# eridgd/WCT-TF

Measured on AMD Instinct MI355X. Metric: stylized frames/sec @512x512, 5-level relu5->1 pipeline, alpha=0.8, higher is better.
Workload: dtype f16

## Files before the change

wct_tf_amd/csrc/api.h:

```cpp
#pragma once
#include "common.h"
#include "../../include/wct_hip.h"

#include <stdio.h>
#include <string.h>
#include <stdlib.h>
#include <memory>
#include <vector>
#include <cmath>
#include <algorithm>

struct DevBuf {
  void* p = nullptr;
  size_t cap = 0;
  DevBuf() = default;
  DevBuf(const DevBuf&) = delete;
  DevBuf& operator=(const DevBuf&) = delete;
  ~DevBuf() { if (p) hipFree(p); }
};

struct ConvLayer {
  half_t* w = nullptr;
  float* b = nullptr;
  half_t* ww = nullptr;
  int cin = 0, cout = 0;
};

struct PlanStep { char kind; int cin, cout, relu; };

struct Decoder {
  bool loaded = false;
  std::vector<PlanStep> plan;
  std::vector<ConvLayer> convs;
  half_t* last_w = nullptr;
  float* last_b = nullptr;
  std::vector<float*> w32, b32, mw, vw, mb, vb, gw, gb;
  std::vector<int> cin, cout;
  float* grad_arena = nullptr;
  size_t grad_count = 0;
};

struct ProfRec { hipEvent_t a, b; int cls; double flops, bytes; };
constexpr int WCT_EIG_WORDS = 2 + 6 * 3;

constexpr int STYLE_CACHE_KEYS = 4;
struct StyleState {
  WctStyleKey key; int kind;
  float* buf;
  unsigned long long stamp;
};
struct StyleSource {
  float* img = nullptr;
  uint8_t* map = nullptr;
  StyleSource() = default;
  StyleSource(const StyleSource&) = delete;
  StyleSource& operator=(const StyleSource&) = delete;
  ~StyleSource() { if (img) hipFree(img); if (map) hipFree(map); }
};
struct wct_style {
  int Hs = 0, Ws = 0;
  unsigned level_set = 0;
  std::shared_ptr<StyleSource> src;
  int label = -1;
  int rows[6] = {0};
  std::vector<StyleState> cache[6];
  ~wct_style() {
    for (auto& lv : cache)
      for (auto& e : lv) if (e.buf) hipFree(e.buf);
  }
};

struct wct_warm {
  unsigned level_set = 0;
  float* basis[6] = {nullptr};
  bool valid[6] = {false};
  ~wct_warm() { for (float* b : basis) if (b) hipFree(b); }
};

struct wct_ctx {
  int device = 0;
  hipStream_t stream = nullptr;
  bool enc_loaded = false;
  half_t* first_w = nullptr;
  float* first_b = nullptr;
  ConvLayer enc[12];
  float* first_w32 = nullptr;
  float* enc_wt[12] = {nullptr};
  DevBuf train_ws;
  Decoder dec[6];
  DevBuf act[2], feat_c, feat_s[6], img_c, img_s, img_t[2], wct_out, wct_ws, stage[4];
  DevBuf usum_c, usum_s[6], umax;
  DevBuf mix_in, feat_mix[6];
  DevBuf mask_in;
  DevBuf region_ws;
  DevBuf tex_noise, tex[2];
  DevBuf band_f, band_g, band_img;
  DevBuf wrap_img, wrap_g, wrap_f;
  DevBuf resize_tab;
  std::vector<int> resize_host;
  ResizeGeom resize_geom = {};
  DevBuf guided_ab;
  int guided_radius = 8, guided_eps = 650;
  std::vector<wct_style*> styles;
  unsigned long long style_clock = 0;
  std::vector<wct_warm*> warms;
  std::vector<wct_warm*> warm_used;

  int* eig_fail = nullptr;
  int* eig_fail_dev = nullptr;
  float ss_alpha = 0.6f;
  int ss_patch = 3, ss_stride = 1;
  bool prof = false;
  bool no_wino = false;
  std::vector<ProfRec> recs;
  std::vector<std::pair<hipEvent_t, hipEvent_t>> free_events;
  double prof_ms[WCT_PROF_CLASSES] = {0};
  long long prof_n[WCT_PROF_CLASSES] = {0};
  double prof_flops[WCT_PROF_CLASSES] = {0};
  double prof_bytes[WCT_PROF_CLASSES] = {0};
};

inline constexpr int LEVEL_C[6] = {0, 64, 128, 256, 512, 512};
inline constexpr int ENC_CIN[12] = {64, 64, 128, 128, 256, 256, 256, 256, 512, 512, 512, 512};
inline constexpr int ENC_COUT[12] = {64, 128, 128, 256, 256, 256, 256, 512, 512, 512, 512, 512};
inline constexpr int ENC_TAP[12] = {0, 2, 0, 3, 0, 0, 0, 4, 0, 0, 0, 5};
inline constexpr int ENC_POOL_AFTER[12] = {1, 0, 1, 0, 0, 0, 1, 0, 0, 0, 1, 0};

#define TRY(expr) do { int _rc = (expr); if (_rc) return _rc; } while (0)

struct ProfScope {
  wct_ctx* c; ProfRec r; bool on;
  ProfScope(wct_ctx* ctx, int cls, double flops, double bytes) : c(ctx), on(ctx->prof) {
    if (!on) return;
    if (c->free_events.empty()) {
      hipEventCreate(&r.a); hipEventCreate(&r.b);
    } else {
      r.a = c->free_events.back().first; r.b = c->free_events.back().second;
      c->free_events.pop_back();
    }
    r.cls = cls; r.flops = flops; r.bytes = bytes;
    hipEventRecord(r.a, c->stream);
  }
  ~ProfScope() {
    if (!on) return;
    hipEventRecord(r.b, c->stream);
    c->recs.push_back(r);
  }
};

struct StageCost { double cov_flops, cov_bytes, apply_flops, apply_bytes, adain_bytes; };

int ensure(wct_ctx* c, DevBuf& b, size_t bytes);
int stage_in(wct_ctx* c, int slot, const void* host, size_t bytes, void** dev);
int fetch(wct_ctx* c, void* host, const void* dev, size_t bytes);
int eig_status(wct_ctx* c);
int eig_stale(wct_ctx* c);
void free_layer(ConvLayer& l);
void free_decoder(Decoder& d);

int upload(wct_ctx* c, const void* host, size_t bytes, void** dev);
int pack_conv(wct_ctx* c, const float* w_hwio, const float* b, int cin, int cout, ConvLayer* out);

static inline WctCall ctx_call(wct_ctx* c, int mode, int stages) {
  WctCall r = {};
  r.mode = mode; r.stages = stages; r.workspace = c->wct_ws.p; r.workspace_bytes = c->wct_ws.cap;
  r.eig_fail = c->eig_fail_dev; r.stream = c->stream;
  return r;
}
template <typename Launch>
static int run_stages(wct_ctx* c, size_t ws_bytes, unsigned flags, const StageCost& cost, Launch&& launch) {
  TRY(ensure(c, c->wct_ws, ws_bytes));
  if (flags & WCT_FLAG_ADAIN) {
    ProfScope ps(c, 7, 0, cost.adain_bytes);
    return launch(ctx_call(c, 0, 0));
  }
  const int mode = (flags & WCT_FLAG_MODE_NP) ? WCT_MODE_NP : WCT_MODE_TF;
  {
    ProfScope ps(c, 4, cost.cov_flops, cost.cov_bytes);
    TRY(launch(ctx_call(c, mode, WCT_STAGE_COV)));
  }
  {
    ProfScope ps(c, 5, 0, 0);
    TRY(launch(ctx_call(c, mode, WCT_STAGE_EIG)));
  }
  ProfScope ps(c, 6, cost.apply_flops, cost.apply_bytes);
  return launch(ctx_call(c, mode, WCT_STAGE_APPLY));
}
void level_dims(int H, int W, int level, int* h, int* w);
int check_min_size(const char* what, int H, int W, int level);
struct ChainLevel { int l, C, H, W, h, w; };
struct Chain { std::vector<ChainLevel> lv; int Ho, Wo; };
int chain_geometry(int Hc, int Wc, const int* levels, int n_levels, Chain* out);
int run_conv(wct_ctx* c, const ConvLayer& l, const half_t* x, half_t* y16, float* y32, int B, int H, int W, int upsample, int relu,
             int pool = 0, float* usum = nullptr, unsigned* umax = nullptr, bool tap_layer = false);
int run_encoder(wct_ctx* c, const float* img, int B, int H, int W, int clamp01, int deepest, float* const taps32[6],
                float* const* usum = nullptr, unsigned* const* umax = nullptr);
int run_decoder(wct_ctx* c, int level, const half_t* feat16, int B, int h, int w, float* img_out);
int run_transform(wct_ctx* c, const float* fc, int Nc, const float* fs, int Ns, int C, int P, float alpha, unsigned flags, float eps,
                  half_t* out16, float* out32, int* sweeps_dev, const WctFeatStats* st = nullptr,
                  const WctStyleRef* prep = nullptr ,
                  const WctWarmRef* warm = nullptr ,
                  const WctStrength* sm = nullptr );
int mix_weights(const float* weights, int K, float* lambda);
int run_transform_mix(wct_ctx* c, const float* fc, int Nc, const float* const* fs, const int* Ns, int K, const float* lambda, int C,
                      float alpha, unsigned flags, float eps, half_t* out16, float* out32, int* sweeps_dev,
                      const WctFeatStats* st = nullptr, const WctStyleRef* prep = nullptr );
int mask_check(const uint8_t* labels, size_t n, int K);
void mask_counts(const uint8_t* mask, int Hm, int Wm, int h, int w, int stride, int K, int* nk);
int run_transform_masked(wct_ctx* c, const float* fc, int Nc, const MaskGeom& g, const int* nk, const float* const* fs, const int* Ns,
                         int K, int C, float alpha, unsigned flags, float eps, half_t* out16, float* out32, int* sweeps_dev);

int band_rows_for(const Chain& chain, int* band_rows);
int band_rows_check(const Chain& chain, int band_rows);
int run_encoder_banded(wct_ctx* c, const float* img, int H, int W, int clamp01, int level, int band_rows, float* F);
int run_decoder_banded(wct_ctx* c, int level, const half_t* G, int h, int w, int band_rows, float* img_out);
int chunk_rule(int h, int w, int C, int stat_rows, int* rows, int* K);
int run_transform_chunked(wct_ctx* c, const float* fc, size_t Nc, int n_full, int K, const float* fs, int Ns, int C, float alpha,
                          unsigned flags, float eps, half_t* out16, float* out32, int* sweeps_dev, const WctStyleRef* prep = nullptr);

void wrap_halo(int level, int* enc, int* dec_before, int* dec_after);
int wrap_chain_check(int H, int W, const int* levels, int n_levels, Chain* chain);

int run_encoder_wrap(wct_ctx* c, const float* img, int B, int H, int W, int clamp01, int level, float* tap);
int run_decoder_wrap(wct_ctx* c, int level, const half_t* G, int B, int h, int w, float* img_out);
int wrap_encoder_buffers(wct_ctx* c, int B, int H, int W, int level);
int wrap_decoder_buffers(wct_ctx* c, int B, int h, int w, int level);

int run_guided_filter(wct_ctx* c, const uint8_t* stylized, const void* content, int content_f32, int B, int Ho, int Wo, int Hc, int Wc,
                      int radius, int eps_q, uint8_t* out);

int warm_live(const wct_ctx* c, const wct_warm* wm);
```

wct_tf_amd/csrc/api_drivers.hip:

```cpp
#include "api.h"

void level_dims(int H, int W, int level, int* h, int* w) {
  for (int l = 1; l < level; ++l) { H = (H + 1) / 2; W = (W + 1) / 2; }
  *h = H; *w = W;
}

int check_min_size(const char* what, int H, int W, int level) {
  int h, w;
  level_dims(H, W, level, &h, &w);
  if (h < 2 || w < 2) {
    wct_set_error("%s %dx%d is too small for relu%d_1: its %dx%d feature map cannot be reflect-padded (need >= %dx%d pixels)",
                  what, H, W, level, h, w, (1 << (level - 1)) + 1, (1 << (level - 1)) + 1);
    return WCT_ERR_ARG;
  }
  return WCT_OK;
}

int chain_geometry(int Hc, int Wc, const int* levels, int n_levels, Chain* out) {
  ARG_CHECK(levels && out && n_levels >= 1 && Hc >= 2 && Wc >= 2);
  out->lv.clear();
  int H = Hc, W = Wc;
  for (int i = 0; i < n_levels; ++i) {
    ARG_CHECK(levels[i] >= 1 && levels[i] <= 5);
    const int l = levels[i];
    TRY(check_min_size("content", H, W, l));
    int h, w;
    level_dims(H, W, l, &h, &w);
    out->lv.push_back(ChainLevel{l, LEVEL_C[l], H, W, h, w});
    H = h << (l - 1); W = w << (l - 1);
  }
  out->Ho = H; out->Wo = W;
  return WCT_OK;
}

int run_conv(wct_ctx* c, const ConvLayer& l, const half_t* x, half_t* y16, float* y32, int B, int H, int W, int upsample, int relu,
             int pool, float* usum, unsigned* umax, bool tap_layer) {
  ConvArgs a;
  a.x = x; a.w = l.w; a.bias = l.b; a.y16 = y16; a.y32 = y32; a.usum = usum; a.umax = umax;
  a.w_wino = c->no_wino || tap_layer ? nullptr : l.ww;
  a.B = B; a.H = H; a.W = W; a.Cin = l.cin; a.Cout = l.cout; a.upsample = upsample; a.relu = relu; a.pool = pool;
  const double px = (double)B * H * W;
  const double in_px = upsample ? px / 4 : px;
  const double out_px = pool ? (double)B * ((H + 1) / 2) * ((W + 1) / 2) : px;
  ProfScope ps(c, conv3x3_wino_takes(a) ? 9 : 0, 2.0 * px * 9 * l.cin * l.cout,
               in_px * l.cin * 2 + out_px * l.cout * ((y16 ? 2 : 0) + (y32 ? 4 : 0)) + 9.0 * l.cin * l.cout * 2);
  return launch_conv3x3(a, c->stream);
}

int run_encoder(wct_ctx* c, const float* img, int B, int H, int W, int clamp01, int deepest, float* const taps32[6],
                float* const* usum, unsigned* const* umax) {
  if (!c->enc_loaded) { wct_set_error("encoder weights not set (wct_set_encoder)"); return WCT_ERR_STATE; }
  ARG_CHECK(deepest >= 1 && deepest <= 5 && H >= 2 && W >= 2);
  const size_t act_bytes = (size_t)B * H * W * 64 * sizeof(half_t);
  TRY(ensure(c, c->act[0], act_bytes));
  TRY(ensure(c, c->act[1], act_bytes));
  half_t* cur = (half_t*)c->act[0].p;
  half_t* nxt = (half_t*)c->act[1].p;
  static const int fuse_conv1_env = getenv("WCT_FUSE_CONV1") ? atoi(getenv("WCT_FUSE_CONV1")) : 1;
  const bool fuse_conv1 = fuse_conv1_env && deepest > 1 && !taps32[1];
  if (!fuse_conv1) {
    ConvFirstArgs a;
    a.x = img; a.wfrag = c->first_w; a.bias = c->first_b;
    a.y16 = deepest > 1 ? cur : nullptr; a.y32 = taps32[1];
    a.B = B; a.H = H; a.W = W; a.clamp01 = clamp01;
    a.usum = usum && taps32[1] ? usum[1] : nullptr; a.umax = a.usum ? umax[1] : nullptr;
    const double px = (double)B * H * W;
    ProfScope ps(c, 1, 2.0 * px * 27 * 64, px * (12 + 64 * ((a.y16 ? 2 : 0) + (a.y32 ? 4 : 0))));
    TRY(launch_conv_first(a, c->stream));
  }
  if (deepest == 1) return WCT_OK;
  int h = H, w = W;
  for (int i = 0; i < 12; ++i) {
    const ConvLayer& l = c->enc[i];
    const int tap = ENC_TAP[i];
    const bool last = tap == deepest;
    const bool fuse = ENC_POOL_AFTER[i];
    float* const us = tap && taps32[tap] && usum ? usum[tap] : nullptr;
    if (i == 0 && fuse_conv1) {
      ConvArgs a;
      a.x = nullptr; a.w = l.w; a.bias = l.b; a.y16 = nxt; a.y32 = nullptr; a.usum = nullptr; a.umax = nullptr;
      a.B = B; a.H = h; a.W = w; a.Cin = 64; a.Cout = 64; a.upsample = 0; a.relu = 1; a.pool = fuse;
      a.img1 = img; a.w1frag = c->first_w; a.bias1 = c->first_b; a.clamp01 = clamp01;
      const double px = (double)B * h * w, out_px = fuse ? (double)B * ((h + 1) / 2) * ((w + 1) / 2) : px;
      ProfScope ps(c, 8, 2.0 * px * (27 * 64 + 9 * 64 * 64), px * 12 + out_px * 64 * 2 + 9.0 * 64 * 64 * 2);
      TRY(launch_conv3x3(a, c->stream));
    } else
    TRY(run_conv(c, l, cur, last ? nullptr : nxt, tap ? taps32[tap] : nullptr, B, h, w, 0, 1, fuse, us, us ? umax[tap] : nullptr, tap != 0));
    half_t* t = cur; cur = nxt; nxt = t;
    if (last) break;
    if (fuse) { h = (h + 1) / 2; w = (w + 1) / 2; }
  }
  return WCT_OK;
}

int run_decoder(wct_ctx* c, int level, const half_t* feat16, int B, int h, int w, float* img_out) {
  Decoder& d = c->dec[level];
  if (!d.loaded) { wct_set_error("decoder weights for relu%d_1 not set (wct_set_decoder)", level); return WCT_ERR_STATE; }
  const int scale = 1 << (level - 1);
  const size_t act_bytes = (size_t)B * h * scale * w * scale * 64 * sizeof(half_t);
  const size_t deep_bytes = (size_t)B * h * w * LEVEL_C[level] * sizeof(half_t) * 4;
  TRY(ensure(c, c->act[0], act_bytes > deep_bytes ? act_bytes : deep_bytes));
  TRY(ensure(c, c->act[1], act_bytes > deep_bytes ? act_bytes : deep_bytes));
  const half_t* cur = feat16;
  half_t* bufs[2] = {(half_t*)c->act[0].p, (half_t*)c->act[1].p};
  int which = 0, ci = 0, up = 0;
  const size_t nsteps = d.plan.size();
  for (size_t si = 0; si < nsteps; ++si) {
    const PlanStep& s = d.plan[si];
    if (s.kind == 'U') { up = 1; h *= 2; w *= 2; continue; }
    if (s.cout == 3) {
      ARG_CHECK(up == 0);
      ConvLastArgs a;
      a.x = cur; a.wfrag = d.last_w; a.bias = d.last_b; a.y = img_out; a.B = B; a.H = h; a.W = w;
      const double px = (double)B * h * w;
      ProfScope ps(c, 2, 2.0 * px * 576 * 3, px * (128 + 12));
      TRY(launch_conv_last(a, c->stream));
    } else {
      half_t* out = bufs[which];
      TRY(run_conv(c, d.convs[ci++], cur, out, nullptr, B, h, w, up, 1));
      cur = out; which ^= 1; up = 0;
    }
  }
  return WCT_OK;
}

int run_transform(wct_ctx* c, const float* fc, int Nc, const float* fs, int Ns, int C, int P, float alpha, unsigned flags, float eps,
                  half_t* out16, float* out32, int* sweeps_dev, const WctFeatStats* st, const WctStyleRef* prep, const WctWarmRef* warm,
                  const WctStrength* sm) {
  const WctSkip skip = (flags & WCT_FLAG_STYLE_SHARED) ? WCT_SKIP_SHARED_STYLE : WCT_SKIP_NONE;
  const StageCost cost = {(double)P * 2.0 * C * C * ((double)Nc + Ns), (double)P * 2.0 * ((double)Nc + Ns) * C * 4,
                          (double)P * (2.0 * C * C * Nc + 6.0 * C * C * C),
                          (double)P * Nc * C * (4 + (out16 ? 2 : 0) + (out32 ? 4 : 0) + (sm ? 4 : 0)) + (sm ? (double)P * Nc : 0.0),
                          (double)P * (2.0 * Nc + 2.0 * Ns) * C * 4 + (double)P * Nc * C * 6 + (sm ? (double)P * Nc : 0.0)};
  return run_stages(c, wct_workspace_bytes(C, Nc, Ns, P), flags, cost, [&](WctCall r) {
    r.alpha = alpha; r.eps = r.stages ? eps : 1e-5f; r.out16 = out16; r.out32 = out32; r.sweeps_dev = sweeps_dev;
    if (!r.stages) return launch_adain(fc, Nc, fs, Ns, C, P, skip, r, st, prep, sm);
    return launch_wct(fc, Nc, fs, Ns, C, P, skip, r, st, prep, warm, sm);
  });
}

int mix_weights(const float* weights, int K, float* lambda) {
  if (K < 1 || K > WCT_MIX_MAX) { wct_set_error("style mix: K = %d styles, must be 1 .. %d", K, (int)WCT_MIX_MAX); return WCT_ERR_ARG; }
  if (!weights) { wct_set_error("style mix: no weights"); return WCT_ERR_ARG; }
  double sum = 0.0;
  for (int k = 0; k < K; ++k) {
    if (!(weights[k] >= 0.f) || !std::isfinite(weights[k])) {
      wct_set_error("style mix: weight %d is %g; weights must be finite and >= 0", k, (double)weights[k]);
      return WCT_ERR_ARG;
    }
    sum += weights[k];
  }
  if (!(sum > 0.0) || !std::isfinite(sum)) { wct_set_error("style mix: the weights sum to %g, must be > 0", sum); return WCT_ERR_ARG; }
  for (int k = 0; k < K; ++k) lambda[k] = (float)(weights[k] / sum);
  return WCT_OK;
}

int run_transform_mix(wct_ctx* c, const float* fc, int Nc, const float* const* fs, const int* Ns, int K, const float* lambda, int C,
                      float alpha, unsigned flags, float eps, half_t* out16, float* out32, int* sweeps_dev, const WctFeatStats* st,
                      const WctStyleRef* prep) {
  double ns = 0;
  for (int k = 0; k < K; ++k) ns += Ns[k];
  const StageCost cost = {2.0 * C * C * (Nc + ns), 2.0 * (Nc + ns) * C * 4, 2.0 * C * C * Nc + 6.0 * C * C * C * (K + 1) + 2.0 * C * C * K,
                          (double)Nc * C * (4 + (out16 ? 2 : 0) + (out32 ? 4 : 0)), (2.0 * Nc + 2.0 * ns) * C * 4 + (double)Nc * C * 6};
  return run_stages(c, wct_mix_workspace_bytes(C, Nc, Ns, K, lambda), flags, cost, [&](WctCall r) {
    r.alpha = alpha; r.eps = r.stages ? eps : 1e-5f; r.out16 = out16; r.out32 = out32; r.sweeps_dev = sweeps_dev;
    if (!r.stages) return launch_adain_mix(fc, Nc, fs, Ns, K, lambda, C, r, st, prep);
    return launch_wct_mix(fc, Nc, fs, Ns, K, lambda, C, r, st, prep);
  });
}

int mask_check(const uint8_t* labels, size_t n, int K) {
  if (K < 1 || K > WCT_MIX_MAX) { wct_set_error("mask: K = %d styles, must be 1 .. %d", K, (int)WCT_MIX_MAX); return WCT_ERR_ARG; }
  uint8_t top = 0;
  for (size_t i = 0; i < n; ++i) top = labels[i] > top ? labels[i] : top;
  if (top >= K) { wct_set_error("mask: label %d with K = %d styles (labels must be 0 .. K - 1)", (int)top, K); return WCT_ERR_ARG; }
  return WCT_OK;
}

void mask_counts(const uint8_t* mask, int Hm, int Wm, int h, int w, int stride, int K, int* nk) {
  for (int k = 0; k < K; ++k) nk[k] = 0;
  for (int i = 0; i < h; ++i) {
    const uint8_t* row = mask + (size_t)std::min(i * stride, Hm - 1) * Wm;
    for (int j = 0; j < w; ++j) ++nk[row[std::min(j * stride, Wm - 1)]];
  }
}

int run_transform_masked(wct_ctx* c, const float* fc, int Nc, const MaskGeom& g, const int* nk, const float* const* fs, const int* Ns,
                         int K, int C, float alpha, unsigned flags, float eps, half_t* out16, float* out32, int* sweeps_dev) {
  double ns = 0;
  int P = 0;
  for (int k = 0; k < K; ++k) { ns += nk[k] >= 2 ? Ns[k] : 0; P += nk[k] >= 2; }
  const StageCost cost = {2.0 * C * C * (Nc + ns), (4.0 * Nc + 2.0 * (Nc + ns)) * C * 4, 2.0 * C * C * Nc + 6.0 * C * C * C * P,
                          (double)Nc * C * (4 + (out16 ? 2 : 0) + (out32 ? 4 : 0)), (4.0 * Nc + 2.0 * ns) * C * 4 + (double)Nc * C * 6};
  return run_stages(c, wct_masked_workspace_bytes(C, Nc, nk, Ns, K), flags, cost, [&](WctCall r) {
    r.alpha = alpha; r.eps = r.stages ? eps : 1e-5f; r.out16 = out16; r.out32 = out32; r.sweeps_dev = sweeps_dev;
    if (!r.stages) return launch_adain_masked(fc, Nc, g, nk, fs, Ns, K, C, r);
    return launch_wct_masked(fc, Nc, g, nk, fs, Ns, K, C, r);
  });
}
```

wct_tf_amd/csrc/api_stylize.hip:

```cpp
#include "api.h"

extern "C" int wct_output_size(int Hc, int Wc, const int* levels, int n_levels, int* Ho, int* Wo) {
  ARG_CHECK(Ho && Wo);
  Chain chain;
  TRY(chain_geometry(Hc, Wc, levels, n_levels, &chain));
  *Ho = chain.Ho; *Wo = chain.Wo;
  return WCT_OK;
}

static int check_levels(const wct_ctx* c, const int* levels, int n_levels, const wct_style* const* handles = nullptr, int K = 0) {
  for (int i = 0; i < n_levels; ++i) {
    ARG_CHECK(levels[i] >= 1 && levels[i] <= 5);
    for (int k = 0; k < K; ++k)
      if (!(handles[k]->level_set & (1u << levels[i]))) {
        wct_set_error("prepared style %d was not prepared for relu%d_1", k, levels[i]);
        return WCT_ERR_ARG;
      }
    if (!c->dec[levels[i]].loaded) { wct_set_error("decoder weights for relu%d_1 not set", levels[i]); return WCT_ERR_STATE; }
  }
  return WCT_OK;
}

static int stylize_checks(wct_ctx* c, int Hc, int Wc, const uint8_t* const* styles, const int* Hs, const int* Ws, int K,
                          const int* levels, int n_levels, int* deepest, Chain* chain) {
  TRY(check_levels(c, levels, n_levels));
  TRY(chain_geometry(Hc, Wc, levels, n_levels, chain));
  *deepest = *std::max_element(levels, levels + n_levels);
  for (int k = 0; k < K; ++k) { ARG_CHECK(styles[k]); TRY(check_min_size("style", Hs[k], Ws[k], *deepest)); }
  return WCT_OK;
}

static size_t sample_bytes(unsigned flags) { return (flags & WCT_FLAG_IMAGES_F32) ? sizeof(float) : 1; }

static int images_f32(wct_ctx* c, unsigned flags, const void* content, size_t nc, const void* style, size_t ns, const float** img_c,
                      const float** img_s) {
  *img_c = (const float*)content; *img_s = (const float*)style;
  if (flags & WCT_FLAG_IMAGES_F32) return WCT_OK;
  TRY(ensure(c, c->img_c, nc * 4));
  TRY(ensure(c, c->img_s, ns * 4));
  ProfScope ps(c, 7, 0, (double)(nc + ns) * 5);
  TRY(launch_u8_to_f32((const uint8_t*)content, (float*)c->img_c.p, nc, c->stream));
  TRY(launch_u8_to_f32((const uint8_t*)style, (float*)c->img_s.p, ns, c->stream));
  *img_c = (const float*)c->img_c.p; *img_s = (const float*)c->img_s.p;
  return WCT_OK;
}

constexpr size_t UROW = 32 * UMAX_SLOTS;
static bool fuse_stats() {
  static const int on = getenv("WCT_FUSE_STATS") ? atoi(getenv("WCT_FUSE_STATS")) : 1;
  return on != 0;
}

template <typename StyleAt, typename Transform>
static int stylize_levels(wct_ctx* c, const float* img_c, const void* content_raw, int B, const Chain& chain, unsigned flags,
                          size_t umax_clear, int clear_from, StyleAt&& style_at, Transform&& transform, uint8_t* out) {
  unsigned* const umax_c = (unsigned*)c->umax.p;
  const float* cur = img_c;
  for (int i = 0; i < (int)chain.lv.size(); ++i) {
    const ChainLevel& g = chain.lv[i];
    const int l = g.l, C = g.C, h = g.h, w = g.w;
    TRY(ensure(c, c->feat_c, (size_t)B * h * w * C * 4));
    float* ctaps[6] = {};
    ctaps[l] = (float*)c->feat_c.p;
    float* us_c[6] = {};
    unsigned* um_c[6] = {};
    if (fuse_stats() && w % 16 == 0) {
      TRY(ensure(c, c->usum_c, (size_t)B * h * (w / 16) * C * 4));
      us_c[l] = (float*)c->usum_c.p; um_c[l] = umax_c;
      if (i >= clear_from) HIP_TRY(hipMemsetAsync(umax_c, 0, umax_clear, c->stream));
    }
    WctFeatStats st = {};
    st.u[0] = us_c[l]; st.umax[0] = um_c[l];
    TRY(run_encoder(c, cur, B, g.H, g.W, i > 0, l, ctaps, us_c, um_c));
    TRY(ensure(c, c->wct_out, (size_t)B * h * w * C * 2));
    if (l == 5 && (flags & WCT_FLAG_SWAP5)) {
      int hs, ws;
      style_at(l, 0, &hs, &ws);
      ARG_CHECK(h >= c->ss_patch && w >= c->ss_patch && hs >= c->ss_patch && ws >= c->ss_patch);
      TRY(ensure(c, c->wct_ws, style_swap_workspace_bytes(C, h, w, hs, ws, c->ss_patch, c->ss_stride)));
      ProfScope ps(c, 7, 0, 0);
      for (int b = 0; b < B; ++b)
        TRY(launch_style_swap((float*)c->feat_c.p + (size_t)b * h * w * C, h, w, style_at(l, b, &hs, &ws), hs, ws, C, c->ss_alpha,
                              c->ss_patch, c->ss_stride, -1.f, (half_t*)c->wct_out.p + (size_t)b * h * w * C, nullptr,
                              c->wct_ws.p, c->wct_ws.cap, c->stream, c->eig_fail_dev));
    } else
      TRY(transform(i, g, st));
    DevBuf& dst = c->img_t[i & 1];
    TRY(ensure(c, dst, (size_t)B * (h << (l - 1)) * (w << (l - 1)) * 3 * 4));
    TRY(run_decoder(c, l, (half_t*)c->wct_out.p, B, h, w, (float*)dst.p));
    cur = (float*)dst.p;
  }
  const int H = chain.Ho, W = chain.Wo, Hc = chain.lv[0].H, Wc = chain.lv[0].W;
  const int f32 = (flags & WCT_FLAG_IMAGES_F32) ? 1 : 0;
  if (flags & WCT_FLAG_GUIDED) {
    {
      ProfScope ps(c, 7, 0, (double)B * H * W * 3 * 5);
      TRY(launch_f32_to_u8(cur, out, (size_t)B * H * W * 3, c->stream));
    }
    TRY(run_guided_filter(c, out, content_raw, f32, B, H, W, Hc, Wc, c->guided_radius, c->guided_eps, out));
    if (!(flags & WCT_FLAG_CONTENT_COLORS)) return WCT_OK;
    ProfScope ps(c, 7, 0, (double)B * H * W * 3 * 2 + (double)B * Hc * Wc * 3 * (f32 ? 4 : 1));
    return launch_content_colors_u8_any(out, content_raw, f32, B, H, W, Hc, Wc, out, c->stream);
  }
  if (flags & WCT_FLAG_CONTENT_COLORS) {
    ProfScope ps(c, 7, 0, (double)B * H * W * 3 * 5 + (double)B * Hc * Wc * 3 * (f32 ? 4 : 1));
    return launch_content_colors_f32(cur, content_raw, f32, B, H, W, Hc, Wc, out, c->stream);
  }
  ProfScope ps(c, 7, 0, (double)B * H * W * 3 * 5);
  return launch_f32_to_u8(cur, out, (size_t)B * H * W * 3, c->stream);
}

template <typename Enqueue>
static int host_frame(wct_ctx* c, const uint8_t* content, int Hc, int Wc, const int* levels, int n_levels, unsigned flags,
                      uint8_t* out, Enqueue&& enqueue) {
  HIP_TRY(hipSetDevice(c->device));
  TRY(eig_stale(c));
  int Ho, Wo;
  TRY(wct_output_size(Hc, Wc, levels, n_levels, &Ho, &Wo));
  void* dc;
  TRY(stage_in(c, 0, content, (size_t)Hc * Wc * 3 * sample_bytes(flags), &dc));
  TRY(ensure(c, c->stage[2], (size_t)Ho * Wo * 3));
  TRY(enqueue(dc, (uint8_t*)c->stage[2].p));
  TRY(fetch(c, out, c->stage[2].p, (size_t)Ho * Wo * 3));
  return eig_status(c);
}

extern "C" int wct_stylize_batch_dev(wct_ctx* c, const uint8_t* content, int Hc, int Wc, const uint8_t* style,
                                     int Hs, int Ws, int B, const int* levels, int n_levels, float alpha,
                                     unsigned flags, uint8_t* out) {
  ARG_CHECK(c && content && style && out && levels && n_levels >= 1 && n_levels <= 16 && B >= 1 && B <= 32);
  HIP_TRY(hipSetDevice(c->device));
  int deepest;
  Chain chain;
  TRY(stylize_checks(c, Hc, Wc, &style, &Hs, &Ws, 1, levels, n_levels, &deepest, &chain));

  const int shared = (flags & WCT_FLAG_STYLE_SHARED) ? 1 : 0;
  const int Bs = shared ? 1 : B;
  const float *img_c, *img_s;
  TRY(images_f32(c, flags, content, (size_t)B * Hc * Wc * 3, style, (size_t)Bs * Hs * Ws * 3, &img_c, &img_s));
  const bool want_stats = fuse_stats();
  TRY(ensure(c, c->umax, 7 * UROW * sizeof(unsigned)));
  unsigned* const umax_c = (unsigned*)c->umax.p;
  if (want_stats) HIP_TRY(hipMemsetAsync(c->umax.p, 0, 7 * UROW * sizeof(unsigned), c->stream));
  float* taps[6] = {};
  float* us_s[6] = {};
  unsigned* um_s[6] = {};
  for (int i = 0; i < n_levels; ++i) {
    const int l = levels[i];
    int h, w;
    level_dims(Hs, Ws, l, &h, &w);
    TRY(ensure(c, c->feat_s[l], (size_t)Bs * h * w * LEVEL_C[l] * 4));
    taps[l] = (float*)c->feat_s[l].p;
    if (want_stats && w % 16 == 0) {
      TRY(ensure(c, c->usum_s[l], (size_t)Bs * h * (w / 16) * LEVEL_C[l] * 4));
      us_s[l] = (float*)c->usum_s[l].p; um_s[l] = umax_c + UROW * l;
    }
  }
  TRY(run_encoder(c, img_s, Bs, Hs, Ws, 0, deepest, taps, us_s, um_s));

  auto style_at = [&](int l, int b, int* hs, int* ws) {
    level_dims(Hs, Ws, l, hs, ws);
    return (const float*)c->feat_s[l].p + (size_t)(shared ? 0 : b) * *hs * *ws * LEVEL_C[l];
  };
  return stylize_levels(c, img_c, content, B, chain, flags, UROW * sizeof(unsigned), 1, style_at,
                        [&](int, const ChainLevel& g, WctFeatStats st) {
                          int hs, ws;
                          const float* fs = style_at(g.l, 0, &hs, &ws);
                          st.u[1] = us_s[g.l]; st.umax[1] = um_s[g.l];
                          return run_transform(c, (float*)c->feat_c.p, g.h * g.w, fs, hs * ws, g.C, B, alpha, flags, -1.f,
                                               (half_t*)c->wct_out.p, nullptr, nullptr, &st);
                        }, out);
}

extern "C" int wct_stylize(wct_ctx* c, const uint8_t* content, int Hc, int Wc, const uint8_t* style, int Hs, int Ws,
                           const int* levels, int n_levels, float alpha, unsigned flags, uint8_t* out) {
  ARG_CHECK(c && content && style && out);
  return host_frame(c, content, Hc, Wc, levels, n_levels, flags, out, [&](void* dc, uint8_t* frame) {
    void* ds;
    TRY(stage_in(c, 1, style, (size_t)Hs * Ws * 3 * sample_bytes(flags), &ds));
    return wct_stylize_batch_dev(c, (uint8_t*)dc, Hc, Wc, (uint8_t*)ds, Hs, Ws, 1, levels, n_levels, alpha, flags, frame);
  });
}

template <typename LevelTransform>
static int stylize_multi(wct_ctx* c, const uint8_t* content, int Hc, int Wc, const uint8_t* const* styles, const int* Hs,
                         const int* Ws, int K, const int* levels, int n_levels, unsigned flags, uint8_t* out,
                         LevelTransform&& level_transform) {
  HIP_TRY(hipSetDevice(c->device));
  int deepest;
  Chain chain;
  TRY(stylize_checks(c, Hc, Wc, styles, Hs, Ws, K, levels, n_levels, &deepest, &chain));
  TRY(eig_stale(c));
  const size_t px = sample_bytes(flags);
  size_t ns_tot = 0, soff[WCT_MIX_MAX];
  for (int k = 0; k < K; ++k) { soff[k] = ns_tot; ns_tot += (size_t)Hs[k] * Ws[k] * 3; }
  const size_t nc = (size_t)Hc * Wc * 3;
  void* dc;
  TRY(stage_in(c, 0, content, nc * px, &dc));
  TRY(ensure(c, c->mix_in, ns_tot * px));
  for (int k = 0; k < K; ++k)
    HIP_TRY(hipMemcpyAsync((char*)c->mix_in.p + soff[k] * px, styles[k], (size_t)Hs[k] * Ws[k] * 3 * px, hipMemcpyHostToDevice, c->stream));
  const float *img_c, *img_s;
  TRY(images_f32(c, flags, dc, nc, c->mix_in.p, ns_tot, &img_c, &img_s));

  size_t foff[6][WCT_MIX_MAX];
  for (int i = 0; i < n_levels; ++i) {
    const int l = levels[i];
    size_t tot = 0;
    for (int k = 0; k < K; ++k) {
      int h, w;
      level_dims(Hs[k], Ws[k], l, &h, &w);
      foff[l][k] = tot;
      tot += (size_t)h * w * LEVEL_C[l];
    }
    TRY(ensure(c, c->feat_mix[l], tot * 4));
  }
  for (int k = 0; k < K; ++k) {
    float* taps[6] = {};
    for (int i = 0; i < n_levels; ++i) taps[levels[i]] = (float*)c->feat_mix[levels[i]].p + foff[levels[i]][k];
    TRY(run_encoder(c, img_s + soff[k], 1, Hs[k], Ws[k], 0, deepest, taps));
  }

  TRY(ensure(c, c->umax, 32 * UMAX_SLOTS * sizeof(unsigned)));
  const size_t frame_bytes = (size_t)chain.Ho * chain.Wo * 3;
  TRY(ensure(c, c->stage[2], frame_bytes));
  auto style_at = [&](int l, int k, int* hs, int* ws) {
    level_dims(Hs[k], Ws[k], l, hs, ws);
    return (const float*)c->feat_mix[l].p + foff[l][k];
  };
  TRY(stylize_levels(c, img_c, dc, 1, chain, flags, UMAX_SLOTS * sizeof(unsigned), 0, style_at,
                     [&](int, const ChainLevel& g, const WctFeatStats& st) {
                       const float* fs[WCT_MIX_MAX];
                       int Ns[WCT_MIX_MAX];
                       for (int k = 0; k < K; ++k) {
                         int hs, ws;
                         fs[k] = style_at(g.l, k, &hs, &ws);
                         Ns[k] = hs * ws;
                       }
                       return level_transform(g, fs, Ns, &st);
                     }, (uint8_t*)c->stage[2].p));
  TRY(fetch(c, out, c->stage[2].p, frame_bytes));
  return eig_status(c);
}

extern "C" int wct_stylize_mix(wct_ctx* c, const uint8_t* content, int Hc, int Wc, const uint8_t* const* styles, const int* Hs,
                               const int* Ws, int K, const float* weights, const int* levels, int n_levels, float alpha,
                               unsigned flags, uint8_t* out) {
  ARG_CHECK(c && content && styles && Hs && Ws && out && levels && n_levels >= 1 && n_levels <= 16);
  float lambda[WCT_MIX_MAX];
  TRY(mix_weights(weights, K, lambda));
  if ((flags & WCT_FLAG_SWAP5) && K > 1) {
    wct_set_error("style mix: WCT_FLAG_SWAP5 needs K = 1 (style-swap is not linear in the style; got K = %d)", K);
    return WCT_ERR_ARG;
  }
  if (flags & WCT_FLAG_STYLE_SHARED) { wct_set_error("style mix: WCT_FLAG_STYLE_SHARED is for wct_stylize_batch_dev"); return WCT_ERR_ARG; }
  return stylize_multi(c, content, Hc, Wc, styles, Hs, Ws, K, levels, n_levels, flags, out,
                       [&](const ChainLevel& g, const float* const* fs, const int* Ns, const WctFeatStats* st) {
                         return run_transform_mix(c, (float*)c->feat_c.p, g.h * g.w, fs, Ns, K, lambda, g.C, alpha, flags, -1.f,
                                                  (half_t*)c->wct_out.p, nullptr, nullptr, st);
                       });
}

extern "C" int wct_stylize_masked(wct_ctx* c, const uint8_t* content, int Hc, int Wc, const uint8_t* mask, const uint8_t* const* styles,
                                  const int* Hs, const int* Ws, int K, const int* levels, int n_levels, float alpha, unsigned flags,
                                  uint8_t* out) {
  ARG_CHECK(c && content && mask && styles && Hs && Ws && out && levels && n_levels >= 1 && n_levels <= 16 && Hc >= 2 && Wc >= 2);
  TRY(mask_check(mask, (size_t)Hc * Wc, K));
  if ((flags & WCT_FLAG_SWAP5) && K > 1) {
    wct_set_error("mask: WCT_FLAG_SWAP5 needs K = 1 (style-swap is not a per-region affine map; got K = %d)", K);
    return WCT_ERR_ARG;
  }
  if (flags & WCT_FLAG_STYLE_SHARED) { wct_set_error("mask: WCT_FLAG_STYLE_SHARED is for wct_stylize_batch_dev"); return WCT_ERR_ARG; }
  for (int i = 0; i < n_levels; ++i) ARG_CHECK(levels[i] >= 1 && levels[i] <= 5);
  HIP_TRY(hipSetDevice(c->device));
  TRY(ensure(c, c->mask_in, (size_t)Hc * Wc));
  HIP_TRY(hipMemcpyAsync(c->mask_in.p, mask, (size_t)Hc * Wc, hipMemcpyHostToDevice, c->stream));
  return stylize_multi(c, content, Hc, Wc, styles, Hs, Ws, K, levels, n_levels, flags, out,
                       [&](const ChainLevel& g, const float* const* fs, const int* Ns, const WctFeatStats*) {
                         int nk[WCT_MIX_MAX];
                         mask_counts(mask, Hc, Wc, g.h, g.w, 1 << (g.l - 1), K, nk);
                         const MaskGeom mg = {(const uint8_t*)c->mask_in.p, Hc, Wc, g.w, 1 << (g.l - 1)};
                         return run_transform_masked(c, (float*)c->feat_c.p, g.h * g.w, mg, nk, fs, Ns, K, g.C, alpha, flags, -1.f,
                                                     (half_t*)c->wct_out.p, nullptr, nullptr);
                       });
}

int warm_live(const wct_ctx* c, const wct_warm* wm) {
  if (wm && std::find(c->warms.begin(), c->warms.end(), wm) != c->warms.end()) return WCT_OK;
  wct_set_error("warm state %p is not a live state of this context (freed, or created by another context)", (const void*)wm);
  return WCT_ERR_STATE;
}

extern "C" int wct_warm_create(wct_ctx* c, const int* levels, int n_levels, wct_warm** out) {
  ARG_CHECK(c && levels && out && n_levels >= 1 && n_levels <= 16);
  *out = nullptr;
  for (int i = 0; i < n_levels; ++i) ARG_CHECK(levels[i] >= 1 && levels[i] <= 5);
  HIP_TRY(hipSetDevice(c->device));
  std::unique_ptr<wct_warm> wm(new wct_warm());
  for (int i = 0; i < n_levels; ++i) {
    const int l = levels[i];
    if (wm->basis[l]) continue;
    wm->level_set |= 1u << l;
    if (hipMalloc((void**)&wm->basis[l], (size_t)LEVEL_C[l] * LEVEL_C[l] * sizeof(float)) != hipSuccess) {
      wct_set_error("hipMalloc failed (warm state, relu%d_1)", l);
      return WCT_ERR_NOMEM;
    }
  }
  c->warms.push_back(wm.get());
  *out = wm.release();
  return WCT_OK;
}

extern "C" void wct_warm_free(wct_ctx* c, wct_warm* wm) {
  if (!c || !wm) return;
  auto it = std::find(c->warms.begin(), c->warms.end(), wm);
  if (it == c->warms.end()) return;
  hipSetDevice(c->device);
  hipStreamSynchronize(c->stream);
  c->warms.erase(it);
  c->warm_used.erase(std::remove(c->warm_used.begin(), c->warm_used.end(), wm), c->warm_used.end());
  delete wm;
}

extern "C" int wct_warm_reset(wct_ctx* c, wct_warm* wm) {
  ARG_CHECK(c != nullptr);
  TRY(warm_live(c, wm));
  for (bool& v : wm->valid) v = false;
  return WCT_OK;
}

extern "C" int wct_warm_basis(wct_ctx* c, const wct_warm* wm, int level, int* valid, float* V_host) {
  ARG_CHECK(c && valid);
  TRY(warm_live(c, wm));
  if (level < 1 || level > 5 || !(wm->level_set & (1u << level))) {
    wct_set_error("warm state: relu%d_1 is not in the state's level set", level);
    return WCT_ERR_ARG;
  }
  HIP_TRY(hipSetDevice(c->device));
  HIP_TRY(hipStreamSynchronize(c->stream));
  *valid = wm->valid[level] ? 1 : 0;
  if (V_host && wm->valid[level]) TRY(fetch(c, V_host, wm->basis[level], (size_t)LEVEL_C[level] * LEVEL_C[level] * sizeof(float)));
  return WCT_OK;
}

static int style_live(const wct_ctx* c, const wct_style* st) {
  if (st && std::find(c->styles.begin(), c->styles.end(), st) != c->styles.end()) return WCT_OK;
  wct_set_error("prepared style %p is not a live handle of this context (freed, or prepared by another context)", (const void*)st);
  return WCT_ERR_STATE;
}

static bool same_key(const WctStyleKey& a, const WctStyleKey& b) { return a.nslab == b.nslab && a.nsplit == b.nsplit && a.ksplit == b.ksplit; }

static StyleState* state_find(wct_style* st, int level, const WctStyleKey& key, int kind) {
  for (auto& e : st->cache[level])
    if (e.kind == kind && same_key(e.key, key)) return &e;
  return nullptr;
}

struct StyleNeed { int level; WctStyleKey key; };

static int style_rows(const wct_style* st, int level) { return st->rows[level]; }

static int region_count(const uint8_t* map, int Hm, int Wm, int h, int w, int stride, int label) {
  int n = 0;
  for (int i = 0; i < h; ++i) {
    const uint8_t* row = map + (size_t)std::min(i * stride, Hm - 1) * Wm;
    for (int j = 0; j < w; ++j) n += row[std::min(j * stride, Wm - 1)] == label;
  }
  return n;
}

static int style_fill(wct_ctx* c, wct_style* const* group, int G, int kind, const std::vector<StyleNeed>* needs) {
  bool any = false;
  for (int g = 0; g < G; ++g) any = any || !needs[g].empty();
  if (!any) return WCT_OK;
  HIP_TRY(hipStreamSynchronize(c->stream));
  const wct_style* st0 = group[0];
  const bool region = st0->label >= 0;
  int deepest = 0, labels = 0;
  size_t row_floats = 0;
  float* taps[6] = {};
  for (int g = 0; g < G; ++g)
    for (const StyleNeed& n : needs[g]) {
      int h, w;
      level_dims(st0->Hs, st0->Ws, n.level, &h, &w);
      TRY(ensure(c, c->feat_s[n.level], (size_t)h * w * LEVEL_C[n.level] * 4));
      taps[n.level] = (float*)c->feat_s[n.level].p;
      deepest = std::max(deepest, n.level);
      labels = std::max(labels, group[g]->label + 1);
      row_floats = std::max(row_floats, (size_t)style_rows(group[g], n.level) * LEVEL_C[n.level]);
    }
  int *perm[6] = {}, *seg_off[6] = {};
  void* compact_ws = nullptr;
  float* rows = nullptr;
  if (region) {
    size_t off = 0, poff[6] = {}, soff[6] = {}, cbytes = 0;
    auto take = [&](size_t bytes) { const size_t at = off; off += (bytes + 255) & ~(size_t)255; return at; };
    for (int l = 1; l <= 5; ++l) {
      if (!taps[l]) continue;
      int h, w;
      level_dims(st0->Hs, st0->Ws, l, &h, &w);
      poff[l] = take((size_t)h * w * sizeof(int));
      soff[l] = take((WCT_MIX_MAX + 1) * sizeof(int));
      cbytes = std::max(cbytes, mask_compact_workspace_bytes(h * w));
    }
    const size_t coff = take(cbytes), roff = take(row_floats * sizeof(float));
    TRY(ensure(c, c->region_ws, off));
    char* base = (char*)c->region_ws.p;
    for (int l = 1; l <= 5; ++l)
      if (taps[l]) { perm[l] = (int*)(base + poff[l]); seg_off[l] = (int*)(base + soff[l]); }
    compact_ws = base + coff;
    rows = (float*)(base + roff);
  }
  TRY(run_encoder(c, st0->src->img, 1, st0->Hs, st0->Ws, 0, deepest, taps));
  if (region)
    for (int l = 1; l <= 5; ++l) {
      if (!taps[l]) continue;
      int h, w;
      level_dims(st0->Hs, st0->Ws, l, &h, &w);
      ProfScope ps(c, 7, 0, (double)h * w * 2);
      TRY(launch_mask_compact(MaskGeom{st0->src->map, st0->Hs, st0->Ws, w, 1 << (l - 1)}, h * w, labels, perm[l], seg_off[l], compact_ws,
                              c->stream));
    }
  std::vector<float*> fresh;
  int rc = WCT_OK;
  for (int g = 0; g < G && !rc; ++g) {
    wct_style* st = group[g];
    int gathered = 0;
    for (const StyleNeed& n : needs[g]) {
      const int C = LEVEL_C[n.level], Ns = style_rows(st, n.level);
      auto& lv = st->cache[n.level];
      float* buf = nullptr;
      if ((int)lv.size() >= STYLE_CACHE_KEYS) {
        int old = -1;
        for (int i = 0; i < (int)lv.size(); ++i)
          if (lv[i].stamp != c->style_clock && (old < 0 || lv[i].stamp < lv[old].stamp)) old = i;
        if (old >= 0) { buf = lv[old].buf; lv.erase(lv.begin() + old); }
      }
      if (!buf && hipMalloc((void**)&buf, wct_style_state_floats(C) * sizeof(float)) != hipSuccess) {
        wct_set_error("hipMalloc failed (prepared style state, relu%d_1)", n.level);
        rc = WCT_ERR_NOMEM;
        break;
      }
      lv.push_back(StyleState{n.key, kind, buf, c->style_clock});
      fresh.push_back(buf);
      if (hipMemsetAsync(buf, 0, wct_style_state_floats(C) * sizeof(float), c->stream) != hipSuccess) { wct_set_error("hipMemsetAsync failed"); rc = WCT_ERR_HIP; break; }
      const float* feat = taps[n.level];
      if (region) {
        if (gathered != n.level) {
          ProfScope ps(c, 7, 0, (double)Ns * C * 8);
          if ((rc = launch_mask_gather_segment(taps[n.level], perm[n.level], seg_off[n.level], st->label, Ns, C, rows, c->stream))) break;
          gathered = n.level;
        }
        feat = rows;
      }
      if ((rc = ensure(c, c->wct_ws, wct_style_workspace_bytes(C, Ns, n.key)))) break;
      ProfScope ps(c, kind == 2 ? 7 : 5, 0, 0);
      WctCall r = ctx_call(c, kind == 1 ? WCT_MODE_NP : WCT_MODE_TF, WCT_STAGE_ALL);
      r.eps = -1.f;
      if ((rc = launch_style_state(feat, Ns, C, n.key, kind == 2, r, buf))) break;
    }
  }
  if (!rc && hipStreamSynchronize(c->stream) != hipSuccess) { wct_set_error("hipStreamSynchronize failed (prepared style)"); rc = WCT_ERR_HIP; }
  if (!rc) rc = eig_status(c);
  if (rc) {
    hipStreamSynchronize(c->stream);
    for (int g = 0; g < G; ++g)
      for (auto& lv : group[g]->cache)
        for (size_t i = lv.size(); i-- > 0;)
          if (std::find(fresh.begin(), fresh.end(), lv[i].buf) != fresh.end()) { hipFree(lv[i].buf); lv.erase(lv.begin() + i); }
  }
  return rc;
}

// ... 709 lines not shown
```

wct_tf_amd/csrc/common.h:

```cpp
#pragma once
#include <hip/hip_runtime.h>
#include <stdint.h>
#include <stddef.h>
#include "skip_rule.h"

typedef _Float16 half_t;
typedef _Float16 half8 __attribute__((ext_vector_type(8)));
typedef _Float16 half4 __attribute__((ext_vector_type(4)));
typedef float f32x16 __attribute__((ext_vector_type(16)));
typedef float f32x4 __attribute__((ext_vector_type(4)));

#define WCT_OK 0
#define WCT_ERR_HIP -1
#define WCT_ERR_ARG -2
#define WCT_ERR_STATE -3
#define WCT_ERR_NOMEM -4
#define WCT_ERR_NOCONV -5

void wct_set_error(const char* fmt, ...);

#define HIP_TRY(expr)                                                          \
  do {                                                                         \
    hipError_t _e = (expr);                                                    \
    if (_e != hipSuccess) {                                                    \
      wct_set_error("%s failed: %s (%s:%d)", #expr, hipGetErrorString(_e),     \
                    __FILE__, __LINE__);                                       \
      return WCT_ERR_HIP;                                                      \
    }                                                                          \
  } while (0)

#define ARG_CHECK(cond)                                                        \
  do {                                                                         \
    if (!(cond)) {                                                             \
      wct_set_error("invalid argument: %s (%s:%d)", #cond, __FILE__, __LINE__);\
      return WCT_ERR_ARG;                                                      \
    }                                                                          \
  } while (0)

static inline int cdiv(int a, int b) { return (a + b - 1) / b; }

constexpr size_t WCT_LAUNCH_BYTES = (size_t)1 << 31;
static inline bool launch_map_fits(size_t elems, size_t bytes) { return elems * bytes < WCT_LAUNCH_BYTES; }


struct ConvArgs {
  const half_t* x;
  const half_t* w;
  const float* bias;
  half_t* y16;
  float* y32;
  int B, H, W;
  int Cin, Cout;
  int upsample;
  int relu;
  int pool;
  float* usum;
  unsigned* umax;
  const float* img1 = nullptr;
  const half_t* w1frag = nullptr;
  const float* bias1 = nullptr;
  int clamp01 = 0;
  const half_t* w_wino = nullptr;
};
constexpr int UMAX_SLOTS = 64;
__device__ __forceinline__ void umax_merge(unsigned* umax_img, int slot, float vmax, int lane) {
#pragma unroll
  for (int o = 32; o > 0; o >>= 1) vmax = fmaxf(vmax, __shfl_xor(vmax, o, 64));
  if (lane == 0) {
    unsigned* w = umax_img + (slot & (UMAX_SLOTS - 1));
    const unsigned bits = __builtin_bit_cast(unsigned, vmax);
    if (bits > __atomic_load_n(w, __ATOMIC_RELAXED)) atomicMax(w, bits);
  }
}
int launch_conv3x3(const ConvArgs& a, hipStream_t s);
bool conv3x3_wino_takes(const ConvArgs& a);
int launch_conv3x3_wino(const ConvArgs& a, hipStream_t s);

struct ConvFirstArgs {
  const float* x;
  const half_t* wfrag;
  const float* bias;
  half_t* y16;
  float* y32;
  int B, H, W;
  int clamp01;
  float* usum;
  unsigned* umax;
};

__device__ __forceinline__ void unit_row_sum4(f32x4& t) {
  float a = t[0], b = t[1], c = t[2], d = t[3];
#define WCT_DPP_STEP(ctrl)                                                             \
  "v_add_f32_dpp %0, %0, %0 " ctrl " row_mask:0xf bank_mask:0xf bound_ctrl:1\n"       \
  "v_add_f32_dpp %1, %1, %1 " ctrl " row_mask:0xf bank_mask:0xf bound_ctrl:1\n"       \
  "v_add_f32_dpp %2, %2, %2 " ctrl " row_mask:0xf bank_mask:0xf bound_ctrl:1\n"       \
  "v_add_f32_dpp %3, %3, %3 " ctrl " row_mask:0xf bank_mask:0xf bound_ctrl:1\n"
  asm volatile("s_nop 1\n"
               WCT_DPP_STEP("quad_perm:[1,0,3,2]")
               WCT_DPP_STEP("quad_perm:[2,3,0,1]")
               WCT_DPP_STEP("row_half_mirror")
               WCT_DPP_STEP("row_mirror")
               : "+v"(a), "+v"(b), "+v"(c), "+v"(d));
#undef WCT_DPP_STEP
  t[0] = a; t[1] = b; t[2] = c; t[3] = d;
}
int launch_conv_first(const ConvFirstArgs& a, hipStream_t s);

struct ConvLastArgs {
  const half_t* x;
  const half_t* wfrag;
  const float* bias;
  float* y;
  int B, H, W;
};
int launch_conv_last(const ConvLastArgs& a, hipStream_t s);

int launch_maxpool2x2(const half_t* x, half_t* y, int B, int H, int W, int C, hipStream_t s);
int launch_u8_to_f32(const uint8_t* x, float* y, size_t n, hipStream_t s);
int launch_f32_to_u8(const float* x, uint8_t* y, size_t n, hipStream_t s);
int launch_f32_to_f16(const float* x, half_t* y, size_t n, hipStream_t s);
int launch_f16_to_f32(const half_t* x, float* y, size_t n, hipStream_t s);

struct GemmArgs {
  const float* A; int lda; int a_kmajor;
  const float* B; int ldb; int b_kmajor;
  const float* a_sub_m;
  const float* b_sub_n;
  const float* a_sub_k;
  const float* a_scale_k;
  int M, N, K;
  int ksplit;
  float* out32; half_t* out16; int ldo;
  size_t out_split_stride;
  const float* bias_n;
  int nsplit;
  size_t sA, sB, s_sub_m, s_sub_n, s_sub_k, s_scale_k, s_out, s_bias;
  const float* A_odd;
  size_t sA_odd;
  WctSkip skip;
  int blend; float alpha; unsigned* mabs;
  const float* mask_diag; size_t s_mask; int* mask_out; const int* mask_in;
};

int launch_gemm(GemmArgs g, int nsplit, int nbatch, hipStream_t s);

enum { WCT_MODE_NP = 0, WCT_MODE_TF = 1 };

struct WctFeatStats { const float* u[2]; const unsigned* umax[2]; };

struct WctStyleKey { int nslab, nsplit, ksplit; };
WctStyleKey wct_style_key(int C, int Nc, int Ns);
size_t wct_style_state_floats(int C);
size_t wct_style_workspace_bytes(int C, int Ns, const WctStyleKey& key);
struct WctStyleRef { const float* state[8]; };
struct WctStyleSlots { const float* state[32]; };

struct WctWarmRef { float* basis; int valid; };

struct WctStrength { const uint8_t* smap; int Hm, Wm, w, stride; };

struct WctCall {
  float alpha; int mode;
  float eps;
  half_t* out16; float* out32;
  void* workspace; size_t workspace_bytes;
  int* sweeps_dev;
  int stages;
  int* eig_fail;
  hipStream_t stream;
};
enum { WCT_STAGE_COV = 1, WCT_STAGE_EIG = 2, WCT_STAGE_APPLY = 4, WCT_STAGE_ALL = 7, WCT_STAGE_EIG_FP32UPDATE = 8 };

int launch_style_state(const float* style, int Ns, int C, const WctStyleKey& key, int adain, const WctCall& r, float* state);

size_t wct_workspace_bytes(int C, int Nc, int Ns, int P);
int launch_wct(const float* content, int Nc, const float* style, int Ns, int C, int P, WctSkip skip, const WctCall& r,
               const WctFeatStats* stats, const WctStyleRef* prep, const WctWarmRef* warm, const WctStrength* sm = nullptr);
int launch_adain(const float* content, int Nc, const float* style, int Ns, int C, int P, WctSkip skip, const WctCall& r,
                 const WctFeatStats* stats, const WctStyleRef* prep, const WctStrength* sm = nullptr);
enum { WCT_MIX_MAX = 8 };
size_t wct_mix_workspace_bytes(int C, int Nc, const int* Ns, int K, const float* lambda);
int launch_wct_mix(const float* content, int Nc, const float* const* styles, const int* Ns, int K, const float* lambda, int C,
                   const WctCall& r, const WctFeatStats* stats, const WctStyleRef* prep);
int launch_adain_mix(const float* content, int Nc, const float* const* styles, const int* Ns, int K, const float* lambda, int C,
                     const WctCall& r, const WctFeatStats* stats, const WctStyleRef* prep);
struct MaskGeom { const uint8_t* mask; int Hm, Wm, w, stride; };
size_t mask_compact_workspace_bytes(int N, int G = 1);
int launch_mask_compact(const MaskGeom& g, int N, int K, int* perm, int* seg_off, void* workspace, hipStream_t s);
int launch_mask_gather_segment(const float* x, const int* perm, const int* seg_off, int k, int nk, int C, float* xg, hipStream_t s);
size_t wct_masked_workspace_bytes(int C, int Nc, const int* nk, const int* Ns, int K);
int launch_wct_masked(const float* content, int Nc, const MaskGeom& g, const int* nk, const float* const* styles, const int* Ns, int K,
                      int C, const WctCall& r);
int launch_adain_masked(const float* content, int Nc, const MaskGeom& g, const int* nk, const float* const* styles, const int* Ns, int K,
                        int C, const WctCall& r);
size_t wct_masked_batch_workspace_bytes(int C, int Nc, int G, const int* nk, const int* Ns, int K);
int wct_masked_batch_pairs(int G, const int* nk, int K);
int launch_mask_compact_batch(const MaskGeom& g, int N, int K, int G, int* perm, int* seg_off, void* workspace, hipStream_t s);
int launch_wct_masked_batch(const float* content, int Nc, int G, const MaskGeom& g, const int* nk, const int* Ns, int K, int C,
                            const WctCall& r, const WctStyleSlots& states);
int launch_adain_masked_batch(const float* content, int Nc, int G, const MaskGeom& g, const int* nk, const int* Ns, int K, int C,
                              const WctCall& r, const WctStyleSlots& states);
int launch_jacobi_eigh(float* A, float* V, int C, int nmat, void* workspace,
                       size_t workspace_bytes, int* sweeps_done_dev, int* eig_fail, hipStream_t s);
size_t jacobi_workspace_bytes(int C, int nmat);

size_t style_swap_workspace_bytes(int C, int hc, int wc, int hs, int ws, int patch, int stride);
int launch_style_swap(const float* content, int hc, int wc, const float* style, int hs, int ws, int C,
                      float alpha, int patch, int stride, float eps, half_t* out16, float* out32,
                      void* workspace, size_t workspace_bytes, hipStream_t s, int* eig_fail);

int launch_im2col_act(const half_t* x, float* col, int B, int H, int W, int C, int upsample, hipStream_t s);
int launch_im2col_grad(const float* g, float* col, int B, int H, int W, int C, hipStream_t s);
int launch_reflect_fold(const float* gp, float* g, int B, int H, int W, int C, hipStream_t s);
int launch_relu_mask16(float* g, const half_t* act, size_t n, hipStream_t s);
int launch_relu_mask32(float* g, const float* act, size_t n, hipStream_t s);
int launch_upsample_adjoint(const float* gb, float* gs, int B, int h, int w, int C, hipStream_t s);
int launch_maxpool_adjoint(const half_t* pre, const float* gpool, float* gpre, int B, int H, int W, int C, hipStream_t s);
int launch_mse(const float* a, const float* b, size_t n, float weight, float* grad, int accumulate, double* partial,
               float* loss_out, hipStream_t s);
int launch_tv(const float* x, int B, int H, int W, int C, float weight, float* grad, double* partial, float* loss_out, hipStream_t s);
int launch_bias_grad(const float* g, size_t rows, int C, float* partial, float* out, hipStream_t s);
int launch_reduce_slabs(const float* partial, size_t n, int nslab, float* out, hipStream_t s);
int launch_adam(float* w, float* m, float* v, const float* g, size_t n, float lr_t, float b1, float b2, float eps, hipStream_t s);
int launch_pack_conv_frag(const float* w, half_t* frag, int cin, int cout, hipStream_t s);
int launch_pack_conv_wino_frag(const float* w, half_t* frag, int cin, int cout, hipStream_t s);
int launch_pack_last_frag(const float* w, half_t* frag, hipStream_t s);
int launch_transpose_w(const float* w, float* wt, int cin, int cout, int cout_pad, hipStream_t s);
int launch_pad3to4(const float* x, float* y, size_t n, hipStream_t s);
int launch_conv_dgrad(const float* g, const float* wt, int B, int H, int W, int cin, int cout,
                      float* col, float* gp, float* gin, void* scratch, hipStream_t s);
int launch_conv_wgrad(const half_t* x16, int upsample, const float* g, int ldg, int B, int H, int W, int cin, int cout,
                      float* col, float* partial, int nsplit, float* dw, void* scratch, hipStream_t s);
int conv_wgrad_splits(int B, int H, int W);
int launch_pow2_scale(const float* x, size_t n, void* scratch, hipStream_t s);
int launch_conv_first_dgrad(const float* g, const float* wf, float* gp, int B, int H, int W, hipStream_t s);

struct CoralApplyArgs {
  double M[9], src_mean[3], src_std[3], tgt_mean[3], tgt_std[3];
};
int launch_coral_stats(const uint8_t* img, size_t npix, unsigned long long* partial, int nblocks,
                       unsigned long long* out9, hipStream_t s);
int launch_coral_apply(const uint8_t* src, size_t npix, const CoralApplyArgs& a, uint8_t* out_u8,
                       double* out_f64, hipStream_t s);

int launch_content_colors_f32(const float* frame, const void* content, int content_f32, int B, int Ho, int Wo, int Hc, int Wc,
                              uint8_t* out, hipStream_t s);
int launch_content_colors_u8(const uint8_t* stylized, const uint8_t* content, int B, int Ho, int Wo, int Hc, int Wc, uint8_t* out,
                             hipStream_t s);
int launch_content_colors_u8_any(const uint8_t* stylized, const void* content, int content_f32, int B, int Ho, int Wo, int Hc, int Wc,
                                 uint8_t* out, hipStream_t s);

int guided_check(int B, int Ho, int Wo, int Hc, int Wc, int radius, int eps_q);
size_t guided_workspace_bytes(int B, int Ho, int Wo);
int launch_guided_filter(const uint8_t* stylized, const void* content, int content_f32, int B, int Ho, int Wo, int Hc, int Wc, int radius,
                         int eps_q, void* workspace, uint8_t* out, hipStream_t s);

int launch_texture_noise(uint8_t* out, int B, int H, int W, unsigned seed, unsigned first_sample, int smooth, hipStream_t s);

int launch_wrap_pad(const void* in, void* out, int B, int H, int W, int E, int elem_bytes, int t, int b, int l, int r, hipStream_t s);
int launch_wrap_crop(const void* in, void* out, int B, int Hp, int Wp, int E, int elem_bytes, int t, int l, int h, int w, hipStream_t s);

struct ResizeGeom { int H, W, h, w, ksx, ksy, th; };
int resize_check_bytes(int B, int H, int W, int h, int w);
size_t resize_table_ints(int H, int W, int h, int w);
int resize_plan(int H, int W, int h, int w, ResizeGeom* g, int* tabs);
int launch_resize(const uint8_t* in, uint8_t* out, int B, const ResizeGeom& g, const int* tabs_dev, hipStream_t s);
```

wct_tf_amd/csrc/conv.hip:

```cpp
#include "common.h"
#include "conv_tile.h"


template <int MT, int NT, bool POOL, bool OUT32>
__device__ __forceinline__ void conv_epilogue_t(const ConvArgs& p, f32x16 (&acc)[NT][MT], int b, int y0, int x0, int n0,
                                                int wm, int wn, int lane, const unsigned char* bias_lds) {
  constexpr int OOB = (int)0x80000000u;
  const int frag_px = lane & 15;
  const int frag_py = (lane & 31) >> 4;
  const int kgrp = lane >> 5;
  const int Ho = POOL ? (p.H + 1) / 2 : p.H, Wo = POOL ? (p.W + 1) / 2 : p.W;
  const unsigned img_elems = (unsigned)Ho * Wo * p.Cout;
  const __amdgpu_buffer_rsrc_t r16 = __builtin_amdgcn_make_buffer_rsrc(
      (void*)(p.y16 ? p.y16 + (size_t)b * img_elems : nullptr), 0, p.y16 ? img_elems * 2 : 0, 0x00020000);
  const __amdgpu_buffer_rsrc_t r32 = __builtin_amdgcn_make_buffer_rsrc(
      (void*)(OUT32 && p.y32 ? p.y32 + (size_t)b * img_elems : nullptr), 0, OUT32 && p.y32 ? img_elems * 4 : 0, 0x00020000);
  f32x4 bvs[NT][4];
#pragma unroll
  for (int nt = 0; nt < NT; ++nt)
#pragma unroll
    for (int rq = 0; rq < 4; ++rq)
      bvs[nt][rq] = *reinterpret_cast<const f32x4*>(bias_lds + ((wn * NT + nt) * 32 + 8 * rq + 4 * kgrp) * 4);
  const float lo1 = p.relu ? 0.f : -__builtin_inff();
  const h2 lo2 = {(half_t)lo1, (half_t)lo1};
  const int ox = x0 + frag_px;
  const int chan = n0 + wn * NT * 32;
  const bool stats = OUT32 && p.usum != nullptr;
  float* const us = stats ? p.usum + (size_t)b * (p.H * (p.W >> 4)) * p.Cout + chan + 4 * kgrp : nullptr;
  float vmax = 0.f;
#pragma unroll
  for (int mt = 0; mt < MT; ++mt) {
    const int oy = y0 + (wm * MT + mt) * 2 + frag_py;
    const bool in_img = (oy < p.H) & (ox < p.W);
    const bool inside = POOL ? (in_img & (frag_py == 0) & ((frag_px & 1) == 0)) : in_img;
    const int pix = POOL ? (oy >> 1) * Wo + (ox >> 1) : oy * p.W + ox;
    const int off16 = inside ? (pix * p.Cout + chan + 8 * kgrp) * 2 : OOB;
    const int off32 = inside ? (pix * p.Cout + chan + 4 * kgrp) * 4 : OOB;
#pragma unroll
    for (int nt = 0; nt < NT; ++nt) {
      unsigned pk[4][2];
#pragma unroll
      for (int rq = 0; rq < 4; ++rq) {
        f32x4 v;
#pragma unroll
        for (int j = 0; j < 4; ++j) v[j] = acc[nt][mt][rq * 4 + j] + bvs[nt][rq][j];
        if (OUT32) {
#pragma unroll
          for (int j = 0; j < 4; ++j) v[j] = fmaxf(v[j], lo1);
          __builtin_amdgcn_raw_buffer_store_b128(__builtin_bit_cast(u32x4, v), r32, off32 + (nt * 32 + 8 * rq) * 4, 0, 0);
          if (stats) {
            f32x4 t = v;
            unit_row_sum4(t);
            if (in_img) {
              vmax = fmaxf(fmaxf(vmax, fmaxf(v[0], v[1])), fmaxf(v[2], v[3]));
              if (frag_px == 0)
                *reinterpret_cast<f32x4*>(us + (size_t)(oy * (p.W >> 4) + (x0 >> 4)) * p.Cout + nt * 32 + 8 * rq) = t;
            }
          }
        }
        h2 lo = {(half_t)v[0], (half_t)v[1]}, hi = {(half_t)v[2], (half_t)v[3]};
        if (!OUT32) {
          lo = __builtin_elementwise_max(lo, lo2);
          hi = __builtin_elementwise_max(hi, lo2);
        }
        if (POOL) {
          const h2 zero = {(half_t)0.f, (half_t)0.f};
          h2 q[2] = {in_img ? lo : zero, in_img ? hi : zero};
#pragma unroll
          for (int d = 0; d < 2; ++d) {
            unsigned t = __builtin_bit_cast(unsigned, q[d]);
            const h2 o = __builtin_bit_cast(h2, __builtin_amdgcn_update_dpp(0, (int)t, 0xB1, 0xF, 0xF, true));
            q[d] = __builtin_elementwise_max(q[d], o);
            t = __builtin_bit_cast(unsigned, q[d]);
            const auto rows = __builtin_amdgcn_permlane16_swap(t, t, false, false);
            q[d] = __builtin_elementwise_max(__builtin_bit_cast(h2, (unsigned)rows[0]), __builtin_bit_cast(h2, (unsigned)rows[1]));
          }
          lo = q[0]; hi = q[1];
        }
        pk[rq][0] = __builtin_bit_cast(unsigned, lo);
        pk[rq][1] = __builtin_bit_cast(unsigned, hi);
      }
#pragma unroll
      for (int m = 0; m < 2; ++m) {
        auto sx = __builtin_amdgcn_permlane32_swap(pk[2 * m][0], pk[2 * m + 1][0], false, false);
        auto sy = __builtin_amdgcn_permlane32_swap(pk[2 * m][1], pk[2 * m + 1][1], false, false);
        u32x4 o = {sx[0], sy[0], sx[1], sy[1]};
        __builtin_amdgcn_raw_buffer_store_b128(o, r16, off16 + (nt * 32 + 16 * m) * 2, 0, 0);
      }
    }
  }
  if (stats) umax_merge(p.umax + b * UMAX_SLOTS, (int)blockIdx.x * 4 + (int)(threadIdx.x >> 6), vmax, lane);
}

template <int MT, int NT>
__device__ __forceinline__ void conv_epilogue(const ConvArgs& p, f32x16 (&acc)[NT][MT], int b, int y0, int x0, int n0,
                                              int wm, int wn, int lane, const unsigned char* bias_lds) {
  if (p.pool) conv_epilogue_t<MT, NT, true, false>(p, acc, b, y0, x0, n0, wm, wn, lane, bias_lds);
  else if (p.y32) conv_epilogue_t<MT, NT, false, true>(p, acc, b, y0, x0, n0, wm, wn, lane, bias_lds);
  else conv_epilogue_t<MT, NT, false, false>(p, acc, b, y0, x0, n0, wm, wn, lane, bias_lds);
}

template <int TH, int BN, int WM, int WN, bool FUSE1 = false>
__global__ __launch_bounds__(256, ((TH / 2) / WM) * ((BN / 32) / WN) > 8 ? 1 : 2) void conv3x3_mfma_kernel(ConvArgs p, int tiles_x, int tiles_y, int n_tiles, int strip) {
  constexpr int PH = TH + 2;
  constexpr int MT = (TH / 2) / WM;
  constexpr int NT = (BN / 32) / WN;
  constexpr int PATCH_ITEMS = PH * 18 * 4;
  constexpr int PATCH_PER_THREAD = (PATCH_ITEMS + 255) / 256;
  constexpr int PATCH_BYTES = PH * PITCH * 64;
  constexpr bool DB = MT * NT > 8;
  constexpr int NBUF = DB ? 2 : 1;
  constexpr int DUMP_OFF = PATCH_BYTES;
  constexpr int BUF_STRIDE = PATCH_BYTES + 4096;
  constexpr int BIAS_OFF = NBUF * BUF_STRIDE;
  constexpr int IMG_OFF = BIAS_OFF + BN * 4, IMG_H = TH + 4, IMG_W = 20, IMG_ROW = IMG_W * 3, IMG_ZERO = IMG_OFF + IMG_H * IMG_ROW * 4;
  constexpr int W1_OFF = IMG_ZERO + 64, B1_OFF = W1_OFF + 8192;
  constexpr int STG_OFF = B1_OFF + 256;
  static_assert(!FUSE1 || (BN == 64 && !(((TH / 2) / WM) * ((BN / 32) / WN) > 8)), "FUSE1: 64 output channels, single patch buffer");
  constexpr int PF_TAP = TH <= 16 ? 6 : 9;

  extern __shared__ __attribute__((aligned(16))) unsigned char smem[];
  unsigned char* const patch_lds = smem;

  int bid = blockIdx.x;
  const int ntile = bid % n_tiles;
  bid /= n_tiles;
  const int strips_x = FUSE1 ? (tiles_x + strip - 1) / strip : tiles_x;
  const int tx = FUSE1 ? (bid % strips_x) * strip : bid % strips_x;
  const int ty = bid / strips_x;
  const int b = blockIdx.y;
  int y0 = ty * TH;
  int x0 = tx * TW;
  int strip_i = 0;
  const int n0 = ntile * BN;
  int tid_ = threadIdx.x;

next_tile:
  if (FUSE1) asm volatile("" : "+v"(tid_), "+s"(y0));
  const int tid = tid_;
  const int lane = tid & 63;
  const int wave = tid >> 6;
  const int wm = wave / WN, wn = wave % WN;

  const int Hin = p.upsample ? p.H / 2 : p.H;
  const int Win = p.upsample ? p.W / 2 : p.W;
  const half_t* xb = p.x + (size_t)b * Hin * Win * p.Cin;

  unsigned patch_src[PATCH_PER_THREAD];
  unsigned patch_dst[PATCH_PER_THREAD];
#pragma unroll
  for (int i = 0; i < PATCH_PER_THREAD; ++i) {
    int item = tid + i * 256;
    int valid = item < PATCH_ITEMS;
    int pix = valid ? item >> 2 : 0;
    int chunk = item & 3;
    int py = pix / 18, px = pix - py * 18;
    int iy = reflect_idx(y0 - 1 + py, p.H);
    int ix = reflect_idx(x0 - 1 + px, p.W);
    if (p.upsample) { iy >>= 1; ix >>= 1; }
    patch_src[i] = valid ? ((iy * Win + ix) * p.Cin + chunk * 8) * 2 : 0;
    patch_dst[i] = valid ? ((py * PITCH + px) * 4 + (chunk ^ ((px >> 2) & 3))) * 16 : DUMP_OFF + tid * 16;
  }

  const int frag_px = lane & 15;
  const int frag_py = (lane & 31) >> 4;
  const int kgrp = lane >> 5;

  int rd_base[3][2];
#pragma unroll
  for (int kx = 0; kx < 3; ++kx)
#pragma unroll
    for (int ks = 0; ks < 2; ++ks) {
      const int px = frag_px + kx;
      rd_base[kx][ks] = ((wm * MT * 2 + frag_py) * PITCH + px) * 64 + (((ks * 2 + kgrp) ^ ((px >> 2) & 3)) * 16);
    }

  const int c16 = p.Cin >> 4;
  unsigned wfrag[NT];
#pragma unroll
  for (int nt = 0; nt < NT; ++nt)
    wfrag[nt] = (((n0 >> 5) + wn * NT + nt) * 9 * c16 * 512 + lane * 8) * 2;
  const __amdgpu_buffer_rsrc_t w_rsrc = __builtin_amdgcn_make_buffer_rsrc((void*)p.w, 0, 0x7FFFFFFF, 0x00020000);
  const __amdgpu_buffer_rsrc_t x_rsrc = __builtin_amdgcn_make_buffer_rsrc((void*)xb, 0, 0x7FFFFFFF, 0x00020000);

  f32x16 acc[NT][MT];
  if (tid < BN / 4 && strip_i == 0)
    *reinterpret_cast<f32x4*>(smem + BIAS_OFF + tid * 16) = *reinterpret_cast<const f32x4*>(p.bias + n0 + tid * 4);

  const int n_chunks = p.Cin / BK;
  u32x4 patch_regs[PATCH_PER_THREAD];
  half8 wf[2][NT][2];
  half8 bf[2][MT];

  auto read_group = [&](half8 (&dst)[MT], int ky, int kx, int ks, int buf) {
#pragma unroll
    for (int mt = 0; mt < MT; ++mt)
      dst[mt] = *reinterpret_cast<const half8*>(patch_lds + rd_base[kx][ks] + (mt * 2 + ky) * PITCH * 64 + buf * BUF_STRIDE);
  };
  auto mma_group = [&](half8 (&w)[NT][2], half8 (&bq)[MT], int ks) {
#pragma unroll
    for (int mt = 0; mt < MT; ++mt)
#pragma unroll
      for (int nt = 0; nt < NT; ++nt)
        acc[nt][mt] = __builtin_amdgcn_mfma_f32_32x32x16_f16(w[nt][ks], bq[mt], acc[nt][mt], 0, 0, 0);
  };
  auto load_patch = [&](int chunk) {
#pragma unroll
    for (int i = 0; i < PATCH_PER_THREAD; ++i)
      patch_regs[i] = __builtin_amdgcn_raw_buffer_load_b128(x_rsrc, patch_src[i], chunk * BK * 2, 0);
  };
  auto store_patch = [&](int buf) {
#pragma unroll
    for (int i = 0; i < PATCH_PER_THREAD; ++i)
      *reinterpret_cast<u32x4*>(smem + patch_dst[i] + buf * BUF_STRIDE) = patch_regs[i];
  };

  auto make_patch = [&](int chunk) {
    typedef _Float16 h2v __attribute__((ext_vector_type(2)));
    const unsigned char* w1 = smem + W1_OFF + chunk * 4096;
    half8 wh[2], wl[2];
#pragma unroll
    for (int ks = 0; ks < 2; ++ks) {
      wh[ks] = *reinterpret_cast<const half8*>(w1 + ((ks * 2 + 0) * 64 + lane) * 16);
      wl[ks] = *reinterpret_cast<const half8*>(w1 + ((ks * 2 + 1) * 64 + lane) * 16);
    }
    const int l = lane & 31, kg = lane >> 5;
    f32x4 b1[4];
#pragma unroll
    for (int rq = 0; rq < 4; ++rq) b1[rq] = *reinterpret_cast<const f32x4*>(smem + B1_OFF + (chunk * 32 + 8 * rq + 4 * kg) * 4);
    constexpr int NMAIN = PH / 2, NEDGE = (PH + 15) / 16, NT1 = (NMAIN + NEDGE + 3) / 4, R = IMG_ROW;
    const int pxm = l & 15, pxe = 16 + (l & 1);
    const int colm = IMG_OFF + (reflect_idx(x0 - 1 + pxm, p.W) - x0 + 1) * 12 - (y0 - 1) * R * 4;
    const int cole = IMG_OFF + (reflect_idx(x0 - 1 + pxe, p.W) - x0 + 1) * 12 - (y0 - 1) * R * 4;
    const int dstm = pxm * 64 + kg * 8, dste = pxe * 64 + kg * 8, swm = (pxm >> 2) & 3;
#pragma unroll 1
    for (int t = 0; t < NT1; ++t) {
      const int T = t * 4 + wave;
      const bool edge = T >= NMAIN;
      const int py = edge ? (T - NMAIN) * 16 + (l >> 1) : 2 * T + (l >> 4);
      const bool valid = py < PH && T < NMAIN + NEDGE;
      const int pyc = py < PH ? py : PH - 1;
      const int base = (edge ? cole : colm) + reflect_idx(y0 - 1 + pyc, p.H) * (R * 4);
      const unsigned char* b8 = smem + base + kg * 32;
      const unsigned char* bR = smem + base + kg * (R - 1) * 4;
      unsigned w[2][8];
      w[0][0] = *reinterpret_cast<const unsigned*>(b8);
#pragma unroll
      for (int j = 1; j < 8; ++j) w[0][j] = *reinterpret_cast<const unsigned*>(bR + j * 4);
      w[1][0] = *reinterpret_cast<const unsigned*>(bR + (R + 7) * 4);
      w[1][1] = *reinterpret_cast<const unsigned*>(bR + (R + 8) * 4);
#pragma unroll
      for (int j = 2; j < 8; ++j) w[1][j] = *reinterpret_cast<const unsigned*>(b8 + (2 * R + j - 2) * 4);
      f32x16 a1;
#pragma unroll
      for (int r = 0; r < 16; ++r) a1[r] = 0.f;
#pragma unroll
      for (int ks = 0; ks < 2; ++ks) {
        unsigned uh[4], ul[4];
#pragma unroll
        for (int i2 = 0; i2 < 4; ++i2) {
          uh[i2] = __builtin_amdgcn_perm(w[ks][2 * i2 + 1], w[ks][2 * i2], 0x05040100u);
          ul[i2] = __builtin_amdgcn_perm(w[ks][2 * i2 + 1], w[ks][2 * i2], 0x07060302u);
        }
        const half8 bh = __builtin_bit_cast(half8, u32x4{uh[0], uh[1], uh[2], uh[3]});
        const half8 bl = __builtin_bit_cast(half8, u32x4{ul[0], ul[1], ul[2], ul[3]});
        a1 = __builtin_amdgcn_mfma_f32_32x32x16_f16(wl[ks], bh, a1, 0, 0, 0);
        a1 = __builtin_amdgcn_mfma_f32_32x32x16_f16(wh[ks], bl, a1, 0, 0, 0);
        a1 = __builtin_amdgcn_mfma_f32_32x32x16_f16(wh[ks], bh, a1, 0, 0, 0);
      }
      const int dst = valid ? pyc * (PITCH * 64) + (edge ? dste : dstm) : DUMP_OFF + tid * 16;
      const int sw = valid && !edge ? swm : 0;
      const h2v zero2 = {(half_t)0.f, (half_t)0.f};
#pragma unroll
      for (int rq = 0; rq < 4; ++rq) {
        h2v h0 = {(half_t)(a1[rq * 4 + 0] + b1[rq][0]), (half_t)(a1[rq * 4 + 1] + b1[rq][1])};
        h2v h1 = {(half_t)(a1[rq * 4 + 2] + b1[rq][2]), (half_t)(a1[rq * 4 + 3] + b1[rq][3])};
        h0 = __builtin_elementwise_max(h0, zero2);
        h1 = __builtin_elementwise_max(h1, zero2);
        typedef unsigned u32x2 __attribute__((ext_vector_type(2)));
        *reinterpret_cast<u32x2*>(smem + dst + (valid ? (rq ^ sw) * 16 : 0)) = u32x2{__builtin_bit_cast(unsigned, h0), __builtin_bit_cast(unsigned, h1)};
      }
    }
  };

  constexpr int IMG_NP = IMG_H * IMG_W, IMG_PER = (IMG_NP + 255) / 256;
  auto fetch_img = [&](int xt) {
    const float* ib = p.img1 + (size_t)b * p.H * p.W * 3;
#pragma unroll
    for (int i = 0; i < IMG_PER; ++i) {
      const int e = tid + i * 256, ee = e < IMG_NP ? e : IMG_NP - 1;
      const int ry = ee / IMG_W, rx = ee - ry * IMG_W;
      const float* s = ib + ((size_t)reflect_idx(y0 - 2 + ry, p.H) * p.W + reflect_idx(xt - 2 + rx, p.W)) * 3;
#pragma unroll
      for (int c = 0; c < 3; ++c)
        __builtin_amdgcn_global_load_lds(s + c, reinterpret_cast<__attribute__((address_space(3))) void*>(
            (__attribute__((address_space(3))) unsigned char*)smem + STG_OFF + ((i * 3 + c) * 256 + wave * 64) * 4), 4, 0, 0);
    }
  };
  auto park_img = [&]() {
    asm volatile("s_waitcnt vmcnt(0)" ::: "memory");
#pragma unroll
    for (int i = 0; i < IMG_PER; ++i) {
      const int e = tid + i * 256;
      if (e < IMG_NP) {
#pragma unroll
        for (int c = 0; c < 3; ++c) {
          const float raw = *reinterpret_cast<const float*>(smem + STG_OFF + ((i * 3 + c) * 256 + tid) * 4);
          const float v = p.clamp01 ? fminf(fmaxf(raw, 0.f), 1.f) : raw;
          const half_t hi = (half_t)v, lo = (half_t)(v - (float)hi);
          *reinterpret_cast<unsigned*>(smem + IMG_OFF + (e * 3 + c) * 4) =
              (unsigned)__builtin_bit_cast(unsigned short, hi) | ((unsigned)__builtin_bit_cast(unsigned short, lo) << 16);
        }
      }
    }
  };
  if (FUSE1 && strip_i == 0) {
    fetch_img(x0);
    const u32x4 wa = *reinterpret_cast<const u32x4*>(reinterpret_cast<const unsigned char*>(p.w1frag) + tid * 32);
    const u32x4 wb = *reinterpret_cast<const u32x4*>(reinterpret_cast<const unsigned char*>(p.w1frag) + tid * 32 + 16);
    *reinterpret_cast<u32x4*>(smem + W1_OFF + tid * 32) = wa;
    *reinterpret_cast<u32x4*>(smem + W1_OFF + tid * 32 + 16) = wb;
    if (tid < 16) {
      *reinterpret_cast<f32x4*>(smem + B1_OFF + tid * 16) = *reinterpret_cast<const f32x4*>(p.bias1 + tid * 4);
      *reinterpret_cast<unsigned*>(smem + IMG_ZERO + tid * 4) = 0u;
    }
  }

#pragma unroll
  for (int nt = 0; nt < NT; ++nt)
#pragma unroll
    for (int mt = 0; mt < MT; ++mt)
#pragma unroll
      for (int r = 0; r < 16; ++r) acc[nt][mt][r] = 0.f;
  if (FUSE1) {
    park_img();
  } else {
    load_patch(0);
  }
#pragma unroll
  for (int nt = 0; nt < NT; ++nt)
#pragma unroll
    for (int ks = 0; ks < 2; ++ks)
      wf[0][nt][ks] = __builtin_bit_cast(half8, __builtin_amdgcn_raw_buffer_load_b128(w_rsrc, wfrag[nt] + ks * 1024, 0, 0));
  if (FUSE1) {
    __syncthreads();
    make_patch(0);
  } else {
    store_patch(0);
  }
  __syncthreads();
  read_group(bf[0], 0, 0, 0, 0);

#pragma unroll 1
  for (int pair = 0; pair < n_chunks; pair += 2) {
#pragma unroll
    for (int t = 0; t < 18; ++t) {
      const int tap = t % 9, chunk_i = pair + t / 9;
      const int ky = tap / 3, kx = tap % 3;
      const int ntap = (tap + 1) % 9, nky = ntap / 3, nkx = ntap % 3;
      const bool more = chunk_i + 1 < n_chunks;
      const int buf = DB ? t / 9 : 0;
      {
        const int nchunk = tap == 8 ? (more ? chunk_i + 1 : chunk_i) : chunk_i;
        const int wtap = (ntap * c16 + nchunk * 2) * 1024;
#pragma unroll
        for (int nt = 0; nt < NT; ++nt)
#pragma unroll
          for (int ks = 0; ks < 2; ++ks)
            wf[(t + 1) & 1][nt][ks] =
                __builtin_bit_cast(half8, __builtin_amdgcn_raw_buffer_load_b128(w_rsrc, wfrag[nt] + ks * 1024, wtap, 0));
      }
      if (!FUSE1 && tap == PF_TAP && more) load_patch(chunk_i + 1);
      read_group(bf[1], ky, kx, 1, buf);
      if (DB && tap == 8 && more) store_patch(buf ^ 1);
      __builtin_amdgcn_sched_barrier(0);
      mma_group(wf[t & 1], bf[0], 0);
      __builtin_amdgcn_sched_barrier(0);
      if (tap != 8) {
        read_group(bf[0], nky, nkx, 0, buf);
        __builtin_amdgcn_sched_barrier(0);
        mma_group(wf[t & 1], bf[1], 1);
      } else {
        mma_group(wf[t & 1], bf[1], 1);
        if (more) {
          __syncthreads();
          if (FUSE1) {
            make_patch(chunk_i + 1);
            __syncthreads();
          } else if (!DB) {
            if (PF_TAP > 8) load_patch(chunk_i + 1);
            store_patch(0);
            __syncthreads();
          }
        }
        read_group(bf[0], 0, 0, 0, DB ? buf ^ 1 : 0);
      }
      __builtin_amdgcn_sched_barrier(0);
    }
  }
  const bool more_tiles = FUSE1 && strip_i + 1 < strip && tx + strip_i + 1 < tiles_x;
  if (more_tiles) fetch_img(x0 + TW);
  conv_epilogue<MT, NT>(p, acc, b, y0, x0, n0, wm, wn, lane, smem + BIAS_OFF);
  if (more_tiles) {
    ++strip_i;
    x0 += TW;
    goto next_tile;
  }
}

template <int TH, int BN, int WM, int WN, bool FUSE1 = false>
static int launch_conv_cfg(const ConvArgs& a, hipStream_t s) {
  const int tiles_x = cdiv(a.W, TW), tiles_y = cdiv(a.H, TH);
  const int n_tiles = a.Cout / BN;
  constexpr int PH = TH + 2;
  constexpr int NBUF = ((TH / 2) / WM) * ((BN / 32) / WN) > 8 ? 2 : 1;
  const size_t lds = (size_t)NBUF * (PH * PITCH * 64 + 4096) + BN * sizeof(float)
                     + (FUSE1 ? (size_t)(TH + 4) * 20 * 3 * 4 + 64 + 8192 + 256 + 9 * 1024 : 0);
  const long tiles = (long)tiles_x * tiles_y * a.B;
  const int strip = !FUSE1 ? 1 : tiles >= 8192 ? 4 : tiles >= 4096 ? 2 : 1;
  dim3 grid((FUSE1 ? cdiv(tiles_x, strip) : tiles_x) * tiles_y * n_tiles, a.B);
  if (lds > 64 * 1024) {
    static bool raised[16] = {};
    int dev = 0;
    HIP_TRY(hipGetDevice(&dev));
    if (dev >= 0 && dev < 16 && !raised[dev]) {
      HIP_TRY(hipFuncSetAttribute(reinterpret_cast<const void*>(&conv3x3_mfma_kernel<TH, BN, WM, WN, FUSE1>),
                                  hipFuncAttributeMaxDynamicSharedMemorySize, (int)lds));
      raised[dev] = true;
    }
  }
  hipLaunchKernelGGL((conv3x3_mfma_kernel<TH, BN, WM, WN, FUSE1>), grid, dim3(256), lds, s, a, tiles_x, tiles_y, n_tiles, strip);
  HIP_TRY(hipGetLastError());
  return WCT_OK;
}

int launch_conv3x3(const ConvArgs& a, hipStream_t s) {
  ARG_CHECK(a.Cin % 64 == 0 && a.Cout % 64 == 0 && a.H > 1 && a.W > 1 && a.B > 0);
  ARG_CHECK(!a.upsample || (a.H % 2 == 0 && a.W % 2 == 0));
  ARG_CHECK(launch_map_fits((size_t)a.H * a.W * a.Cin, 2));
  ARG_CHECK(launch_map_fits((size_t)a.H * a.W * a.Cout, a.y32 ? 4 : 2));
  ARG_CHECK(!a.usum || (a.y32 && a.umax && a.relu && a.W % 16 == 0));
  ARG_CHECK(!a.pool || (a.relu && !a.y32));
  if (conv3x3_wino_takes(a)) return launch_conv3x3_wino(a, s);
  if (a.img1) {
    ARG_CHECK(a.Cin == 64 && a.Cout == 64 && !a.upsample && a.w1frag && a.bias1);
    return launch_conv_cfg<32, 64, 4, 1, true>(a, s);
  }
  const long px16 = (long)cdiv(a.W, TW) * cdiv(a.H, 16) * a.B;
  const long px32 = (long)cdiv(a.W, TW) * cdiv(a.H, 32) * a.B;
  if (a.Cout % 128 == 0 && px16 * (a.Cout / 128) >= 512) return launch_conv_cfg<16, 128, 2, 2>(a, s);
  if (px32 * (a.Cout / 64) >= 512) return launch_conv_cfg<32, 64, 4, 1>(a, s);
  if (a.Cout % 128 == 0 && px16 * (a.Cout / 128) >= 256) return launch_conv_cfg<16, 128, 2, 2>(a, s);
  if (px16 * (a.Cout / 64) >= 256) return launch_conv_cfg<16, 64, 4, 1>(a, s);
  return launch_conv_cfg<8, 64, 2, 2>(a, s);
}

__global__ __launch_bounds__(256) void conv_first_kernel(ConvFirstArgs p, int strips_x) {
  constexpr int CF_TILES = 4, PATCH_N = 18 * 18 * 3, PER = (PATCH_N + 255) / 256;
  __shared__ float patch[PATCH_N + 4];
  __shared__ __attribute__((aligned(16))) unsigned char tr[4][32 * 256];
  typedef unsigned int u32x4 __attribute__((ext_vector_type(4)));
  const int tid = threadIdx.x, lane = tid & 63, wave = tid >> 6;
  const int sx = blockIdx.x % strips_x, ty = blockIdx.x / strips_x;
  const int b = blockIdx.y;
  const int y0 = ty * 16;
  const float* xb = p.x + (size_t)b * p.H * p.W * 3;
  int e_row[PER], e_px[PER], e_c[PER];
#pragma unroll
  for (int i = 0; i < PER; ++i) {
    const int e = tid + i * 256;
    const int pix = e < PATCH_N ? e / 3 : 0;
    e_c[i] = e < PATCH_N ? e - pix * 3 : 0;
    const int py = pix / 18;
    e_px[i] = pix - py * 18;
    e_row[i] = reflect_idx(y0 - 1 + py, p.H) * p.W;
  }
  float pre[PER];
  auto fetch = [&](int x0) {
#pragma unroll
    for (int i = 0; i < PER; ++i) {
      float v = xb[((size_t)e_row[i] + reflect_idx(x0 - 1 + e_px[i], p.W)) * 3 + e_c[i]];
      pre[i] = p.clamp01 ? fminf(fmaxf(v, 0.f), 1.f) : v;
    }
  };
  auto park = [&]() {
#pragma unroll
    for (int i = 0; i < PER; ++i) if (tid + i * 256 < PATCH_N) patch[tid + i * 256] = pre[i];
  };
  if (tid < 4) patch[PATCH_N + tid] = 0.f;
  fetch(sx * CF_TILES * 16);
  half8 wh[2][2], wl[2][2];
#pragma unroll
  for (int t = 0; t < 2; ++t)
#pragma unroll
    for (int ks = 0; ks < 2; ++ks) {
      wh[t][ks] = *reinterpret_cast<const half8*>(p.wfrag + (((t * 2 + ks) * 2 + 0) * 64 + lane) * 8);
      wl[t][ks] = *reinterpret_cast<const half8*>(p.wfrag + (((t * 2 + ks) * 2 + 1) * 64 + lane) * 8);
    }
  const int frag_px = lane & 15, frag_py = (lane & 31) >> 4, kgrp = lane >> 5;
  int addr[2][8];
#pragma unroll
  for (int ks = 0; ks < 2; ++ks)
#pragma unroll
    for (int j = 0; j < 8; ++j) {
      const int k = ks * 16 + kgrp * 8 + j;
      const int ky = k / 9, kp = k - ky * 9;
      addr[ks][j] = k < 27 ? (((wave * 4 + frag_py + ky) * 18 + frag_px) * 3 + kp) * 4 : 972 * 4;
    }
  f32x4 bias[2][4];
#pragma unroll
  for (int nt = 0; nt < 2; ++nt)
#pragma unroll
    for (int rq = 0; rq < 4; ++rq) bias[nt][rq] = *reinterpret_cast<const f32x4*>(p.bias + nt * 32 + 8 * rq + 4 * kgrp);
  park();
  __syncthreads();
  const unsigned char* pb = reinterpret_cast<const unsigned char*>(patch);
  unsigned char* const wt = tr[wave];
  float vmax = 0.f;
  for (int tile = 0; tile < CF_TILES; ++tile) {
  const int x0 = (sx * CF_TILES + tile) * 16;
  if (x0 >= p.W) break;
  const bool next = tile + 1 < CF_TILES && x0 + 16 < p.W;
  if (next) fetch(x0 + 16);
#pragma unroll
  for (int mt = 0; mt < 2; ++mt) {
    f32x16 acc[2];
#pragma unroll
    for (int nt = 0; nt < 2; ++nt)
#pragma unroll
      for (int r = 0; r < 16; ++r) acc[nt][r] = 0.f;
#pragma unroll
    for (int ks = 0; ks < 2; ++ks) {
      half8 bh, bl;
#pragma unroll
      for (int j = 0; j < 8; ++j) {
        const int off = (ks * 16 + kgrp * 8 + j < 27) ? mt * 2 * 54 * 4 : 0;
        const float v = *reinterpret_cast<const float*>(pb + addr[ks][j] + off);
        bh[j] = (half_t)v;
        bl[j] = (half_t)(v - (float)bh[j]);
      }
#pragma unroll
      for (int nt = 0; nt < 2; ++nt) {
        acc[nt] = __builtin_amdgcn_mfma_f32_32x32x16_f16(wl[nt][ks], bh, acc[nt], 0, 0, 0);
        acc[nt] = __builtin_amdgcn_mfma_f32_32x32x16_f16(wh[nt][ks], bl, acc[nt], 0, 0, 0);
        acc[nt] = __builtin_amdgcn_mfma_f32_32x32x16_f16(wh[nt][ks], bh, acc[nt], 0, 0, 0);
      }
    }
    const int px = lane & 31;
#pragma unroll
    for (int nt = 0; nt < 2; ++nt)
#pragma unroll
      for (int rq = 0; rq < 4; ++rq) {
        f32x4 v;
#pragma unroll
        for (int j = 0; j < 4; ++j) v[j] = fmaxf(acc[nt][rq * 4 + j] + bias[nt][rq][j], 0.f);
        const int piece = nt * 8 + 2 * rq + kgrp;
        *reinterpret_cast<f32x4*>(wt + (px * 16 + (piece ^ (px & 15))) * 16) = v;
        if (p.usum) {
          f32x4 t = v;
          unit_row_sum4(t);
          const int sy = y0 + wave * 4 + mt * 2 + frag_py;
          if (sy < p.H) {
            vmax = fmaxf(fmaxf(vmax, fmaxf(v[0], v[1])), fmaxf(v[2], v[3]));
            if (frag_px == 0)
              *reinterpret_cast<f32x4*>(p.usum + ((size_t)b * (p.H * (p.W >> 4)) + sy * (p.W >> 4) + (x0 >> 4)) * 64 + piece * 4) = t;
          }
        }
      }
    __builtin_amdgcn_fence(__ATOMIC_RELEASE, "wavefront");
    __builtin_amdgcn_wave_barrier();
    const int oy0 = y0 + wave * 4 + mt * 2;
    if (p.y32) {
      const int piece = lane & 15;
#pragma unroll
      for (int it = 0; it < 8; ++it) {
        const int q = it * 4 + (lane >> 4);
        const int oy = oy0 + (q >> 4), ox = x0 + (q & 15);
        const f32x4 v = *reinterpret_cast<const f32x4*>(wt + (q * 16 + (piece ^ (q & 15))) * 16);
        if (oy < p.H && ox < p.W) *reinterpret_cast<f32x4*>(p.y32 + (((size_t)b * p.H + oy) * p.W + ox) * 64 + piece * 4) = v;
      }
    }
    if (p.y16) {
      const int c8 = lane & 7;
#pragma unroll
      for (int it = 0; it < 4; ++it) {
        const int q = it * 8 + (lane >> 3);
        const int oy = oy0 + (q >> 4), ox = x0 + (q & 15);
        const f32x4 v0 = *reinterpret_cast<const f32x4*>(wt + (q * 16 + ((2 * c8) ^ (q & 15))) * 16);
        const f32x4 v1 = *reinterpret_cast<const f32x4*>(wt + (q * 16 + ((2 * c8 + 1) ^ (q & 15))) * 16);
        half8 h;
#pragma unroll
        for (int j = 0; j < 4; ++j) { h[j] = (half_t)v0[j]; h[4 + j] = (half_t)v1[j]; }
        if (oy < p.H && ox < p.W) *reinterpret_cast<half8*>(p.y16 + (((size_t)b * p.H + oy) * p.W + ox) * 64 + c8 * 8) = h;
      }
    }
    __builtin_amdgcn_fence(__ATOMIC_RELEASE, "wavefront");
    __builtin_amdgcn_wave_barrier();
  }
  if (next) {
    __syncthreads();
    park();
    __syncthreads();
  }
  }
  if (p.usum) umax_merge(p.umax + b * UMAX_SLOTS, (int)blockIdx.x * 4 + wave, vmax, lane);
}

int launch_conv_first(const ConvFirstArgs& a, hipStream_t s) {
  ARG_CHECK(a.H > 1 && a.W > 1 && a.B > 0);
  ARG_CHECK(!a.usum || (a.y32 && a.umax && a.W % 16 == 0));
  const int strips_x = cdiv(a.W, 64), tiles_y = cdiv(a.H, 16);
  hipLaunchKernelGGL(conv_first_kernel, dim3(strips_x * tiles_y, a.B), dim3(256), 0, s, a, strips_x);
  HIP_TRY(hipGetLastError());
  return WCT_OK;
}

__global__ __launch_bounds__(256) void conv_last_kernel(ConvLastArgs p, int tiles_x) {
  constexpr int PP = 33;
  __shared__ float part[18 * 18 * PP];
  const int tid = threadIdx.x, lane = tid & 63, wave = tid >> 6;
  const int tx = blockIdx.x % tiles_x, ty = blockIdx.x / tiles_x;
  const int b = blockIdx.y;
  const int y0 = ty * 16, x0 = tx * 16;
  const half_t* xb = p.x + (size_t)b * p.H * p.W * 64;
  half8 wf[4];
#pragma unroll
  for (int ks = 0; ks < 4; ++ks) wf[ks] = *reinterpret_cast<const half8*>(p.wfrag + (ks * 64 + lane) * 8);
  half8 bf[3][4];
  int qs[3];
#pragma unroll
  for (int i = 0; i < 3; ++i) {
    const int tile = wave + 4 * i;
    const int q = tile * 32 + (lane & 31);
    qs[i] = q;
    const int qq = q < 324 ? q : 323;
    const int py = qq / 18, px = qq - py * 18;
    const int iy = reflect_idx(y0 - 1 + py, p.H), ix = reflect_idx(x0 - 1 + px, p.W);
    const half_t* src = xb + ((size_t)iy * p.W + ix) * 64 + (lane >> 5) * 8;
    if (tile < 11) {
#pragma unroll
      for (int ks = 0; ks < 4; ++ks) bf[i][ks] = *reinterpret_cast<const half8*>(src + ks * 16);
    }
  }
#pragma unroll
  for (int i = 0; i < 3; ++i) {
    if (wave + 4 * i >= 11) break;
    f32x16 acc;
#pragma unroll
    for (int r = 0; r < 16; ++r) acc[r] = 0.f;
#pragma unroll
    for (int ks = 0; ks < 4; ++ks) acc = __builtin_amdgcn_mfma_f32_32x32x16_f16(wf[ks], bf[i][ks], acc, 0, 0, 0);
    if (qs[i] < 324) {
#pragma unroll
      for (int r = 0; r < 16; ++r)
        part[qs[i] * PP + (r & 3) + 8 * (r >> 2) + 4 * (lane >> 5)] = acc[r];
    }
  }
  __syncthreads();
  const int ly = tid >> 4, lx = tid & 15;
  const int oy = y0 + ly, ox = x0 + lx;
  float a0 = p.bias[0], a1 = p.bias[1], a2 = p.bias[2];
#pragma unroll
  for (int tap = 0; tap < 9; ++tap) {
    const int ky = tap / 3, kx = tap - ky * 3;
    const float* pq = part + ((ly + ky) * 18 + lx + kx) * PP + tap * 3;
    a0 += pq[0]; a1 += pq[1]; a2 += pq[2];
  }
  if (oy < p.H && ox < p.W) {
    float* o = p.y + (((size_t)b * p.H + oy) * p.W + ox) * 3;
    o[0] = a0; o[1] = a1; o[2] = a2;
  }
}

int launch_conv_last(const ConvLastArgs& a, hipStream_t s) {
  ARG_CHECK(a.H > 1 && a.W > 1 && a.B > 0);
  const int tiles_x = cdiv(a.W, 16), tiles_y = cdiv(a.H, 16);
  hipLaunchKernelGGL(conv_last_kernel, dim3(tiles_x * tiles_y, a.B), dim3(256), 0, s, a, tiles_x);
  HIP_TRY(hipGetLastError());
  return WCT_OK;
}

__global__ void maxpool_kernel(const half_t* x, half_t* y, int B, int H, int W, int C, int Ho, int Wo) {
  const int c8 = C / 8;
  size_t total = (size_t)B * Ho * Wo * c8;
  for (size_t i = blockIdx.x * (size_t)blockDim.x + threadIdx.x; i < total; i += (size_t)gridDim.x * blockDim.x) {
    int c = (int)(i % c8);
    size_t t = i / c8;
    int ox = (int)(t % Wo); t /= Wo;
    int oy = (int)(t % Ho);
    int b = (int)(t / Ho);
    const half_t* xb = x + (size_t)b * H * W * C;
    int iy = oy * 2, ix = ox * 2;
    half8 m = *reinterpret_cast<const half8*>(xb + ((size_t)iy * W + ix) * C + c * 8);
    if (ix + 1 < W) m = __builtin_elementwise_max(m, *reinterpret_cast<const half8*>(xb + ((size_t)iy * W + ix + 1) * C + c * 8));
    if (iy + 1 < H) {
      m = __builtin_elementwise_max(m, *reinterpret_cast<const half8*>(xb + ((size_t)(iy + 1) * W + ix) * C + c * 8));
      if (ix + 1 < W) m = __builtin_elementwise_max(m, *reinterpret_cast<const half8*>(xb + ((size_t)(iy + 1) * W + ix + 1) * C + c * 8));
    }
    *reinterpret_cast<half8*>(y + i * 8) = m;
  }
}

int launch_maxpool2x2(const half_t* x, half_t* y, int B, int H, int W, int C, hipStream_t s) {
  ARG_CHECK(C % 8 == 0);
  const int Ho = (H + 1) / 2, Wo = (W + 1) / 2;
  size_t total = (size_t)B * Ho * Wo * (C / 8);
  int blocks = (int)((total + 255) / 256);
  if (blocks > 4096) blocks = 4096;
  hipLaunchKernelGGL(maxpool_kernel, dim3(blocks), dim3(256), 0, s, x, y, B, H, W, C, Ho, Wo);
  HIP_TRY(hipGetLastError());
  return WCT_OK;
}

__global__ void u8_to_f32_kernel(const uint8_t* x, float* y, size_t n) {
  for (size_t i = blockIdx.x * (size_t)blockDim.x + threadIdx.x; i < n; i += (size_t)gridDim.x * blockDim.x)
    y[i] = (float)((double)x[i] / 255.0);
}
__global__ void f32_to_u8_kernel(const float* x, uint8_t* y, size_t n) {
  for (size_t i = blockIdx.x * (size_t)blockDim.x + threadIdx.x; i < n; i += (size_t)gridDim.x * blockDim.x) {
    float v = fminf(fmaxf(x[i], 0.f), 1.f) * 255.f;
    y[i] = (uint8_t)v;
  }
}
__global__ void f32_to_f16_kernel(const float* x, half_t* y, size_t n) {
  for (size_t i = blockIdx.x * (size_t)blockDim.x + threadIdx.x; i < n; i += (size_t)gridDim.x * blockDim.x) y[i] = (half_t)x[i];
}
__global__ void f16_to_f32_kernel(const half_t* x, float* y, size_t n) {
  for (size_t i = blockIdx.x * (size_t)blockDim.x + threadIdx.x; i < n; i += (size_t)gridDim.x * blockDim.x) y[i] = (float)x[i];
}

static inline int ew_blocks(size_t n) {
  size_t b = (n + 255) / 256;
  return (int)(b > 4096 ? 4096 : (b ? b : 1));
}
int launch_u8_to_f32(const uint8_t* x, float* y, size_t n, hipStream_t s) {
  hipLaunchKernelGGL(u8_to_f32_kernel, dim3(ew_blocks(n)), dim3(256), 0, s, x, y, n);
  HIP_TRY(hipGetLastError());
  return WCT_OK;
}
int launch_f32_to_u8(const float* x, uint8_t* y, size_t n, hipStream_t s) {
  hipLaunchKernelGGL(f32_to_u8_kernel, dim3(ew_blocks(n)), dim3(256), 0, s, x, y, n);
  HIP_TRY(hipGetLastError());
  return WCT_OK;
}
int launch_f32_to_f16(const float* x, half_t* y, size_t n, hipStream_t s) {
  hipLaunchKernelGGL(f32_to_f16_kernel, dim3(ew_blocks(n)), dim3(256), 0, s, x, y, n);
  HIP_TRY(hipGetLastError());
  return WCT_OK;
}
int launch_f16_to_f32(const half_t* x, float* y, size_t n, hipStream_t s) {
  hipLaunchKernelGGL(f16_to_f32_kernel, dim3(ew_blocks(n)), dim3(256), 0, s, x, y, n);
  HIP_TRY(hipGetLastError());
  return WCT_OK;
}
```

wct_tf_amd/csrc/stats_gemm.hip:

```cpp
#include "wct_stages.h"


struct StatArgs {
  const float* x[2];
  int n[2];
  const float* u[2];
  const unsigned* umax[2];
  const float* mean;
  float* partial;
  float* absmax;
  int C, nslab;
  WctSkip skip;
};

__global__ __launch_bounds__(256) void colsum_kernel(StatArgs p) {
  __shared__ f32x4 red[256];
  const int mat = blockIdx.y, slab = blockIdx.x;
  if (skip_style_mat(mat, p.skip)) return;
  const int b = mat & 1, pair = mat >> 1;
  const int C = p.C, cq = C / 4;
  const int nrp = 256 / cq;
  const int tid = threadIdx.x;
  const int rp = tid / cq, c4 = tid % cq;
  const int N = p.n[b];
  const float* x = p.x[b] + (size_t)pair * N * C;
  f32x4 acc = {0.f, 0.f, 0.f, 0.f};
  float amax = 0.f;
  if (p.mean) {
    const int rows_per_slab = (N + p.nslab - 1) / p.nslab;
    const int r0 = slab * rows_per_slab;
    const int r1 = min(N, r0 + rows_per_slab);
    const f32x4 m = *reinterpret_cast<const f32x4*>(p.mean + mat * C + c4 * 4);
    if (rp < nrp)
      for (int r = r0 + rp; r < r1; r += nrp) {
        f32x4 v = *reinterpret_cast<const f32x4*>(x + (size_t)r * C + c4 * 4);
        v -= m; acc += v * v;
      }
  } else {
    const int units = (N + 15) >> 4;
    const int ups = (units + p.nslab - 1) / p.nslab;
    const int u0 = slab * ups, u1 = min(units, u0 + ups);
    const float* U = p.u[b] ? p.u[b] + (size_t)pair * units * C : nullptr;
    if (rp < nrp)
      for (int u = u0 + rp; u < u1; u += nrp) {
        if (U) {
          acc += *reinterpret_cast<const f32x4*>(U + (size_t)u * C + c4 * 4);
        } else {
          f32x4 t[16];
#pragma unroll
          for (int i = 0; i < 16; ++i) {
            const int r = u * 16 + i;
            t[i] = *reinterpret_cast<const f32x4*>(x + (size_t)min(r, N - 1) * C + c4 * 4);
            if (r >= N) t[i] = f32x4{0.f, 0.f, 0.f, 0.f};
            amax = fmaxf(fmaxf(amax, fmaxf(fabsf(t[i][0]), fabsf(t[i][1]))), fmaxf(fabsf(t[i][2]), fabsf(t[i][3])));
          }
#pragma unroll
          for (int w = 1; w < 16; w <<= 1)
#pragma unroll
            for (int i = 0; i < 16; i += 2 * w) t[i] += t[i + w];
          acc += t[0];
        }
      }
    if (U) amax = __builtin_bit_cast(float, p.umax[b][pair * UMAX_SLOTS + (tid & (UMAX_SLOTS - 1))]);
  }
  red[tid] = acc;
  __syncthreads();
  if (rp == 0) {
    for (int j = 1; j < nrp; ++j) acc += red[j * cq + c4];
    *reinterpret_cast<f32x4*>(p.partial + ((size_t)mat * p.nslab + slab) * C + c4 * 4) = acc;
  }
  if (p.absmax) {
    __syncthreads();
    float* redf = reinterpret_cast<float*>(red);
    redf[tid] = amax;
    __syncthreads();
    for (int st = 128; st > 0; st >>= 1) {
      if (tid < st) redf[tid] = fmaxf(redf[tid], redf[tid + st]);
      __syncthreads();
    }
    if (tid == 0) p.absmax[(size_t)mat * p.nslab + slab] = redf[0];
  }
}

__global__ void colsum_finish_kernel(const float* partial, float* out, int C, int nslab, float d0, float d1, int skip,
                                     const float* absmax = nullptr, float* scale = nullptr) {
  const int mat = blockIdx.y;
  if (skip_style_mat(mat, skip)) return;
  if (scale && blockIdx.x == 0 && threadIdx.x < 64) {
    float m = 0.f;
    for (int i = threadIdx.x; i < nslab; i += 64) m = fmaxf(m, absmax[(size_t)mat * nslab + i]);
    for (int o = 32; o > 0; o >>= 1) m = fmaxf(m, __shfl_xor(m, o, 64));
    if (threadIdx.x == 0) {
      float sc = 1.f;
      if (m > 0.f && m < 1e30f) {
        int e;
        frexpf(2.f * m, &e);
        sc = ldexpf(1.f, 14 - e);
      }
      scale[mat] = sc;
    }
  }
  const int c = blockIdx.x * blockDim.x + threadIdx.x;
  if (c >= C) return;
  float a[8] = {0.f, 0.f, 0.f, 0.f, 0.f, 0.f, 0.f, 0.f};
  const float* pp = partial + (size_t)mat * nslab * C + c;
  int i = 0;
  for (; i + 8 <= nslab; i += 8) {
#pragma unroll
    for (int j = 0; j < 8; ++j) a[j] += pp[(size_t)(i + j) * C];
  }
  for (; i < nslab; ++i) a[i & 7] += pp[(size_t)i * C];
  const float s = ((a[0] + a[1]) + (a[2] + a[3])) + ((a[4] + a[5]) + (a[6] + a[7]));
  out[mat * C + c] = s / ((mat & 1) == 0 ? d0 : d1);
}

constexpr int GK = 16;

template <int BX>
struct GemmStage {
  static constexpr int NV = GK * BX / 4 / 256;
  f32x4 v[NV];
  __device__ __forceinline__ void load(const float* src, int ld, bool kmajor, int k0, int kend, int x0, int X,
                                       const float* sub_x, const float* sub_k, const float* scale_k, int tid) {
#pragma unroll
    for (int i = 0; i < NV; ++i) {
      const int item = tid + i * 256;
      f32x4 t = {0.f, 0.f, 0.f, 0.f};
      if (kmajor) {
        const int k = item / (BX / 4), x4 = item % (BX / 4);
        const int gk = k0 + k, gx = x0 + x4 * 4;
        if (gk < kend && gx < X) {
          t = *reinterpret_cast<const f32x4*>(src + (size_t)gk * ld + gx);
          if (sub_x) t -= *reinterpret_cast<const f32x4*>(sub_x + gx);
        }
      } else {
        const int x = item / (GK / 4), k4 = item % (GK / 4);
        const int gx = x0 + x, gk = k0 + k4 * 4;
        if (gx < X && gk < kend) {
          t = *reinterpret_cast<const f32x4*>(src + (size_t)gx * ld + gk);
          if (sub_k) t -= *reinterpret_cast<const f32x4*>(sub_k + gk);
          if (scale_k) t *= *reinterpret_cast<const f32x4*>(scale_k + gk);
        }
      }
      v[i] = t;
    }
  }
  __device__ __forceinline__ void store(float* lds , bool kmajor, int tid) const {
    constexpr int P = BX + 4;
#pragma unroll
    for (int i = 0; i < NV; ++i) {
      const int item = tid + i * 256;
      if (kmajor) {
        const int k = item / (BX / 4), x4 = item % (BX / 4);
        *reinterpret_cast<f32x4*>(lds + k * P + x4 * 4) = v[i];
      } else {
        const int x = item / (GK / 4), k4 = item % (GK / 4);
#pragma unroll
        for (int j = 0; j < 4; ++j) lds[(k4 * 4 + j) * P + x] = v[i][j];
      }
    }
  }
};

constexpr float REFRESH_RATIO = 1e-4f;
__device__ __forceinline__ bool refresh_needed(const float* Am, int C, int tid) {
  float dmax = 0.f, dmin = 3.0e38f;
  for (int i = tid; i < C; i += 256) {
    const float d = Am[(size_t)i * C + i];
    dmax = fmaxf(dmax, fabsf(d));
    if (d > 3.3e-6f) dmin = fminf(dmin, d);
  }
  for (int o = 32; o > 0; o >>= 1) { dmax = fmaxf(dmax, __shfl_xor(dmax, o, 64)); dmin = fminf(dmin, __shfl_xor(dmin, o, 64)); }
  __shared__ float red[2][4];
  if ((tid & 63) == 0) { red[0][tid >> 6] = dmax; red[1][tid >> 6] = dmin; }
  __syncthreads();
  dmax = fmaxf(fmaxf(red[0][0], red[0][1]), fmaxf(red[0][2], red[0][3]));
  dmin = fminf(fminf(red[1][0], red[1][1]), fminf(red[1][2], red[1][3]));
  return dmin < 3.0e38f && dmin < REFRESH_RATIO * dmax;
}

template <int BM, int BN>
__global__ __launch_bounds__(256, 4) void gemm_f32_kernel(GemmArgs p) {
  constexpr int TM = BM / 64, TN = BN / 64;
  constexpr int PA = BM + 4, PB = BN + 4;
  __shared__ __attribute__((aligned(16))) float As[GK * PA];
  __shared__ __attribute__((aligned(16))) float Bs[GK * PB];
  const int tid = threadIdx.x, lane = tid & 63, wave = tid >> 6;
  const int wm = wave >> 1, wn = wave & 1;
  const int m0 = blockIdx.y * BM, n0 = blockIdx.x * BN;
  const int batch = blockIdx.z / p.nsplit, split = blockIdx.z % p.nsplit;
  if (p.skip != WCT_SKIP_NONE && skip_style_mat(batch, p.skip)) return;
  if (p.mask_in && !p.mask_in[batch]) return;
  if (p.mask_diag) {
    const bool need = refresh_needed(p.mask_diag + batch * p.s_mask, p.M, tid);
    if (p.mask_out && blockIdx.x == 0 && blockIdx.y == 0 && split == 0 && tid == 0) p.mask_out[batch] = need ? 1 : 0;
    if (!need) return;
  }
  const int kbeg = split * p.ksplit;
  const int kend = min(p.K, kbeg + p.ksplit);
  if (p.A_odd) p.A = (batch & 1) ? p.A_odd + (batch >> 1) * p.sA_odd : p.A + (batch >> 1) * p.sA;
  else p.A += batch * p.sA;
  p.B += batch * p.sB;
  if (p.a_sub_m) p.a_sub_m += batch * p.s_sub_m;
  if (p.b_sub_n) p.b_sub_n += batch * p.s_sub_n;
  if (p.a_sub_k) p.a_sub_k += batch * p.s_sub_k;
  if (p.a_scale_k) p.a_scale_k += batch * p.s_scale_k;
  if (p.bias_n) p.bias_n += batch * p.s_bias;

  f32x16 acc[TM][TN];
#pragma unroll
  for (int i = 0; i < TM; ++i)
#pragma unroll
    for (int j = 0; j < TN; ++j)
#pragma unroll
      for (int r = 0; r < 16; ++r) acc[i][j][r] = 0.f;

  GemmStage<BM> sa;
  GemmStage<BN> sb;
  if (kbeg < kend) {
    sa.load(p.A, p.lda, p.a_kmajor, kbeg, kend, m0, p.M, p.a_sub_m, p.a_sub_k, p.a_scale_k, tid);
    sb.load(p.B, p.ldb, p.b_kmajor, kbeg, kend, n0, p.N, p.b_sub_n, nullptr, nullptr, tid);
  }
  for (int k0 = kbeg; k0 < kend; k0 += GK) {
    sa.store(As, p.a_kmajor, tid);
    sb.store(Bs, p.b_kmajor, tid);
    __syncthreads();
    if (k0 + GK < kend) {
      sa.load(p.A, p.lda, p.a_kmajor, k0 + GK, kend, m0, p.M, p.a_sub_m, p.a_sub_k, p.a_scale_k, tid);
      sb.load(p.B, p.ldb, p.b_kmajor, k0 + GK, kend, n0, p.N, p.b_sub_n, nullptr, nullptr, tid);
    }
#pragma unroll
    for (int kk = 0; kk < GK; kk += 2) {
      float a[TM], b[TN];
      const int kr = kk + (lane >> 5);
#pragma unroll
      for (int i = 0; i < TM; ++i) a[i] = As[kr * PA + (wm * TM + i) * 32 + (lane & 31)];
#pragma unroll
      for (int j = 0; j < TN; ++j) b[j] = Bs[kr * PB + (wn * TN + j) * 32 + (lane & 31)];
#pragma unroll
      for (int i = 0; i < TM; ++i)
#pragma unroll
        for (int j = 0; j < TN; ++j)
          acc[i][j] = __builtin_amdgcn_mfma_f32_32x32x2f32(a[i], b[j], acc[i][j], 0, 0, 0);
    }
    __syncthreads();
  }

  float* o32 = p.out32 ? p.out32 + batch * p.s_out + (size_t)split * p.out_split_stride : nullptr;
  half_t* o16 = p.out16 ? p.out16 + batch * p.s_out : nullptr;
  float biasv[TN];
#pragma unroll
  for (int j = 0; j < TN; ++j) {
    const int gn = n0 + (wn * TN + j) * 32 + (lane & 31);
    biasv[j] = (p.bias_n && gn < p.N) ? p.bias_n[gn] : 0.f;
  }
#pragma unroll
  for (int j = 0; j < TN; ++j) asm volatile("" : "+v"(biasv[j]));
  float av = 0.f;
#pragma unroll
  for (int i = 0; i < TM; ++i)
#pragma unroll
    for (int j = 0; j < TN; ++j) {
      const int gn = n0 + (wn * TN + j) * 32 + (lane & 31);
      const float bias = biasv[j];
#pragma unroll
      for (int r = 0; r < 16; ++r) {
        const int gm = m0 + (wm * TM + i) * 32 + (r & 3) + 8 * (r >> 2) + 4 * (lane >> 5);
        if (gm < p.M && gn < p.N) {
          float v = acc[i][j][r] + bias;
          if (p.blend) {
            v = p.alpha * acc[i][j][r];
            if (gm == gn) v += 1.f - p.alpha;
            av = fmaxf(av, fabsf(v));
          }
          if (o32) o32[(size_t)gm * p.ldo + gn] = v;
          if (o16) o16[(size_t)gm * p.ldo + gn] = (half_t)v;
        }
      }
    }
  if (p.blend) {
    for (int o = 32; o > 0; o >>= 1) av = fmaxf(av, __shfl_xor(av, o, 64));
    if (lane == 0 && av < 1e30f) atomicMax(p.mabs + batch, __float_as_uint(av));
  }
}

int launch_gemm(GemmArgs g, int nsplit, int nbatch, hipStream_t s) {
  g.nsplit = nsplit;
  const int gz = nsplit * nbatch;
  const bool small_grid = (long)cdiv(g.M, 128) * cdiv(g.N, 128) * gz < 256;
  if (g.M >= 128 && g.N >= 128 && !small_grid) {
    dim3 grid(cdiv(g.N, 128), cdiv(g.M, 128), gz);
    hipLaunchKernelGGL((gemm_f32_kernel<128, 128>), grid, dim3(256), 0, s, g);
  } else if (g.M >= 128 && !small_grid) {
    dim3 grid(cdiv(g.N, 64), cdiv(g.M, 128), gz);
    hipLaunchKernelGGL((gemm_f32_kernel<128, 64>), grid, dim3(256), 0, s, g);
  } else {
    dim3 grid(cdiv(g.N, 64), cdiv(g.M, 64), gz);
    hipLaunchKernelGGL((gemm_f32_kernel<64, 64>), grid, dim3(256), 0, s, g);
  }
  HIP_TRY(hipGetLastError());
  return WCT_OK;
}

struct CovArgs {
  const float* x[2];
  int n[2];
  const float* mean;
  const float* scale;
  float* partial;
  int C, ksplit, nsplit, ntile;
  WctSkip skip;
};

template <int BT>
__global__ __launch_bounds__(256, 2) void cov_f16x2_kernel(CovArgs p) {
  constexpr int TM = BT / 64;
  constexpr int KPT = BT * 32 / 256;
  constexpr int NPC = KPT / 8;
  __shared__ __attribute__((aligned(16))) unsigned char lds[4][BT * 64];
  const int tid = threadIdx.x, lane = tid & 63, wave = tid >> 6;
  const int wm = wave >> 1, wn = wave & 1;
  int ti = 0, rem = blockIdx.x;
  while (rem >= p.ntile - ti) { rem -= p.ntile - ti; ++ti; }
  const int tj = ti + rem;
  const bool diag = ti == tj;
  const int m0 = ti * BT, n0 = tj * BT;
  const int mat = blockIdx.z, split = blockIdx.y;
  if (skip_style_mat(mat, p.skip)) return;
  const int side = mat & 1, pair = mat >> 1;
  const int N = p.n[side], C = p.C;
  const float* x = p.x[side] + (size_t)pair * N * C;
  const int kbeg = split * p.ksplit;
  const int kend = min(N, kbeg + p.ksplit);
  const float sc = p.scale[mat];

  const int c = tid % BT;
  const int kg = __builtin_amdgcn_readfirstlane(tid / BT);
  const float mean_a = p.mean[mat * C + min(m0 + c, C - 1)];
  const float mean_b = p.mean[mat * C + min(n0 + c, C - 1)];
  const __amdgpu_buffer_rsrc_t rsrc = __builtin_amdgcn_make_buffer_rsrc((void*)x, 0, (int)((size_t)N * C * 4), 0x00020000);
  const int voff_a = min(m0 + c, C - 1) * 4, voff_b = min(n0 + c, C - 1) * 4;

  f32x16 acc[TM][TM];
#pragma unroll
  for (int i = 0; i < TM; ++i)
#pragma unroll
    for (int j = 0; j < TM; ++j)
#pragma unroll
      for (int r = 0; r < 16; ++r) acc[i][j][r] = 0.f;

  auto load = [&](float (&r)[KPT], int voff, int k0) {
#pragma unroll
    for (int j = 0; j < KPT; ++j)
      r[j] = __builtin_bit_cast(float, __builtin_amdgcn_raw_buffer_load_b32(rsrc, voff, (k0 + kg * KPT + j) * C * 4, 0));
  };
  auto split_store = [&](const float (&r)[KPT], float mean, int k0, bool tail, unsigned char* hi, unsigned char* lo) {
#pragma unroll
    for (int q = 0; q < NPC; ++q) {
      half8 h, l;
#pragma unroll
      for (int j = 0; j < 8; ++j) {
        const float s_in = (!tail || k0 + kg * KPT + q * 8 + j < kend) ? sc : 0.f;
        const float v = (r[q * 8 + j] - mean) * s_in;
        h[j] = (half_t)v;
        l[j] = (half_t)(v - (float)h[j]);
      }
      const int chunk = kg * NPC + q;
      const int off = (c * 4 + (chunk ^ ((c >> 2) & 3))) * 16;
      *reinterpret_cast<half8*>(hi + off) = h;
      *reinterpret_cast<half8*>(lo + off) = l;
    }
  };
  auto mma_stage = [&](const unsigned char* bh, const unsigned char* bl) {
#pragma unroll
    for (int ks = 0; ks < 2; ++ks) {
      const int chunk = ks * 2 + (lane >> 5);
      half8 ah[TM], al[TM], bhf[TM], blf[TM];
#pragma unroll
      for (int i = 0; i < TM; ++i) {
        const int r = (wm * TM + i) * 32 + (lane & 31);
        const int off = (r * 4 + (chunk ^ ((r >> 2) & 3))) * 16;
        ah[i] = *reinterpret_cast<const half8*>(lds[0] + off);
        al[i] = *reinterpret_cast<const half8*>(lds[1] + off);
      }
#pragma unroll
      for (int j = 0; j < TM; ++j) {
        const int r = (wn * TM + j) * 32 + (lane & 31);
        const int off = (r * 4 + (chunk ^ ((r >> 2) & 3))) * 16;
        bhf[j] = *reinterpret_cast<const half8*>(bh + off);
        blf[j] = *reinterpret_cast<const half8*>(bl + off);
      }
#pragma unroll
      for (int i = 0; i < TM; ++i)
#pragma unroll
        for (int j = 0; j < TM; ++j) {
          acc[i][j] = __builtin_amdgcn_mfma_f32_32x32x16_f16(al[i], bhf[j], acc[i][j], 0, 0, 0);
          acc[i][j] = __builtin_amdgcn_mfma_f32_32x32x16_f16(ah[i], blf[j], acc[i][j], 0, 0, 0);
          acc[i][j] = __builtin_amdgcn_mfma_f32_32x32x16_f16(ah[i], bhf[j], acc[i][j], 0, 0, 0);
        }
    }
  };

  float ra[KPT], rb[KPT];
  if (diag) {
    if (kbeg < kend) load(ra, voff_a, kbeg);
    for (int k0 = kbeg; k0 < kend; k0 += 32) {
      if (k0 + 32 <= kend) split_store(ra, mean_a, k0, false, lds[0], lds[1]);
      else split_store(ra, mean_a, k0, true, lds[0], lds[1]);
      __syncthreads();
      if (k0 + 32 < kend) load(ra, voff_a, k0 + 32);
      mma_stage(lds[0], lds[1]);
      __syncthreads();
    }
  } else {
    if (kbeg < kend) { load(ra, voff_a, kbeg); load(rb, voff_b, kbeg); }
    for (int k0 = kbeg; k0 < kend; k0 += 32) {
      if (k0 + 32 <= kend) {
        split_store(ra, mean_a, k0, false, lds[0], lds[1]);
        split_store(rb, mean_b, k0, false, lds[2], lds[3]);
      } else {
        split_store(ra, mean_a, k0, true, lds[0], lds[1]);
        split_store(rb, mean_b, k0, true, lds[2], lds[3]);
      }
      __syncthreads();
      if (k0 + 32 < kend) { load(ra, voff_a, k0 + 32); load(rb, voff_b, k0 + 32); }
      mma_stage(lds[2], lds[3]);
      __syncthreads();
    }
  }

  float* out = p.partial + ((size_t)mat * p.nsplit + split) * C * C;
#pragma unroll
  for (int i = 0; i < TM; ++i)
#pragma unroll
    for (int j = 0; j < TM; ++j) {
      const int gn = n0 + (wn * TM + j) * 32 + (lane & 31);
#pragma unroll
      for (int r = 0; r < 16; ++r) {
        const int gm = m0 + (wm * TM + i) * 32 + (r & 3) + 8 * (r >> 2) + 4 * (lane >> 5);
        if (gm < C && gn < C) out[(size_t)gm * C + gn] = acc[i][j][r];
      }
    }
}

__global__ __launch_bounds__(256) void cov_finish_kernel(const float* partial, const float* scale, float* cov, int C, int nsplit, int BT,
                                                         float inv0, float inv1, float eps, int skip, float* cov0 = nullptr) {
  __shared__ float tt[64][65];
  const int mat = blockIdx.z;
  if (skip_style_mat(mat, skip)) return;
  const size_t cc = (size_t)C * C;
  const int r0 = blockIdx.y * 64, c0 = blockIdx.x * 64, tid = threadIdx.x, ty = tid >> 4, tx = tid & 15;
  const bool mirror = r0 / BT > c0 / BT;
  const float* pb = partial + (size_t)mat * nsplit * cc;
  const float sc = scale[mat];
  const float f = ((mat & 1) == 0 ? inv0 : inv1) / (sc * sc);
  f32x4 acc[4];
#pragma unroll
  for (int i = 0; i < 4; ++i) {
    const int r = (mirror ? c0 : r0) + ty * 4 + i, c = (mirror ? r0 : c0) + tx * 4;
    f32x4 sum = {0.f, 0.f, 0.f, 0.f};
    if (r < C && c < C)
      for (int k = 0; k < nsplit; ++k) sum += *reinterpret_cast<const f32x4*>(pb + (size_t)k * cc + (size_t)r * C + c);
    acc[i] = sum;
  }
  if (mirror) {
#pragma unroll
    for (int i = 0; i < 4; ++i)
#pragma unroll
      for (int j = 0; j < 4; ++j) tt[ty * 4 + i][tx * 4 + j] = acc[i][j];
    __syncthreads();
#pragma unroll
    for (int i = 0; i < 4; ++i)
#pragma unroll
      for (int j = 0; j < 4; ++j) acc[i][j] = tt[tx * 4 + j][ty * 4 + i];
  }
#pragma unroll
  for (int i = 0; i < 4; ++i) {
    const int r = r0 + ty * 4 + i, c = c0 + tx * 4;
    if (r >= C || c >= C) continue;
    f32x4 v = acc[i] * f;
#pragma unroll
    for (int j = 0; j < 4; ++j) if (r == c + j) v[j] += eps;
    *reinterpret_cast<f32x4*>(cov + (size_t)mat * cc + (size_t)r * C + c) = v;
    if (cov0) *reinterpret_cast<f32x4*>(cov0 + (size_t)mat * cc + (size_t)r * C + c) = v;
  }
}

static int stat_passes(StatArgs sa, int nmat, float* mean, float* var, float* scale, float d0, float d1, hipStream_t s) {
  const int C = sa.C;
  sa.mean = nullptr;
  hipLaunchKernelGGL(colsum_kernel, dim3(sa.nslab, nmat), dim3(256), 0, s, sa);
  hipLaunchKernelGGL(colsum_finish_kernel, dim3(cdiv(C, 256), nmat), dim3(256), 0, s, sa.partial, mean, C, sa.nslab, d0, d1, (int)sa.skip,
                     (const float*)sa.absmax, scale);
  if (var) {
    sa.mean = mean; sa.absmax = nullptr;
    hipLaunchKernelGGL(colsum_kernel, dim3(sa.nslab, nmat), dim3(256), 0, s, sa);
    hipLaunchKernelGGL(colsum_finish_kernel, dim3(cdiv(C, 256), nmat), dim3(256), 0, s, sa.partial, var, C, sa.nslab, d0, d1, (int)sa.skip,
                       (const float*)nullptr, (float*)nullptr);
  }
  HIP_TRY(hipGetLastError());
  return WCT_OK;
}

int launch_means(const float* content, int Nc, const float* style, int Ns, int C, int P, const WctCarve& w, bool with_var, WctSkip skip,
                 hipStream_t s, const WctFeatStats* fs) {
  StatArgs sa;
  sa.x[0] = content; sa.x[1] = style; sa.n[0] = Nc; sa.n[1] = Ns;
  for (int b = 0; b < 2; ++b) {
    sa.u[b] = fs && fs->umax[b] ? fs->u[b] : nullptr;
    sa.umax[b] = sa.u[b] ? fs->umax[b] : nullptr;
  }
  sa.partial = w.stat_partial; sa.absmax = w.absmax; sa.C = C; sa.nslab = w.nslab; sa.skip = skip;
  return stat_passes(sa, 2 * P, w.mean, with_var ? w.var : nullptr, w.scale, (float)Nc, (float)Ns, s);
}

static int cov_passes(CovArgs ca, int nmat, float* A, float* A0, float inv0, float inv1, float eps, hipStream_t s) {
  const int C = ca.C, BT = C >= 128 ? 128 : 64;
  ca.ntile = cdiv(C, BT);
  dim3 grid(ca.ntile * (ca.ntile + 1) / 2, ca.nsplit, nmat);
  if (BT == 128) hipLaunchKernelGGL((cov_f16x2_kernel<128>), grid, dim3(256), 0, s, ca);
  else hipLaunchKernelGGL((cov_f16x2_kernel<64>), grid, dim3(256), 0, s, ca);
  hipLaunchKernelGGL(cov_finish_kernel, dim3(cdiv(C, 64), cdiv(C, 64), nmat), dim3(256), 0, s, ca.partial, ca.scale, A, C, ca.nsplit, BT,
                     inv0, inv1, eps, (int)ca.skip, A0);
  HIP_TRY(hipGetLastError());
  return WCT_OK;
}

int launch_cov(const float* content, int Nc, const float* style, int Ns, int C, int P, const WctCarve& w, float eps, WctSkip skip,
               hipStream_t s) {
  CovArgs ca;
  ca.x[0] = content; ca.x[1] = style; ca.n[0] = Nc; ca.n[1] = Ns;
  ca.mean = w.mean; ca.scale = w.scale; ca.partial = w.cov_partial;
  ca.C = C; ca.ksplit = w.ksplit; ca.nsplit = w.nsplit; ca.skip = skip;
  return cov_passes(ca, 2 * P, w.A, w.A0, 1.f / (float)(Nc - 1), 1.f / (float)(Ns - 1), eps, s);
}

static int launch_slot_means(const float* x, int N, int C, int m, int nslab, const WctCarve& w, bool with_var, hipStream_t s,
                             const float* u, const unsigned* umax) {
  StatArgs sa = {};
  sa.x[0] = sa.x[1] = x; sa.n[0] = sa.n[1] = N;
  sa.u[0] = umax ? u : nullptr; sa.umax[0] = sa.u[0] ? umax : nullptr;
  sa.partial = w.stat_partial + (size_t)m * w.nslab * C; sa.absmax = w.absmax + (size_t)m * w.nslab;
  sa.C = C; sa.nslab = nslab; sa.skip = WCT_SKIP_NONE;
  return stat_passes(sa, 1, w.mean + (size_t)m * C, with_var ? w.var + (size_t)m * C : nullptr, w.scale + m, (float)N, (float)N, s);
}

static int launch_slot_cov(const float* x, int N, int C, int m, int nsplit, int ksplit, float eps, const WctCarve& w, hipStream_t s) {
  const size_t cc = (size_t)C * C;
  CovArgs ca;
  ca.x[0] = ca.x[1] = x; ca.n[0] = ca.n[1] = N;
  ca.mean = w.mean + (size_t)m * C; ca.scale = w.scale + m; ca.partial = w.cov_partial + (size_t)m * w.nsplit * cc;
  ca.C = C; ca.ksplit = ksplit; ca.nsplit = nsplit; ca.skip = WCT_SKIP_NONE;
  return cov_passes(ca, 1, w.A + m * cc, w.A0 + m * cc, 1.f / (float)(N - 1), 1.f / (float)(N - 1), eps, s);
}

int launch_plan_stats(const SlotPlan& sp, int C, bool with_var, bool with_cov, float eps, hipStream_t s) {
  int rc;
  for (int m = 0; m < 2 * sp.P; ++m) {
    const SlotPlan::Slot& t = sp.slot[m];
    if (!t.n) continue;
    if ((rc = launch_slot_means(t.x, t.n, C, m, t.lay.nslab, sp.w, with_var, s, m ? nullptr : sp.u0, m ? nullptr : sp.umax0))) return rc;
    if (with_cov && (rc = launch_slot_cov(t.x, t.n, C, m, t.lay.nsplit, t.lay.ksplit, eps, sp.w, s))) return rc;
  }
  return WCT_OK;
}
```

wct_tf_amd/csrc/wct.hip:

```cpp
#include "wct_stages.h"
#include "jacobi_dev.h"
#include "strength_rule.h"
#include <algorithm>
#include <type_traits>



template <int BC, int BP, typename Args = ApplyArgs>
__global__ __launch_bounds__(256, 2) void apply_f16x2_kernel(Args p) {
  constexpr bool SEGB = std::is_same<Args, ApplySegBatchArgs>::value;
  constexpr bool SEG = std::is_same<Args, ApplySegArgs>::value || SEGB;
  constexpr bool MAP = std::is_same<Args, ApplyMapArgs>::value;
  constexpr int TM = BC / 64, TN = BP / 64;
  constexpr int MI = BC * 4 / 256, XI = BP * 4 / 256;
  __shared__ __attribute__((aligned(16))) unsigned char lm[2][BC * 64];
  __shared__ __attribute__((aligned(16))) unsigned char lx[2][BP * 64];
  typedef unsigned int u32x4 __attribute__((ext_vector_type(4)));
  const int tid = threadIdx.x, lane = tid & 63, wave = tid >> 6;
  const int wm = wave >> 1, wn = wave & 1;
  const int pair = blockIdx.z;
  const int n0 = blockIdx.x * BP, c0 = blockIdx.y * BC;
  int seg0 = 0, N = p.N;
  [[maybe_unused]] int row0 = 0;
  if constexpr (SEGB) {
    const int f = seg_frame(p.fl[pair]), lab = seg_label(p.fl[pair]);
    const int first = p.seg_off[f * (WCT_MIX_MAX + 1) + lab];
    N = p.seg_off[f * (WCT_MIX_MAX + 1) + lab + 1] - first;
    if (n0 >= N) return;
    row0 = f * p.N;
    seg0 = row0 + first;
  } else if constexpr (SEG) {
    seg0 = p.seg_off[p.lab[pair]];
    N = p.seg_off[p.lab[pair] + 1] - seg0;
    if (n0 >= N) return;
  }
  const int C = p.C;
  const float* x = p.x + (SEG ? (size_t)seg0 * C : (size_t)pair * N * C);
  const float* M = p.M + (size_t)pair * C * C;
  const float* mean = p.mean + (size_t)pair * 2 * C;
  const float sx = p.xscale[2 * pair];
  float sM = 1.f;
  {
    const float m = __uint_as_float(p.mabs[pair]);
    if (m > 0.f) { int e; frexpf(m, &e); sM = ldexpf(1.f, 14 - e); }
  }

  const float* mp[MI]; const float* xp[XI];
  int moff[MI], xoff[XI], xk[XI];
#pragma unroll
  for (int i = 0; i < MI; ++i) {
    const int item = tid + i * 256, row = item >> 2, kq = item & 3;
    mp[i] = M + (size_t)min(c0 + row, C - 1) * C + kq * 8;
    moff[i] = (row * 4 + (kq ^ ((row >> 2) & 3))) * 16;
  }
#pragma unroll
  for (int i = 0; i < XI; ++i) {
    const int item = tid + i * 256, row = item >> 2, kq = item & 3;
    xp[i] = x + (size_t)min(n0 + row, N - 1) * C + kq * 8;
    xoff[i] = (row * 4 + (kq ^ ((row >> 2) & 3))) * 16;
    xk[i] = kq * 8;
  }

  f32x16 acc[TM][TN];
#pragma unroll
  for (int i = 0; i < TM; ++i)
#pragma unroll
    for (int j = 0; j < TN; ++j)
#pragma unroll
      for (int r = 0; r < 16; ++r) acc[i][j][r] = 0.f;

  f32x4 rm[MI][2], rx[XI][2];
  auto load = [&](int k0) {
#pragma unroll
    for (int i = 0; i < MI; ++i) {
      rm[i][0] = *reinterpret_cast<const f32x4*>(mp[i] + k0);
      rm[i][1] = *reinterpret_cast<const f32x4*>(mp[i] + k0 + 4);
    }
#pragma unroll
    for (int i = 0; i < XI; ++i) {
      rx[i][0] = *reinterpret_cast<const f32x4*>(xp[i] + k0) - *reinterpret_cast<const f32x4*>(mean + k0 + xk[i]);
      rx[i][1] = *reinterpret_cast<const f32x4*>(xp[i] + k0 + 4) - *reinterpret_cast<const f32x4*>(mean + k0 + xk[i] + 4);
    }
  };
  auto split_store = [&](const f32x4 (&r)[2], float sc, unsigned char* hi, unsigned char* lo, int off) {
    half8 h, l;
#pragma unroll
    for (int j = 0; j < 8; ++j) {
      const float v = r[j >> 2][j & 3] * sc;
      h[j] = (half_t)v;
      l[j] = (half_t)(v - (float)h[j]);
    }
    *reinterpret_cast<half8*>(hi + off) = h;
    *reinterpret_cast<half8*>(lo + off) = l;
  };

  load(0);
  for (int k0 = 0; k0 < C; k0 += 32) {
#pragma unroll
    for (int i = 0; i < MI; ++i) split_store(rm[i], sM, lm[0], lm[1], moff[i]);
#pragma unroll
    for (int i = 0; i < XI; ++i) split_store(rx[i], sx, lx[0], lx[1], xoff[i]);
    __syncthreads();
    if (k0 + 32 < C) load(k0 + 32);
#pragma unroll
    for (int ks = 0; ks < 2; ++ks) {
      const int chunk = ks * 2 + (lane >> 5);
      half8 ah[TM], al[TM], bh[TN], bl[TN];
#pragma unroll
      for (int i = 0; i < TM; ++i) {
        const int r = (wm * TM + i) * 32 + (lane & 31);
        const int off = (r * 4 + (chunk ^ ((r >> 2) & 3))) * 16;
        ah[i] = *reinterpret_cast<const half8*>(lm[0] + off);
        al[i] = *reinterpret_cast<const half8*>(lm[1] + off);
      }
#pragma unroll
      for (int j = 0; j < TN; ++j) {
        const int r = (wn * TN + j) * 32 + (lane & 31);
        const int off = (r * 4 + (chunk ^ ((r >> 2) & 3))) * 16;
        bh[j] = *reinterpret_cast<const half8*>(lx[0] + off);
        bl[j] = *reinterpret_cast<const half8*>(lx[1] + off);
      }
#pragma unroll
      for (int i = 0; i < TM; ++i)
#pragma unroll
        for (int j = 0; j < TN; ++j) {
          acc[i][j] = __builtin_amdgcn_mfma_f32_32x32x16_f16(al[i], bh[j], acc[i][j], 0, 0, 0);
          acc[i][j] = __builtin_amdgcn_mfma_f32_32x32x16_f16(ah[i], bl[j], acc[i][j], 0, 0, 0);
          acc[i][j] = __builtin_amdgcn_mfma_f32_32x32x16_f16(ah[i], bh[j], acc[i][j], 0, 0, 0);
        }
    }
    __syncthreads();
  }

  const float inv = 1.f / (sx * sM);
  const float* bias = p.bias + (size_t)pair * C;
  const int kgrp = lane >> 5;
  f32x4 bvs[TM][4];
#pragma unroll
  for (int i = 0; i < TM; ++i)
#pragma unroll
    for (int rq = 0; rq < 4; ++rq) {
      const int co = c0 + (wm * TM + i) * 32 + 8 * rq + 4 * kgrp;
      const f32x4 z = {0.f, 0.f, 0.f, 0.f};
      bvs[i][rq] = co < C ? *reinterpret_cast<const f32x4*>(bias + co) : z;
    }
  int dst[TN];
  if constexpr (SEG)
#pragma unroll
    for (int j = 0; j < TN; ++j) {
      const int n = n0 + (wn * TN + j) * 32 + (lane & 31);
      dst[j] = p.perm[seg0 + (n < N ? n : 0)];
      if constexpr (SEGB) dst[j] += row0;
    }
  [[maybe_unused]] float amap[TN];
  [[maybe_unused]] f32x4 xv[TN][TM][4];
  if constexpr (MAP)
#pragma unroll
    for (int j = 0; j < TN; ++j) {
      const int n = n0 + (wn * TN + j) * 32 + (lane & 31), nc = n < N ? n : 0;
      const uint8_t* sm = p.smap + (size_t)pair * p.Hm * p.Wm;
      amap[j] = wct_strength_a(p.alpha, sm[wct_strength_index(nc / p.w, nc % p.w, p.stride, p.Hm, p.Wm)]);
#pragma unroll
      for (int i = 0; i < TM; ++i)
#pragma unroll
        for (int rq = 0; rq < 4; ++rq) {
          const int co = c0 + (wm * TM + i) * 32 + 8 * rq + 4 * kgrp;
          const f32x4 z = {0.f, 0.f, 0.f, 0.f};
          xv[j][i][rq] = co < C ? *reinterpret_cast<const f32x4*>(x + (size_t)nc * C + co) : z;
        }
    }
#pragma unroll
  for (int j = 0; j < TN; ++j) {
    const int n = n0 + (wn * TN + j) * 32 + (lane & 31);
    const bool n_ok = n < N;
    const size_t row = SEG ? (size_t)dst[j] * C : ((size_t)pair * N + (n_ok ? n : 0)) * C;
#pragma unroll
    for (int i = 0; i < TM; ++i) {
      const int cb = c0 + (wm * TM + i) * 32;
      unsigned pk[4][2];
#pragma unroll
      for (int rq = 0; rq < 4; ++rq) {
        const int co = cb + 8 * rq + 4 * kgrp;
        const f32x4 bv = bvs[i][rq];
        f32x4 v;
#pragma unroll
        for (int q = 0; q < 4; ++q) v[q] = acc[i][j][rq * 4 + q] * inv + bv[q];
        if constexpr (MAP)
#pragma unroll
          for (int q = 0; q < 4; ++q) v[q] = wct_strength_blend(amap[j], v[q], xv[j][i][rq][q]);
        if (p.out32 && n_ok && co < C) *reinterpret_cast<f32x4*>(p.out32 + row + co) = v;
        typedef _Float16 h2 __attribute__((ext_vector_type(2)));
        h2 lo = {(half_t)v[0], (half_t)v[1]}, hi = {(half_t)v[2], (half_t)v[3]};
        pk[rq][0] = __builtin_bit_cast(unsigned, lo);
        pk[rq][1] = __builtin_bit_cast(unsigned, hi);
      }
      if (p.out16) {
#pragma unroll
        for (int m = 0; m < 2; ++m) {
          auto sxw = __builtin_amdgcn_permlane32_swap(pk[2 * m][0], pk[2 * m + 1][0], false, false);
          auto syw = __builtin_amdgcn_permlane32_swap(pk[2 * m][1], pk[2 * m + 1][1], false, false);
          u32x4 o = {sxw[0], syw[0], sxw[1], syw[1]};
          const int co = cb + 16 * m + 8 * kgrp;
          if (n_ok && co < C) *reinterpret_cast<u32x4*>(p.out16 + row + co) = o;
        }
      }
    }
  }
}

template <typename Args>
int launch_apply_args(const Args& a, int nmax, int P, hipStream_t s) {
  const int C = a.C;
  if (C >= 128) hipLaunchKernelGGL((apply_f16x2_kernel<128, 128, Args>), dim3(cdiv(nmax, 128), cdiv(C, 128), P), dim3(256), 0, s, a);
  else hipLaunchKernelGGL((apply_f16x2_kernel<64, 128, Args>), dim3(cdiv(nmax, 128), cdiv(C, 64), P), dim3(256), 0, s, a);
  HIP_TRY(hipGetLastError());
  return WCT_OK;
}
template int launch_apply_args<ApplySegArgs>(const ApplySegArgs&, int, int, hipStream_t);
template int launch_apply_args<ApplySegBatchArgs>(const ApplySegBatchArgs&, int, int, hipStream_t);
template int launch_apply_args<ApplyMapArgs>(const ApplyMapArgs&, int, int, hipStream_t);

static int wct_nslab(int N) { int s = cdiv(N, 64); return s < 1 ? 1 : (s > 256 ? 256 : s); }

static void cov_split(int C, int Nmax, int P, int* nsplit, int* ksplit) {
  const int nt = C >= 128 ? cdiv(C, 128) : 1;
  const int tiles = nt * (nt + 1) / 2 * P;
  int want = 32 / tiles;
  if (want < 1) want = 1;
  int ks = cdiv(cdiv(Nmax, want), 32) * 32;
  if (ks < 256) ks = 256;
  *ksplit = ks;
  *nsplit = cdiv(Nmax, ks);
}

PairLayout pair_layout(int C, int Nc, int Ns) {
  PairLayout L;
  const int Nmax = Nc > Ns ? Nc : Ns;
  L.nslab = wct_nslab(Nmax);
  cov_split(C, Nmax, 1, &L.nsplit, &L.ksplit);
  return L;
}

WctCarve carve(void* base, int C, int P, const PairLayout& lay) {
  WctCarve w;
  w.nslab = lay.nslab; w.nsplit = lay.nsplit; w.ksplit = lay.ksplit;
  size_t off = 0;
  char* b = reinterpret_cast<char*>(base);
  auto take = [&](size_t bytes) { void* p = b ? b + off : nullptr; off += align_up(bytes); return p; };
  const size_t cc = (size_t)C * C * sizeof(float);
  w.mean = (float*)take((size_t)2 * P * C * sizeof(float));
  w.var = (float*)take((size_t)2 * P * C * sizeof(float));
  w.stat_partial = (float*)take((size_t)2 * P * w.nslab * C * sizeof(float));
  w.absmax = (float*)take((size_t)2 * P * w.nslab * sizeof(float));
  w.scale = (float*)take((size_t)2 * P * sizeof(float));
  w.cov_partial = (float*)take((size_t)2 * P * w.nsplit * cc);
  w.A = (float*)take(2 * P * cc);
  w.A0 = (float*)take(2 * P * cc);
  w.refresh = (int*)take((size_t)2 * P * sizeof(int));
  w.V = (float*)take(2 * P * cc);
  w.d = (float*)take((size_t)2 * P * C * sizeof(float));
  w.G = (float*)take(2 * P * cc);
  w.X = (float*)take(2 * P * cc);
  w.S2 = (float*)take(7 * P * cc);
  w.Tw = (float*)take(2 * P * cc);
  w.Tcs = w.Tw + (size_t)C * C;
  w.T = (float*)take(P * cc);
  w.M = (float*)take(P * cc);
  w.bias = (float*)take((size_t)P * C * sizeof(float));
  w.mabs = (unsigned*)take((size_t)P * sizeof(unsigned));
  w.jacobi_bytes = jacobi_workspace_bytes(C, 2 * P) + 4 * (1024 + 64 * sizeof(JacobiState));
  w.jacobi_ws = take(w.jacobi_bytes);
  w.mix = (float*)take((size_t)2 * C * sizeof(float));
  w.total = off;
  return w;
}

size_t wct_workspace_bytes(int C, int Nc, int Ns, int P) {
  const int Cw = C < 32 ? 32 : C;
  return carve(nullptr, Cw, P, pair_layout(Cw, Nc, Ns)).total;
}

int launch_blend(const WctCarve& w, int C, int P, float alpha, WctSkip skip, hipStream_t s) {
  const size_t cc = (size_t)C * C;
  GemmArgs g = {};
  g.A = w.Tcs; g.lda = C; g.a_kmajor = 0; g.B = w.Tw; g.ldb = C; g.b_kmajor = 1; g.sA = one_style(skip) ? 0 : 2 * cc; g.sB = 2 * cc;
  g.M = C; g.N = C; g.K = C; g.ksplit = C; g.out32 = w.M; g.ldo = C; g.s_out = cc;
  g.blend = 1; g.alpha = alpha; g.mabs = w.mabs;
  return launch_gemm(g, 1, P, s);
}

int launch_apply(const WctCarve& w, const float* content, int Nc, int C, int P, half_t* out16, float* out32, hipStream_t s) {
  return launch_apply_args(apply_args<ApplyArgs>(w, content, Nc, C, out16, out32), Nc, P, s);
}

static bool strength_ok(const WctStrength& sm, int Nc) {
  return sm.smap && sm.Hm >= 1 && sm.Wm >= 1 && sm.w >= 1 && sm.stride >= 1 && Nc % sm.w == 0;
}

static int launch_blend_apply_map(const WctCarve& w, const float* content, int Nc, int C, int P, WctSkip skip, const WctCall& r,
                                  const WctStrength& sm) {
  int rc;
  if ((rc = launch_blend(w, C, P, 1.f, skip, r.stream))) return rc;
  ApplyMapArgs a = apply_args<ApplyMapArgs>(w, content, Nc, C, r.out16, r.out32);
  a.smap = sm.smap; a.Hm = sm.Hm; a.Wm = sm.Wm; a.w = sm.w; a.stride = sm.stride; a.alpha = r.alpha;
  return launch_apply_args(a, Nc, P, r.stream);
}

static int launch_blend_apply(const WctCarve& w, const float* content, int Nc, int C, int P, WctSkip skip, const WctCall& r) {
  int rc;
  if ((rc = launch_blend(w, C, P, r.alpha, skip, r.stream))) return rc;
  return launch_apply(w, content, Nc, C, P, r.out16, r.out32, r.stream);
}

WctStyleKey wct_style_key(int C, int Nc, int Ns) {
  const PairLayout L = pair_layout(std::max(C, 32), Nc, Ns);
  return WctStyleKey{L.nslab, L.nsplit, L.ksplit};
}
size_t wct_style_state_floats(int C) { return (size_t)2 * C + (size_t)C * C; }

template <typename Ref>
__global__ __launch_bounds__(256) void style_load_kernel(Ref r, float* mean, float* var, float* Tw, int C, int with_T) {
  const int k = blockIdx.y;
  const float* src = r.state[k];
  const size_t cc = (size_t)C * C, n = (size_t)2 * C + (with_T ? cc : 0), slot = (size_t)(2 * k + 1);
  for (size_t i = (blockIdx.x * (size_t)blockDim.x + threadIdx.x) * 4; i < n; i += (size_t)gridDim.x * blockDim.x * 4) {
    const f32x4 v = *reinterpret_cast<const f32x4*>(src + i);
    float* dst = i < (size_t)C ? mean + slot * C + i : (i < (size_t)2 * C ? var + slot * C + (i - C) : Tw + slot * cc + (i - 2 * C));
    *reinterpret_cast<f32x4*>(dst) = v;
  }
}

template <typename Ref>
static int launch_style_load(const Ref& r, int K, const WctCarve& w, int C, bool with_T, hipStream_t s) {
  for (int k = 0; k < K; ++k) ARG_CHECK(r.state[k] != nullptr);
  const size_t n4 = ((size_t)2 * C + (with_T ? (size_t)C * C : 0)) / 4;
  hipLaunchKernelGGL(style_load_kernel<Ref>, dim3((unsigned)std::min<size_t>((n4 + 255) / 256, 256), K), dim3(256), 0, s, r, w.mean, w.var,
                     w.Tw, C, with_T ? 1 : 0);
  HIP_TRY(hipGetLastError());
  return WCT_OK;
}

int launch_style_load_slots(const WctStyleSlots& r, int P, const WctCarve& w, int C, bool with_T, hipStream_t s) {
  ARG_CHECK(P >= 1 && P <= WCT_PLAN_PAIRS);
  return launch_style_load(r, P, w, C, with_T, s);
}

static void style_plan(SlotPlan* sp, void* base, int C, const float* style, int Ns, const WctStyleKey& key) {
  *sp = SlotPlan{};
  sp->P = 1; sp->skip = WCT_SKIP_CONTENT; sp->nwhite = 0;
  sp->slot[1] = {style, Ns, PairLayout{key.nslab, key.nsplit, key.ksplit}};
  plan_carve(sp, base, C);
}

size_t wct_style_workspace_bytes(int C, int Ns, const WctStyleKey& key) {
  SlotPlan sp;
  style_plan(&sp, nullptr, C, nullptr, Ns, key);
  return sp.total;
}

int launch_style_state(const float* style, int Ns, int C, const WctStyleKey& key, int adain, const WctCall& r, float* state) {
  const int mode = r.mode; hipStream_t s = r.stream;
  ARG_CHECK(style && state && C % 32 == 0 && C >= 32 && C <= 1024 && Ns >= (adain ? 1 : 2) && launch_map_fits((size_t)Ns * C, 4));
  ARG_CHECK(adain || mode == WCT_MODE_NP || mode == WCT_MODE_TF);
  ARG_CHECK(key.nslab >= 1 && key.nslab <= 256 && key.nsplit >= 1 && key.ksplit >= 256 && key.ksplit % 32 == 0 &&
            (long long)key.nsplit * key.ksplit >= Ns);
  SlotPlan sp;
  style_plan(&sp, r.workspace, C, style, Ns, key);
  ARG_CHECK(r.workspace_bytes >= sp.total);
  const WctCarve& w = sp.w;
  int rc;
  if (adain) {
    if ((rc = launch_plan_stats(sp, C, true, false, 0.f, s))) return rc;
    HIP_TRY(hipMemcpyAsync(state + C, w.var + C, (size_t)C * sizeof(float), hipMemcpyDeviceToDevice, s));
  } else {
    if ((rc = launch_plan_stats(sp, C, false, true, cov_eps(mode, r.eps), s))) return rc;
    if ((rc = launch_eig_stage(w, C, sp.P, sp.skip, 1, nullptr, r.eig_fail, s))) return rc;
    if ((rc = launch_spectral_tail(w, C, sp.P, 1.f, mode, r.eps, sp.skip, sp.nwhite, s))) return rc;
    HIP_TRY(hipMemcpyAsync(state + 2 * C, w.Tw + (size_t)C * C, (size_t)C * C * sizeof(float), hipMemcpyDeviceToDevice, s));
  }
  HIP_TRY(hipMemcpyAsync(state, w.mean + C, (size_t)C * sizeof(float), hipMemcpyDeviceToDevice, s));
  return WCT_OK;
}

int launch_wct(const float* content, int Nc, const float* style, int Ns, int C, int P, WctSkip skip, const WctCall& r,
               const WctFeatStats* stats, const WctStyleRef* prep, const WctWarmRef* warm, const WctStrength* sm) {
  const int mode = r.mode, stages = r.stages; hipStream_t s = r.stream;
  ARG_CHECK(C % 32 == 0 && C >= 32 && C <= 1024 && Nc >= 2 && Ns >= 2 && P >= 1 && P <= 32);
  ARG_CHECK(!sm || strength_ok(*sm, Nc));
  ARG_CHECK(skip == WCT_SKIP_NONE || skip == WCT_SKIP_SHARED_STYLE);
  ARG_CHECK(!warm || (warm->basis && (skip == WCT_SKIP_NONE || prep)));
  if (prep) skip = WCT_SKIP_STYLE;
  ARG_CHECK(mode == WCT_MODE_NP || mode == WCT_MODE_TF);
  ARG_CHECK(launch_map_fits((size_t)Nc * C, 4) && launch_map_fits((size_t)Ns * C, 4));
  WctCarve w = carve(r.workspace, C, P, pair_layout(C, Nc, Ns));
  ARG_CHECK(r.workspace_bytes >= w.total);
  int rc;
  if (stages & WCT_STAGE_COV) {
    if ((rc = launch_means(content, Nc, style, Ns, C, P, w, false, skip, s, stats))) return rc;
    if ((rc = launch_cov(content, Nc, style, Ns, C, P, w, cov_eps(mode, r.eps), skip, s))) return rc;
  }
  if (stages & WCT_STAGE_EIG) {
    const bool rotate = warm && warm->valid;
    if (rotate && (rc = launch_warm_rotate(w, C, P, warm->basis, s))) return rc;
    if ((rc = launch_eig_stage(w, C, P, skip, (stages & WCT_STAGE_EIG_FP32UPDATE) ? 0 : 1, r.sweeps_dev, r.eig_fail, s, rotate ? 0 : 2)))
      return rc;
    if (rotate && (rc = launch_warm_compose(w, C, P, warm->basis, s))) return rc;
    if (warm && (rc = launch_warm_store(w.V + (size_t)2 * (P - 1) * C * C, w.X, warm->basis, C, s))) return rc;
  }
  if (!(stages & WCT_STAGE_APPLY)) return WCT_OK;

  if (prep && (rc = launch_style_load(*prep, 1, w, C, true, s))) return rc;
  if ((rc = launch_spectral_tail(w, C, P, sm ? 1.f : r.alpha, mode, r.eps, skip, P, s))) return rc;
  if (sm) return launch_blend_apply_map(w, content, Nc, C, P, skip, r, *sm);
  return launch_blend_apply(w, content, Nc, C, P, skip, r);
}

void plan_carve(SlotPlan* sp, void* base, int C) {
  PairLayout mx = {1, 1, 0};
  for (int m = 0; m < 2 * sp->P; ++m)
    if (sp->slot[m].n) { mx.nslab = std::max(mx.nslab, sp->slot[m].lay.nslab); mx.nsplit = std::max(mx.nsplit, sp->slot[m].lay.nsplit); }
  sp->w = carve(base, C, std::max(sp->P, 1), mx);
  sp->total = sp->w.total;
}

bool plan_fits(const SlotPlan& sp, int C) {
  for (int m = 0; m < 2 * sp.P; ++m)
    if (!launch_map_fits((size_t)sp.slot[m].n * C, 4)) return false;
  return true;
}

static bool mix_plan(SlotPlan* sp, void* base, int C, const float* content, int Nc, const float* const* styles, const int* Ns,
                     int K, const float* lambda, int nmin, const WctFeatStats* stats, bool prepared = false) {
  if (!Ns || !lambda || K < 1 || K > WCT_MIX_MAX) return false;
  int ref = 0;
  for (int k = 0; k < K; ++k) {
    if ((styles && !styles[k]) || Ns[k] < nmin || !(lambda[k] >= 0.f && lambda[k] <= 1.f)) return false;
    if (lambda[k] > lambda[ref]) ref = k;
  }
  const int Cw = std::max(C, 32);
  *sp = SlotPlan{};
  sp->P = K; sp->skip = WCT_SKIP_MIX; sp->nwhite = 1;
  if (stats) { sp->u0 = stats->u[0]; sp->umax0 = stats->umax[0]; }
  sp->slot[0] = {content, Nc, pair_layout(Cw, Nc, Ns[ref])};
  for (int k = 0; k < K; ++k) sp->slot[2 * k + 1] = {styles ? styles[k] : nullptr, Ns[k], pair_layout(Cw, Nc, Ns[k])};
  if (prepared) {
    sp->skip = WCT_SKIP_MIX_STYLE;
    for (int k = 0; k < K; ++k) sp->slot[2 * k + 1].n = 0;
  }
  plan_carve(sp, base, Cw);
  return true;
}

size_t wct_mix_workspace_bytes(int C, int Nc, const int* Ns, int K, const float* lambda) {
  SlotPlan sp;
  return mix_plan(&sp, nullptr, C, nullptr, Nc, nullptr, Ns, K, lambda, 1, nullptr) ? sp.total : 0;
}

struct MixWeights { float lambda[WCT_MIX_MAX]; int K; };

__global__ __launch_bounds__(256) void wct_mix_kernel(float* Tw, float* bias, int C, MixWeights mw) {
  const size_t cc = (size_t)C * C, n4 = cc / 4;
  for (size_t i = blockIdx.x * (size_t)blockDim.x + threadIdx.x; i < n4; i += (size_t)gridDim.x * blockDim.x) {
    f32x4 acc = {0.f, 0.f, 0.f, 0.f};
    for (int k = 0; k < mw.K; ++k) {
      const f32x4 t = *reinterpret_cast<const f32x4*>(Tw + (2 * k + 1) * cc + i * 4);
#pragma unroll
      for (int j = 0; j < 4; ++j) acc[j] = fmaf(mw.lambda[k], t[j], acc[j]);
    }
    *reinterpret_cast<f32x4*>(Tw + cc + i * 4) = acc;
  }
  if (blockIdx.x == 0)
    for (int c = threadIdx.x; c < C; c += blockDim.x) {
      float acc = 0.f;
      for (int k = 0; k < mw.K; ++k) acc = fmaf(mw.lambda[k], bias[(size_t)k * C + c], acc);
      bias[c] = acc;
    }
}

int launch_wct_mix(const float* content, int Nc, const float* const* styles, const int* Ns, int K, const float* lambda, int C,
                   const WctCall& r, const WctFeatStats* stats, const WctStyleRef* prep) {
  const int mode = r.mode, stages = r.stages; hipStream_t s = r.stream;
  SlotPlan sp;
  ARG_CHECK(C % 32 == 0 && C >= 32 && C <= 1024 && Nc >= 2 && content && (styles || prep) &&
            mix_plan(&sp, r.workspace, C, content, Nc, prep ? nullptr : styles, Ns, K, lambda, 2, stats, prep != nullptr));
  ARG_CHECK(mode == WCT_MODE_NP || mode == WCT_MODE_TF);
  ARG_CHECK(plan_fits(sp, C));
  ARG_CHECK(r.workspace_bytes >= sp.total);
  const WctCarve& w = sp.w;
  int rc;
  if ((stages & WCT_STAGE_COV) && (rc = launch_plan_stats(sp, C, false, true, cov_eps(mode, r.eps), s))) return rc;
  if ((stages & WCT_STAGE_EIG) && (rc = launch_eig_stage(w, C, sp.P, sp.skip, 1, r.sweeps_dev, r.eig_fail, s))) return rc;
  if (!(stages & WCT_STAGE_APPLY)) return WCT_OK;
  if (prep && (rc = launch_style_load(*prep, K, w, C, true, s))) return rc;
  if ((rc = launch_spectral_tail(w, C, sp.P, r.alpha, mode, r.eps, sp.skip, sp.nwhite, s))) return rc;
  MixWeights mw = {};
  mw.K = K;
  for (int k = 0; k < K; ++k) mw.lambda[k] = lambda[k];
  const size_t n4 = (size_t)C * C / 4;
  hipLaunchKernelGGL(wct_mix_kernel, dim3((unsigned)std::min<size_t>((n4 + 255) / 256, 1024)), dim3(256), 0, s, w.Tw, w.bias, C, mw);
  HIP_TRY(hipGetLastError());
  return launch_blend_apply(w, content, Nc, C, 1, WCT_SKIP_NONE, r);
}

__global__ void adain_apply_kernel(const float* x, size_t n4_per_pair, int C, const float* mean, const float* var,
                                   float alpha, float eps, half_t* out16, float* out32, int style_of_pair0,
                                   const float* mix_mu = nullptr, const float* mix_sd = nullptr) {
  const int pair = blockIdx.y;
  const int cq = C / 4;
  const float* mp = mean + (size_t)pair * 2 * C;
  const float* vp = var + (size_t)pair * 2 * C;
  const float* ms = mix_mu ? mix_mu : mean + (size_t)(style_of_pair0 ? 0 : pair) * 2 * C + C;
  const float* vs = var + (size_t)(style_of_pair0 ? 0 : pair) * 2 * C + C;
  const size_t base = (size_t)pair * n4_per_pair;
  for (size_t i = blockIdx.x * (size_t)blockDim.x + threadIdx.x; i < n4_per_pair; i += (size_t)gridDim.x * blockDim.x) {
    const int c = (int)(i % cq) * 4;
    f32x4 v = *reinterpret_cast<const f32x4*>(x + (base + i) * 4);
    f32x4 o;
#pragma unroll
    for (int j = 0; j < 4; ++j) {
      const float inv = 1.f / sqrtf(vp[c + j] + eps);
      const float sd = mix_sd ? mix_sd[c + j] : sqrtf(vs[c + j]);
      const float y = (v[j] - mp[c + j]) * inv * sd + ms[c + j];
      o[j] = alpha * y + (1.f - alpha) * v[j];
    }
    if (out32) *reinterpret_cast<f32x4*>(out32 + (base + i) * 4) = o;
    if (out16) {
      half4 h;
#pragma unroll
      for (int j = 0; j < 4; ++j) h[j] = (half_t)o[j];
      *reinterpret_cast<half4*>(out16 + (base + i) * 4) = h;
    }
  }
}

__global__ void adain_apply_map_kernel(const float* x, size_t n4_per_pair, int C, const float* mean, const float* var, float eps,
                                       half_t* out16, float* out32, int style_of_pair0, WctStrength m, float alpha) {
  const int pair = blockIdx.y;
  const int cq = C / 4;
  const float* mp = mean + (size_t)pair * 2 * C;
  const float* vp = var + (size_t)pair * 2 * C;
  const float* ms = mean + (size_t)(style_of_pair0 ? 0 : pair) * 2 * C + C;
  const float* vs = var + (size_t)(style_of_pair0 ? 0 : pair) * 2 * C + C;
  const uint8_t* sm = m.smap + (size_t)pair * m.Hm * m.Wm;
  const size_t base = (size_t)pair * n4_per_pair;
  for (size_t i = blockIdx.x * (size_t)blockDim.x + threadIdx.x; i < n4_per_pair; i += (size_t)gridDim.x * blockDim.x) {
    const int c = (int)(i % cq) * 4, n = (int)(i / cq);
    const float a = wct_strength_a(alpha, sm[wct_strength_index(n / m.w, n % m.w, m.stride, m.Hm, m.Wm)]);
    f32x4 v = *reinterpret_cast<const f32x4*>(x + (base + i) * 4);
    f32x4 o;
#pragma unroll
    for (int j = 0; j < 4; ++j) {
      const float inv = 1.f / sqrtf(vp[c + j] + eps);
      const float sd = sqrtf(vs[c + j]);
      const float y = (v[j] - mp[c + j]) * inv * sd + ms[c + j];
      o[j] = wct_strength_blend(a, y, v[j]);
    }
    if (out32) *reinterpret_cast<f32x4*>(out32 + (base + i) * 4) = o;
    if (out16) {
      half4 h;
#pragma unroll
      for (int j = 0; j < 4; ++j) h[j] = (half_t)o[j];
      *reinterpret_cast<half4*>(out16 + (base + i) * 4) = h;
    }
  }
}

int launch_adain(const float* content, int Nc, const float* style, int Ns, int C, int P, WctSkip skip, const WctCall& r,
                 const WctFeatStats* stats, const WctStyleRef* prep, const WctStrength* sm) {
  hipStream_t s = r.stream;
  ARG_CHECK(C % 4 == 0 && C <= 1024 && Nc >= 1 && Ns >= 1 && P >= 1 && P <= 32);
  ARG_CHECK(!sm || strength_ok(*sm, Nc));
  ARG_CHECK(skip == WCT_SKIP_NONE || skip == WCT_SKIP_SHARED_STYLE);
  if (prep) skip = WCT_SKIP_STYLE;
  const int Cw = C < 32 ? 32 : C;
  WctCarve w = carve(r.workspace, Cw, P, pair_layout(Cw, Nc, Ns));
  ARG_CHECK(r.workspace_bytes >= w.total);
  int rc;
  if ((rc = launch_means(content, Nc, style, Ns, C, P, w, true, skip, s, stats))) return rc;
  if (prep && (rc = launch_style_load(*prep, 1, w, C, false, s))) return rc;
  const size_t n4 = (size_t)Nc * C / 4;
  if (sm)
    hipLaunchKernelGGL(adain_apply_map_kernel, dim3(rows_grid(Nc, C), P), dim3(256), 0, s, content, n4, C, w.mean, w.var, r.eps, r.out16,
                       r.out32, one_style(skip) ? 1 : 0, *sm, r.alpha);
  else
  hipLaunchKernelGGL(adain_apply_kernel, dim3(rows_grid(Nc, C), P), dim3(256), 0, s, content, n4, C, w.mean, w.var, r.alpha, r.eps, r.out16, r.out32,
                     one_style(skip) ? 1 : 0);
  HIP_TRY(hipGetLastError());
  return WCT_OK;
}

__global__ void adain_mix_moments_kernel(const float* mean, const float* var, float* mix, int C, MixWeights mw) {
  const int c = blockIdx.x * blockDim.x + threadIdx.x;
  if (c >= C) return;
  float mu = 0.f, sd = 0.f;
  for (int k = 0; k < mw.K; ++k) {
    mu = fmaf(mw.lambda[k], mean[(size_t)(2 * k + 1) * C + c], mu);
    sd = fmaf(mw.lambda[k], sqrtf(var[(size_t)(2 * k + 1) * C + c]), sd);
  }
  mix[c] = mu;
  mix[C + c] = sd;
}

int launch_adain_mix(const float* content, int Nc, const float* const* styles, const int* Ns, int K, const float* lambda, int C,
                     const WctCall& r, const WctFeatStats* stats, const WctStyleRef* prep) {
  hipStream_t s = r.stream;
  SlotPlan sp;
  ARG_CHECK(C % 4 == 0 && C <= 1024 && Nc >= 1 && content && (styles || prep) &&
            mix_plan(&sp, r.workspace, C, content, Nc, prep ? nullptr : styles, Ns, K, lambda, 1, stats, prep != nullptr));
  ARG_CHECK(!prep || C >= 32);
  ARG_CHECK(r.workspace_bytes >= sp.total);
  const WctCarve& w = sp.w;
  int rc;
  if ((rc = launch_plan_stats(sp, C, true, false, 0.f, s))) return rc;
  if (prep && (rc = launch_style_load(*prep, K, w, C, false, s))) return rc;
  MixWeights mw = {};
  mw.K = K;
  for (int k = 0; k < K; ++k) mw.lambda[k] = lambda[k];
  hipLaunchKernelGGL(adain_mix_moments_kernel, dim3(cdiv(C, 256)), dim3(256), 0, s, w.mean, w.var, w.mix, C, mw);
  const size_t n4 = (size_t)Nc * C / 4;
  hipLaunchKernelGGL(adain_apply_kernel, dim3(rows_grid(Nc, C), 1), dim3(256), 0, s, content, n4, C, w.mean, w.var, r.alpha, r.eps, r.out16,
                     r.out32, 0, (const float*)w.mix, (const float*)(w.mix + C));
  HIP_TRY(hipGetLastError());
  return WCT_OK;
}
```

wct_tf_amd/csrc/wct_stages.h:

```cpp
#pragma once
#include "common.h"


constexpr int EIG_CORRECT = 2;
constexpr float JACOBI_TOL_FN = 1.5e-2f;
constexpr float JACOBI_TOL_FN2 = 4e-2f;
constexpr float JACOBI_TOL_FN_WCT = EIG_CORRECT >= 2 ? JACOBI_TOL_FN2 : (EIG_CORRECT ? JACOBI_TOL_FN : 0.f);

static inline size_t align_up(size_t x) { return (x + 255) & ~(size_t)255; }

struct WctCarve {
  float *mean, *var, *stat_partial, *absmax, *scale, *cov_partial, *A, *A0, *V, *d, *G, *X, *S2, *Tw, *Tcs, *T, *M, *bias, *mix;
  unsigned* mabs; int* refresh;
  void* jacobi_ws; size_t jacobi_bytes;
  int nslab, nsplit, ksplit;
  size_t total;
};

struct PairLayout { int nslab, nsplit, ksplit; };
PairLayout pair_layout(int C, int Nc, int Ns);
WctCarve carve(void* base, int C, int P, const PairLayout& lay);

static inline float cov_eps(int mode, float eps_in) {
  return mode == WCT_MODE_TF ? (eps_in >= 0.f ? eps_in : 1e-8f) : 0.f;
}

static inline unsigned rows_grid(size_t N, int C) {
  const size_t blocks = (N * C / 4 + 255) / 256;
  return (unsigned)(blocks > 2048 ? 2048 : blocks);
}

constexpr int WCT_PLAN_PAIRS = 32;
struct SlotPlan {
  int P; WctSkip skip; int nwhite;
  struct Slot { const float* x; int n; PairLayout lay; } slot[2 * WCT_PLAN_PAIRS];
  const float* u0; const unsigned* umax0;
  WctCarve w;
  size_t total;
};
void plan_carve(SlotPlan* sp, void* base, int C);
bool plan_fits(const SlotPlan& sp, int C);

struct ApplyArgs {
  const float* x; int N; int C;
  const float* mean;
  const float* M; const float* bias;
  const float* xscale;
  const unsigned* mabs;
  half_t* out16; float* out32;
};
struct ApplySegArgs : ApplyArgs { const int* seg_off; const int* perm; int lab[WCT_MIX_MAX]; };
struct ApplySegBatchArgs : ApplyArgs { const int* seg_off; const int* perm; unsigned char fl[WCT_PLAN_PAIRS]; };
struct ApplyMapArgs : ApplyArgs { const uint8_t* smap; int Hm, Wm, w, stride; float alpha; };
template <typename Args>
static inline Args apply_args(const WctCarve& w, const float* x, int N, int C, half_t* out16, float* out32) {
  Args a;
  a.x = x; a.N = N; a.C = C; a.mean = w.mean; a.M = w.M; a.bias = w.bias;
  a.xscale = w.scale; a.mabs = w.mabs; a.out16 = out16; a.out32 = out32;
  return a;
}
__device__ __host__ __forceinline__ int seg_frame(unsigned char fl) { return fl >> 3; }
__device__ __host__ __forceinline__ int seg_label(unsigned char fl) { return fl & 7; }

int launch_means(const float* content, int Nc, const float* style, int Ns, int C, int P, const WctCarve& w, bool with_var,
                 WctSkip skip, hipStream_t s, const WctFeatStats* fs);
int launch_cov(const float* content, int Nc, const float* style, int Ns, int C, int P, const WctCarve& w, float eps, WctSkip skip,
               hipStream_t s);
int launch_plan_stats(const SlotPlan& sp, int C, bool with_var, bool with_cov, float eps, hipStream_t s);
int launch_eig_stage(const WctCarve& w, int C, int P, WctSkip skip, int u_f16, int* sweeps_dev, int* eig_fail, hipStream_t s,
                     int check_from = 2);
int launch_spectral_tail(const WctCarve& w, int C, int P, float alpha, int mode, float eps_in, WctSkip skip, int nwhite, hipStream_t s);
int launch_spectral_tail_refreshed(const WctCarve& w, int C, int P, float alpha, int mode, float eps_in, WctSkip skip, int nwhite,
                                   hipStream_t s);
int launch_blend(const WctCarve& w, int C, int P, float alpha, WctSkip skip, hipStream_t s);
int launch_apply(const WctCarve& w, const float* content, int Nc, int C, int P, half_t* out16, float* out32, hipStream_t s);
template <typename Args> int launch_apply_args(const Args& a, int nmax, int P, hipStream_t s);
int launch_warm_rotate(const WctCarve& w, int C, int P, const float* V0, hipStream_t s);
int launch_warm_compose(const WctCarve& w, int C, int P, const float* V0, hipStream_t s);
int launch_warm_store(const float* V, float* scratch, float* basis, int C, hipStream_t s);
int launch_style_load_slots(const WctStyleSlots& r, int P, const WctCarve& w, int C, bool with_T, hipStream_t s);
```

Before: 687.0.

## Recompute relu1_1 features from image inside covariance and apply kernels

Result: faster. 695.0, median of 6 (+1.2%).

```diff
diff --git a/wct_tf_amd/csrc/api.h b/wct_tf_amd/csrc/api.h
--- a/wct_tf_amd/csrc/api.h
+++ b/wct_tf_amd/csrc/api.h
@@ -200,7 +200,8 @@
                   half_t* out16, float* out32, int* sweeps_dev, const WctFeatStats* st = nullptr,
                   const WctStyleRef* prep = nullptr ,
                   const WctWarmRef* warm = nullptr ,
-                  const WctStrength* sm = nullptr );
+                  const WctStrength* sm = nullptr ,
+                  const WctImageSrc* src = nullptr );
 int mix_weights(const float* weights, int K, float* lambda);
 int run_transform_mix(wct_ctx* c, const float* fc, int Nc, const float* const* fs, const int* Ns, int K, const float* lambda, int C,
                       float alpha, unsigned flags, float eps, half_t* out16, float* out32, int* sweeps_dev,
diff --git a/wct_tf_amd/csrc/api_drivers.hip b/wct_tf_amd/csrc/api_drivers.hip
--- a/wct_tf_amd/csrc/api_drivers.hip
+++ b/wct_tf_amd/csrc/api_drivers.hip
@@ -57,15 +57,16 @@
   half_t* cur = (half_t*)c->act[0].p;
   half_t* nxt = (half_t*)c->act[1].p;
   static const int fuse_conv1_env = getenv("WCT_FUSE_CONV1") ? atoi(getenv("WCT_FUSE_CONV1")) : 1;
-  const bool fuse_conv1 = fuse_conv1_env && deepest > 1 && !taps32[1];
+  const bool stats1 = usum && usum[1] && !taps32[1];
+  const bool fuse_conv1 = fuse_conv1_env && deepest > 1 && !taps32[1] && !stats1;
   if (!fuse_conv1) {
     ConvFirstArgs a;
     a.x = img; a.wfrag = c->first_w; a.bias = c->first_b;
     a.y16 = deepest > 1 ? cur : nullptr; a.y32 = taps32[1];
     a.B = B; a.H = H; a.W = W; a.clamp01 = clamp01;
-    a.usum = usum && taps32[1] ? usum[1] : nullptr; a.umax = a.usum ? umax[1] : nullptr;
+    a.usum = usum && (taps32[1] || stats1) ? usum[1] : nullptr; a.umax = a.usum ? umax[1] : nullptr;
     const double px = (double)B * H * W;
-    ProfScope ps(c, 1, 2.0 * px * 27 * 64, px * (12 + 64 * ((a.y16 ? 2 : 0) + (a.y32 ? 4 : 0))));
+    ProfScope ps(c, 1, 2.0 * px * 27 * 64, px * (12 + 64 * ((a.y16 ? 2 : 0) + (a.y32 ? 4 : 0)) + (stats1 ? 64 * 4 / 16.0 : 0)));
     TRY(launch_conv_first(a, c->stream));
   }
   if (deepest == 1) return WCT_OK;
@@ -126,16 +127,19 @@
 
 int run_transform(wct_ctx* c, const float* fc, int Nc, const float* fs, int Ns, int C, int P, float alpha, unsigned flags, float eps,
                   half_t* out16, float* out32, int* sweeps_dev, const WctFeatStats* st, const WctStyleRef* prep, const WctWarmRef* warm,
-                  const WctStrength* sm) {
+                  const WctStrength* sm, const WctImageSrc* src) {
+  ARG_CHECK(!src || !(flags & WCT_FLAG_ADAIN));
   const WctSkip skip = (flags & WCT_FLAG_STYLE_SHARED) ? WCT_SKIP_SHARED_STYLE : WCT_SKIP_NONE;
-  const StageCost cost = {(double)P * 2.0 * C * C * ((double)Nc + Ns), (double)P * 2.0 * ((double)Nc + Ns) * C * 4,
-                          (double)P * (2.0 * C * C * Nc + 6.0 * C * C * C),
+  const StageCost cost = {(double)P * 2.0 * C * (C + (src ? 27 : 0)) * ((double)Nc + Ns),
+                          (double)P * ((double)Nc + Ns) * (src ? 12 + C * 4 / 16.0 : 2.0 * C * 4),
+                          (double)P * (2.0 * C * (C + (src ? 27 : 0)) * Nc + 6.0 * C * C * C),
+                          src ? (double)P * Nc * (12 + C * ((out16 ? 2 : 0) + (out32 ? 4 : 0))) :
                           (double)P * Nc * C * (4 + (out16 ? 2 : 0) + (out32 ? 4 : 0) + (sm ? 4 : 0)) + (sm ? (double)P * Nc : 0.0),
                           (double)P * (2.0 * Nc + 2.0 * Ns) * C * 4 + (double)P * Nc * C * 6 + (sm ? (double)P * Nc : 0.0)};
   return run_stages(c, wct_workspace_bytes(C, Nc, Ns, P), flags, cost, [&](WctCall r) {
     r.alpha = alpha; r.eps = r.stages ? eps : 1e-5f; r.out16 = out16; r.out32 = out32; r.sweeps_dev = sweeps_dev;
     if (!r.stages) return launch_adain(fc, Nc, fs, Ns, C, P, skip, r, st, prep, sm);
-    return launch_wct(fc, Nc, fs, Ns, C, P, skip, r, st, prep, warm, sm);
+    return launch_wct(fc, Nc, fs, Ns, C, P, skip, r, st, prep, warm, sm, src);
   });
 }
 
diff --git a/wct_tf_amd/csrc/api_stylize.hip b/wct_tf_amd/csrc/api_stylize.hip
--- a/wct_tf_amd/csrc/api_stylize.hip
+++ b/wct_tf_amd/csrc/api_stylize.hip
@@ -53,15 +53,19 @@
 
 template <typename StyleAt, typename Transform>
 static int stylize_levels(wct_ctx* c, const float* img_c, const void* content_raw, int B, const Chain& chain, unsigned flags,
-                          size_t umax_clear, int clear_from, StyleAt&& style_at, Transform&& transform, uint8_t* out) {
+                          size_t umax_clear, int clear_from, StyleAt&& style_at, Transform&& transform, uint8_t* out,
+                          bool l1_img = false) {
   unsigned* const umax_c = (unsigned*)c->umax.p;
   const float* cur = img_c;
   for (int i = 0; i < (int)chain.lv.size(); ++i) {
     const ChainLevel& g = chain.lv[i];
     const int l = g.l, C = g.C, h = g.h, w = g.w;
-    TRY(ensure(c, c->feat_c, (size_t)B * h * w * C * 4));
+    const bool from_image = l == 1 && l1_img;
     float* ctaps[6] = {};
-    ctaps[l] = (float*)c->feat_c.p;
+    if (!from_image) {
+      TRY(ensure(c, c->feat_c, (size_t)B * h * w * C * 4));
+      ctaps[l] = (float*)c->feat_c.p;
+    }
     float* us_c[6] = {};
     unsigned* um_c[6] = {};
     if (fuse_stats() && w % 16 == 0) {
@@ -142,6 +146,13 @@
   TRY(ensure(c, c->umax, 7 * UROW * sizeof(unsigned)));
   unsigned* const umax_c = (unsigned*)c->umax.p;
   if (want_stats) HIP_TRY(hipMemsetAsync(c->umax.p, 0, 7 * UROW * sizeof(unsigned), c->stream));
+  static const int l1_env = getenv("WCT_L1_FROM_IMAGE") ? atoi(getenv("WCT_L1_FROM_IMAGE")) : 1;
+  bool l1_img = false;
+  if (l1_env && want_stats && !(flags & WCT_FLAG_ADAIN) && Ws % 16 == 0)
+    for (const ChainLevel& g : chain.lv)
+      if (g.l == 1) l1_img = true;
+  for (const ChainLevel& g : chain.lv)
+    if (g.l == 1 && g.W % 16 != 0) l1_img = false;
   float* taps[6] = {};
   float* us_s[6] = {};
   unsigned* um_s[6] = {};
@@ -149,8 +160,10 @@
     const int l = levels[i];
     int h, w;
     level_dims(Hs, Ws, l, &h, &w);
-    TRY(ensure(c, c->feat_s[l], (size_t)Bs * h * w * LEVEL_C[l] * 4));
-    taps[l] = (float*)c->feat_s[l].p;
+    if (!(l == 1 && l1_img)) {
+      TRY(ensure(c, c->feat_s[l], (size_t)Bs * h * w * LEVEL_C[l] * 4));
+      taps[l] = (float*)c->feat_s[l].p;
+    }
     if (want_stats && w % 16 == 0) {
       TRY(ensure(c, c->usum_s[l], (size_t)Bs * h * (w / 16) * LEVEL_C[l] * 4));
       us_s[l] = (float*)c->usum_s[l].p; um_s[l] = umax_c + UROW * l;
@@ -163,13 +176,19 @@
     return (const float*)c->feat_s[l].p + (size_t)(shared ? 0 : b) * *hs * *ws * LEVEL_C[l];
   };
   return stylize_levels(c, img_c, content, B, chain, flags, UROW * sizeof(unsigned), 1, style_at,
-                        [&](int, const ChainLevel& g, WctFeatStats st) {
+                        [&](int i, const ChainLevel& g, WctFeatStats st) {
                           int hs, ws;
                           const float* fs = style_at(g.l, 0, &hs, &ws);
                           st.u[1] = us_s[g.l]; st.umax[1] = um_s[g.l];
+                          if (g.l == 1 && l1_img) {
+                            const float* in = i == 0 ? img_c : (const float*)c->img_t[(i - 1) & 1].p;
+                            const WctImageSrc src = {{{in, g.H, g.W, i > 0}, {img_s, Hs, Ws, 0}}, c->first_w, c->first_b};
+                            return run_transform(c, nullptr, g.h * g.w, nullptr, hs * ws, g.C, B, alpha, flags, -1.f,
+                                                 (half_t*)c->wct_out.p, nullptr, nullptr, &st, nullptr, nullptr, nullptr, &src);
+                          }
                           return run_transform(c, (float*)c->feat_c.p, g.h * g.w, fs, hs * ws, g.C, B, alpha, flags, -1.f,
                                                (half_t*)c->wct_out.p, nullptr, nullptr, &st);
-                        }, out);
+                        }, out, l1_img);
 }
 
 extern "C" int wct_stylize(wct_ctx* c, const uint8_t* content, int Hc, int Wc, const uint8_t* style, int Hs, int Ws,
diff --git a/wct_tf_amd/csrc/common.h b/wct_tf_amd/csrc/common.h
--- a/wct_tf_amd/csrc/common.h
+++ b/wct_tf_amd/csrc/common.h
@@ -148,6 +148,9 @@
 
 struct WctFeatStats { const float* u[2]; const unsigned* umax[2]; };
 
+struct WctImageSide { const float* img; int H, W, clamp01; };
+struct WctImageSrc { WctImageSide side[2]; const half_t* wfrag; const float* bias; };
+
 struct WctStyleKey { int nslab, nsplit, ksplit; };
 WctStyleKey wct_style_key(int C, int Nc, int Ns);
 size_t wct_style_state_floats(int C);
@@ -175,7 +178,8 @@
 
 size_t wct_workspace_bytes(int C, int Nc, int Ns, int P);
 int launch_wct(const float* content, int Nc, const float* style, int Ns, int C, int P, WctSkip skip, const WctCall& r,
-               const WctFeatStats* stats, const WctStyleRef* prep, const WctWarmRef* warm, const WctStrength* sm = nullptr);
+               const WctFeatStats* stats, const WctStyleRef* prep, const WctWarmRef* warm, const WctStrength* sm = nullptr,
+               const WctImageSrc* src = nullptr );
 int launch_adain(const float* content, int Nc, const float* style, int Ns, int C, int P, WctSkip skip, const WctCall& r,
                  const WctFeatStats* stats, const WctStyleRef* prep, const WctStrength* sm = nullptr);
 enum { WCT_MIX_MAX = 8 };
diff --git a/wct_tf_amd/csrc/conv.hip b/wct_tf_amd/csrc/conv.hip
--- a/wct_tf_amd/csrc/conv.hip
+++ b/wct_tf_amd/csrc/conv.hip
@@ -1,5 +1,6 @@
 #include "common.h"
 #include "conv_tile.h"
+#include "conv_first_tile.h"
 
 
 template <int MT, int NT, bool POOL, bool OUT32>
@@ -455,10 +456,11 @@
   return launch_conv_cfg<8, 64, 2, 2>(a, s);
 }
 
+template <bool STORE>
 __global__ __launch_bounds__(256) void conv_first_kernel(ConvFirstArgs p, int strips_x) {
   constexpr int CF_TILES = 4, PATCH_N = 18 * 18 * 3, PER = (PATCH_N + 255) / 256;
   __shared__ float patch[PATCH_N + 4];
-  __shared__ __attribute__((aligned(16))) unsigned char tr[4][32 * 256];
+  __shared__ __attribute__((aligned(16))) unsigned char tr[4][STORE ? 32 * 256 : 16];
   typedef unsigned int u32x4 __attribute__((ext_vector_type(4)));
   const int tid = threadIdx.x, lane = tid & 63, wave = tid >> 6;
   const int sx = blockIdx.x % strips_x, ty = blockIdx.x / strips_x;
@@ -479,8 +481,7 @@
   auto fetch = [&](int x0) {
 #pragma unroll
     for (int i = 0; i < PER; ++i) {
-      float v = xb[((size_t)e_row[i] + reflect_idx(x0 - 1 + e_px[i], p.W)) * 3 + e_c[i]];
-      pre[i] = p.clamp01 ? fminf(fmaxf(v, 0.f), 1.f) : v;
+      pre[i] = conv1_fetch(xb[((size_t)e_row[i] + reflect_idx(x0 - 1 + e_px[i], p.W)) * 3 + e_c[i]], p.clamp01);
     }
   };
   auto park = [&]() {
@@ -490,13 +491,7 @@
   if (tid < 4) patch[PATCH_N + tid] = 0.f;
   fetch(sx * CF_TILES * 16);
   half8 wh[2][2], wl[2][2];
-#pragma unroll
-  for (int t = 0; t < 2; ++t)
-#pragma unroll
-    for (int ks = 0; ks < 2; ++ks) {
-      wh[t][ks] = *reinterpret_cast<const half8*>(p.wfrag + (((t * 2 + ks) * 2 + 0) * 64 + lane) * 8);
-      wl[t][ks] = *reinterpret_cast<const half8*>(p.wfrag + (((t * 2 + ks) * 2 + 1) * 64 + lane) * 8);
-    }
+  conv1_weights(p.wfrag, lane, wh, wl);
   const int frag_px = lane & 15, frag_py = (lane & 31) >> 4, kgrp = lane >> 5;
   int addr[2][8];
 #pragma unroll
@@ -525,27 +520,10 @@
 #pragma unroll
   for (int mt = 0; mt < 2; ++mt) {
     f32x16 acc[2];
-#pragma unroll
-    for (int nt = 0; nt < 2; ++nt)
-#pragma unroll
-      for (int r = 0; r < 16; ++r) acc[nt][r] = 0.f;
-#pragma unroll
-    for (int ks = 0; ks < 2; ++ks) {
-      half8 bh, bl;
-#pragma unroll
-      for (int j = 0; j < 8; ++j) {
-        const int off = (ks * 16 + kgrp * 8 + j < 27) ? mt * 2 * 54 * 4 : 0;
-        const float v = *reinterpret_cast<const float*>(pb + addr[ks][j] + off);
-        bh[j] = (half_t)v;
-        bl[j] = (half_t)(v - (float)bh[j]);
-      }
-#pragma unroll
-      for (int nt = 0; nt < 2; ++nt) {
-        acc[nt] = __builtin_amdgcn_mfma_f32_32x32x16_f16(wl[nt][ks], bh, acc[nt], 0, 0, 0);
-        acc[nt] = __builtin_amdgcn_mfma_f32_32x32x16_f16(wh[nt][ks], bl, acc[nt], 0, 0, 0);
-        acc[nt] = __builtin_amdgcn_mfma_f32_32x32x16_f16(wh[nt][ks], bh, acc[nt], 0, 0, 0);
-      }
-    }
+    conv1_tile(wh, wl, [=](int ks, int j) {
+      const int off = (ks * 16 + kgrp * 8 + j < 27) ? mt * 2 * 54 * 4 : 0;
+      return *reinterpret_cast<const float*>(pb + addr[ks][j] + off);
+    }, acc);
     const int px = lane & 31;
 #pragma unroll
     for (int nt = 0; nt < 2; ++nt)
@@ -553,9 +531,9 @@
       for (int rq = 0; rq < 4; ++rq) {
         f32x4 v;
 #pragma unroll
-        for (int j = 0; j < 4; ++j) v[j] = fmaxf(acc[nt][rq * 4 + j] + bias[nt][rq][j], 0.f);
+        for (int j = 0; j < 4; ++j) v[j] = conv1_act(acc[nt][rq * 4 + j], bias[nt][rq][j]);
         const int piece = nt * 8 + 2 * rq + kgrp;
-        *reinterpret_cast<f32x4*>(wt + (px * 16 + (piece ^ (px & 15))) * 16) = v;
+        if (STORE) *reinterpret_cast<f32x4*>(wt + (px * 16 + (piece ^ (px & 15))) * 16) = v;
         if (p.usum) {
           f32x4 t = v;
           unit_row_sum4(t);
@@ -567,6 +545,7 @@
           }
         }
       }
+    if (!STORE) continue;
     __builtin_amdgcn_fence(__ATOMIC_RELEASE, "wavefront");
     __builtin_amdgcn_wave_barrier();
     const int oy0 = y0 + wave * 4 + mt * 2;
@@ -608,9 +587,11 @@
 
 int launch_conv_first(const ConvFirstArgs& a, hipStream_t s) {
   ARG_CHECK(a.H > 1 && a.W > 1 && a.B > 0);
-  ARG_CHECK(!a.usum || (a.y32 && a.umax && a.W % 16 == 0));
+  ARG_CHECK(!a.usum || (a.umax && a.W % 16 == 0));
+  ARG_CHECK(a.y16 || a.y32 || a.usum);
   const int strips_x = cdiv(a.W, 64), tiles_y = cdiv(a.H, 16);
-  hipLaunchKernelGGL(conv_first_kernel, dim3(strips_x * tiles_y, a.B), dim3(256), 0, s, a, strips_x);
+  if (a.y16 || a.y32) hipLaunchKernelGGL(conv_first_kernel<true>, dim3(strips_x * tiles_y, a.B), dim3(256), 0, s, a, strips_x);
+  else hipLaunchKernelGGL(conv_first_kernel<false>, dim3(strips_x * tiles_y, a.B), dim3(256), 0, s, a, strips_x);
   HIP_TRY(hipGetLastError());
   return WCT_OK;
 }
diff --git a/wct_tf_amd/csrc/conv_first_tile.h b/wct_tf_amd/csrc/conv_first_tile.h
--- /dev/null
+++ b/wct_tf_amd/csrc/conv_first_tile.h
@@ -0,0 +1,75 @@
+#pragma once
+#include "common.h"
+
+__device__ __forceinline__ float conv1_fetch(float v, int clamp01) { return clamp01 ? fminf(fmaxf(v, 0.f), 1.f) : v; }
+
+template <bool PIXEL_ROWS = false, typename Value>
+__device__ __forceinline__ void conv1_tile(const half8 (&wh)[2][2], const half8 (&wl)[2][2], Value value, f32x16 (&acc)[2]) {
+#pragma unroll
+  for (int nt = 0; nt < 2; ++nt)
+#pragma unroll
+    for (int r = 0; r < 16; ++r) acc[nt][r] = 0.f;
+#pragma unroll
+  for (int ks = 0; ks < 2; ++ks) {
+    half8 bh, bl;
+#pragma unroll
+    for (int j = 0; j < 8; ++j) {
+      const float v = value(ks, j);
+      bh[j] = (half_t)v;
+      bl[j] = (half_t)(v - (float)bh[j]);
+    }
+#pragma unroll
+    for (int nt = 0; nt < 2; ++nt) {
+      if constexpr (PIXEL_ROWS) {
+        acc[nt] = __builtin_amdgcn_mfma_f32_32x32x16_f16(bh, wl[nt][ks], acc[nt], 0, 0, 0);
+        acc[nt] = __builtin_amdgcn_mfma_f32_32x32x16_f16(bl, wh[nt][ks], acc[nt], 0, 0, 0);
+        acc[nt] = __builtin_amdgcn_mfma_f32_32x32x16_f16(bh, wh[nt][ks], acc[nt], 0, 0, 0);
+      } else {
+        acc[nt] = __builtin_amdgcn_mfma_f32_32x32x16_f16(wl[nt][ks], bh, acc[nt], 0, 0, 0);
+        acc[nt] = __builtin_amdgcn_mfma_f32_32x32x16_f16(wh[nt][ks], bl, acc[nt], 0, 0, 0);
+        acc[nt] = __builtin_amdgcn_mfma_f32_32x32x16_f16(wh[nt][ks], bh, acc[nt], 0, 0, 0);
+      }
+    }
+  }
+}
+
+__device__ __forceinline__ float conv1_act(float acc, float bias) { return fmaxf(acc + bias, 0.f); }
+
+__device__ __forceinline__ void conv1_weights(const half_t* wfrag, int lane, half8 (&wh)[2][2], half8 (&wl)[2][2]) {
+#pragma unroll
+  for (int t = 0; t < 2; ++t)
+#pragma unroll
+    for (int ks = 0; ks < 2; ++ks) {
+      wh[t][ks] = *reinterpret_cast<const half8*>(wfrag + (((t * 2 + ks) * 2 + 0) * 64 + lane) * 8);
+      wl[t][ks] = *reinterpret_cast<const half8*>(wfrag + (((t * 2 + ks) * 2 + 1) * 64 + lane) * 8);
+    }
+}
+
+__device__ __forceinline__ void conv1_patch_load(const float* x, int y, int px, int H, int W, int kgrp, float (&pre)[2][8]) {
+  const int ry[3] = {abs(y - 1), y, min(y + 1, 2 * H - 3 - y)};
+  const int rx[3] = {abs(px - 1) * 3, px * 3, min(px + 1, 2 * W - 3 - px) * 3};
+  int t[3][3];
+#pragma unroll
+  for (int ky = 0; ky < 3; ++ky)
+#pragma unroll
+    for (int kx = 0; kx < 3; ++kx) t[ky][kx] = ry[ky] * (W * 3) + rx[kx];
+#pragma unroll
+  for (int ks = 0; ks < 2; ++ks)
+#pragma unroll
+    for (int j = 0; j < 8; ++j) {
+      const int ka = ks * 16 + j, kb = ks * 16 + 8 + j < 27 ? ks * 16 + 8 + j : ka;
+      const int oa = t[ka / 9][(ka % 9) / 3] + ka % 3, ob = t[kb / 9][(kb % 9) / 3] + kb % 3;
+      pre[ks][j] = x[kgrp ? ob : oa];
+    }
+}
+__device__ __forceinline__ void conv1_patch_values(const float (&pre)[2][8], int kgrp, int clamp01, float (&cur)[2][8]) {
+#pragma unroll
+  for (int ks = 0; ks < 2; ++ks)
+#pragma unroll
+    for (int j = 0; j < 8; ++j) cur[ks][j] = ks * 16 + 8 + j < 27 ? pre[ks][j] : (kgrp ? 0.f : pre[ks][j]);
+  if (clamp01)
+#pragma unroll
+    for (int ks = 0; ks < 2; ++ks)
+#pragma unroll
+      for (int j = 0; j < 8; ++j) cur[ks][j] = conv1_fetch(cur[ks][j], 1);
+}
diff --git a/wct_tf_amd/csrc/stats_gemm.hip b/wct_tf_amd/csrc/stats_gemm.hip
--- a/wct_tf_amd/csrc/stats_gemm.hip
+++ b/wct_tf_amd/csrc/stats_gemm.hip
@@ -1,4 +1,6 @@
 #include "wct_stages.h"
+#include "conv_first_tile.h"
+#include <type_traits>
 
 
 struct StatArgs {
@@ -486,6 +488,116 @@
   }
 }
 
+struct CovImageArgs {
+  WctImageSrc src;
+  const float* mean;
+  const float* scale;
+  float* partial;
+  int ksplit, nsplit;
+  WctSkip skip;
+};
+
+__global__ __launch_bounds__(256, 2) void cov_image_kernel(CovImageArgs p) {
+  constexpr int C = 64;
+  __shared__ __attribute__((aligned(16))) unsigned char lds[4][2][C * 64];
+  const int tid = threadIdx.x, lane = tid & 63, wave = tid >> 6;
+  const int wm = wave >> 1, wn = wave & 1;
+  const int mat = blockIdx.z, split = blockIdx.y;
+  if (skip_style_mat(mat, p.skip)) return;
+  const int side = mat & 1, pair = mat >> 1;
+  const int H = side ? p.src.side[1].H : p.src.side[0].H, W = side ? p.src.side[1].W : p.src.side[0].W;
+  const int clamp01 = side ? p.src.side[1].clamp01 : p.src.side[0].clamp01;
+  const int N = H * W;
+  const float* x = (side ? p.src.side[1].img : p.src.side[0].img) + (size_t)pair * N * 3;
+  const int kbeg = split * p.ksplit;
+  const int kend = min(N, kbeg + p.ksplit);
+  const float sc = p.scale[mat];
+  const int kgrp = lane >> 5, ch = lane & 31;
+
+  half8 wh[2][2], wl[2][2];
+  conv1_weights(p.src.wfrag, lane, wh, wl);
+  float bias[2], mean[2];
+#pragma unroll
+  for (int nt = 0; nt < 2; ++nt) { bias[nt] = p.src.bias[nt * 32 + ch]; mean[nt] = p.mean[mat * C + nt * 32 + ch]; }
+
+  f32x16 acc;
+#pragma unroll
+  for (int r = 0; r < 16; ++r) acc[r] = 0.f;
+
+  float pre[2][8];
+  int py, px;
+  {
+    const int n = kbeg + wave * 32 + (lane & 31);
+    py = n / W; px = n - py * W;
+  }
+  auto fetch = [&]() {
+    conv1_patch_load(x, min(py, H - 1), px, H, W, kgrp, pre);
+    px += 128;
+    while (px >= W) { px -= W; ++py; }
+  };
+  auto mma_stage = [&](const unsigned char* hi, const unsigned char* lo) {
+#pragma unroll
+    for (int ks = 0; ks < 2; ++ks) {
+      const int chunk = ks * 2 + (lane >> 5);
+      const int ra = wm * 32 + (lane & 31), rb = wn * 32 + (lane & 31);
+      const int offa = (ra * 4 + (chunk ^ ((ra >> 2) & 3))) * 16, offb = (rb * 4 + (chunk ^ ((rb >> 2) & 3))) * 16;
+      const half8 ah = *reinterpret_cast<const half8*>(hi + offa), al = *reinterpret_cast<const half8*>(lo + offa);
+      const half8 bh = *reinterpret_cast<const half8*>(hi + offb), bl = *reinterpret_cast<const half8*>(lo + offb);
+      acc = __builtin_amdgcn_mfma_f32_32x32x16_f16(al, bh, acc, 0, 0, 0);
+      acc = __builtin_amdgcn_mfma_f32_32x32x16_f16(ah, bl, acc, 0, 0, 0);
+      acc = __builtin_amdgcn_mfma_f32_32x32x16_f16(ah, bh, acc, 0, 0, 0);
+    }
+  };
+
+  auto park = [&](const f32x16 (&f)[2], int ks0, auto tail) {
+#pragma unroll
+    for (int nt = 0; nt < 2; ++nt) {
+      const int c = nt * 32 + ch;
+#pragma unroll
+      for (int rq = 0; rq < 4; ++rq) {
+        half4 h, l;
+#pragma unroll
+        for (int j = 0; j < 4; ++j) {
+          const float s_in = (!decltype(tail)::value || ks0 + rq * 8 + kgrp * 4 + j < kend) ? sc : 0.f;
+          const float v = (conv1_act(f[nt][rq * 4 + j], bias[nt]) - mean[nt]) * s_in;
+          h[j] = (half_t)v;
+          l[j] = (half_t)(v - (float)h[j]);
+        }
+        const int off = (c * 4 + (rq ^ ((c >> 2) & 3))) * 16 + kgrp * 8;
+        *reinterpret_cast<half4*>(lds[wave][0] + off) = h;
+        *reinterpret_cast<half4*>(lds[wave][1] + off) = l;
+      }
+    }
+  };
+
+  if (kbeg + wave * 32 < kend) fetch();
+  for (int k0 = kbeg; k0 < kend; k0 += 128) {
+    const int ks0 = k0 + wave * 32;
+    if (ks0 < kend) {
+      float cur[2][8];
+      conv1_patch_values(pre, kgrp, clamp01, cur);
+      if (ks0 + 128 < kend) fetch();
+      f32x16 f[2];
+      conv1_tile<true>(wh, wl, [=](int ks, int j) { return cur[ks][j]; }, f);
+      if (ks0 + 32 <= kend) park(f, ks0, std::false_type());
+      else park(f, ks0, std::true_type());
+    }
+    __syncthreads();
+#pragma unroll
+    for (int st = 0; st < 4; ++st)
+      if (k0 + st * 32 < kend) mma_stage(lds[st][0], lds[st][1]);
+    __syncthreads();
+  }
+
+  float* out = p.partial + ((size_t)mat * p.nsplit + split) * C * C;
+  const int gn = wn * 32 + (lane & 31);
+#pragma unroll
+  for (int r = 0; r < 16; ++r) {
+    const int gm = wm * 32 + (r & 3) + 8 * (r >> 2) + 4 * (lane >> 5);
+    out[(size_t)gm * C + gn] = acc[r];
+  }
+}
+
 static int stat_passes(StatArgs sa, int nmat, float* mean, float* var, float* scale, float d0, float d1, hipStream_t s) {
   const int C = sa.C;
   sa.mean = nullptr;
@@ -535,6 +647,21 @@
   return cov_passes(ca, 2 * P, w.A, w.A0, 1.f / (float)(Nc - 1), 1.f / (float)(Ns - 1), eps, s);
 }
 
+int launch_cov_image(const WctImageSrc& src, int P, const WctCarve& w, float eps, WctSkip skip, hipStream_t s) {
+  constexpr int C = 64;
+  for (int b = 0; b < 2; ++b) ARG_CHECK(src.side[b].img && src.side[b].H >= 2 && src.side[b].W >= 16 && src.side[b].W % 16 == 0);
+  ARG_CHECK(src.wfrag && src.bias && w.ksplit % 32 == 0);
+  const int Nc = src.side[0].H * src.side[0].W, Ns = src.side[1].H * src.side[1].W;
+  CovImageArgs ca;
+  ca.src = src; ca.mean = w.mean; ca.scale = w.scale; ca.partial = w.cov_partial;
+  ca.ksplit = w.ksplit; ca.nsplit = w.nsplit; ca.skip = skip;
+  hipLaunchKernelGGL(cov_image_kernel, dim3(1, w.nsplit, 2 * P), dim3(256), 0, s, ca);
+  hipLaunchKernelGGL(cov_finish_kernel, dim3(1, 1, 2 * P), dim3(256), 0, s, ca.partial, ca.scale, w.A, C, ca.nsplit, 64,
+                     1.f / (float)(Nc - 1), 1.f / (float)(Ns - 1), eps, (int)skip, w.A0);
+  HIP_TRY(hipGetLastError());
+  return WCT_OK;
+}
+
 static int launch_slot_means(const float* x, int N, int C, int m, int nslab, const WctCarve& w, bool with_var, hipStream_t s,
                              const float* u, const unsigned* umax) {
   StatArgs sa = {};
diff --git a/wct_tf_amd/csrc/wct.hip b/wct_tf_amd/csrc/wct.hip
--- a/wct_tf_amd/csrc/wct.hip
+++ b/wct_tf_amd/csrc/wct.hip
@@ -1,6 +1,7 @@
 #include "wct_stages.h"
 #include "jacobi_dev.h"
 #include "strength_rule.h"
+#include "conv_first_tile.h"
 #include <algorithm>
 #include <type_traits>
 
@@ -219,6 +220,179 @@
 template int launch_apply_args<ApplySegArgs>(const ApplySegArgs&, int, int, hipStream_t);
 template int launch_apply_args<ApplySegBatchArgs>(const ApplySegBatchArgs&, int, int, hipStream_t);
 template int launch_apply_args<ApplyMapArgs>(const ApplyMapArgs&, int, int, hipStream_t);
+
+struct ApplyImageArgs : ApplyArgs { WctImageSide img; const half_t* wfrag; const float* bias1; };
+constexpr int APPLY_IMAGE_TILES = 8;
+
+__global__ __launch_bounds__(256, 2) void apply_image_kernel(ApplyImageArgs p) {
+  constexpr int C = 64, BP = 128, TN = BP / 64;
+  __shared__ __attribute__((aligned(16))) unsigned char lm[2][2][C * 64];
+  __shared__ __attribute__((aligned(16))) unsigned char lx[2][2][BP * 64];
+  __shared__ __attribute__((aligned(16))) float lbm[2][C];
+  typedef unsigned int u32x4 __attribute__((ext_vector_type(4)));
+  const int tid = threadIdx.x, lane = tid & 63, wave = tid >> 6;
+  const int wm = wave >> 1, wn = wave & 1;
+  const int pair = blockIdx.z;
+  const int H = p.img.H, W = p.img.W, N = H * W;
+  const int tile0 = blockIdx.x * APPLY_IMAGE_TILES;
+  const int ntile = min(APPLY_IMAGE_TILES, (N + BP - 1) / BP - tile0);
+  const float* x = p.img.img + (size_t)pair * N * 3;
+  const float* M = p.M + (size_t)pair * C * C;
+  const float* mean = p.mean + (size_t)pair * 2 * C;
+  const float sx = p.xscale[2 * pair];
+  float sM = 1.f;
+  {
+    const float m = __uint_as_float(p.mabs[pair]);
+    if (m > 0.f) { int e; frexpf(m, &e); sM = ldexpf(1.f, 14 - e); }
+  }
+  const int kgrp = lane >> 5;
+
+  const int mrow = tid >> 2, mkq = tid & 3;
+  const float* mp = M + (size_t)mrow * C + mkq * 8;
+  const int moff = (mrow * 4 + (mkq ^ ((mrow >> 2) & 3))) * 16;
+  f32x4 rm[2][2];
+#pragma unroll
+  for (int s = 0; s < 2; ++s) {
+    rm[s][0] = *reinterpret_cast<const f32x4*>(mp + s * 32);
+    rm[s][1] = *reinterpret_cast<const f32x4*>(mp + s * 32 + 4);
+  }
+  const float* bias = p.bias + (size_t)pair * C;
+  f32x4 bvs[4];
+#pragma unroll
+  for (int rq = 0; rq < 4; ++rq) bvs[rq] = *reinterpret_cast<const f32x4*>(bias + wm * 32 + 8 * rq + 4 * kgrp);
+  if (tid < C) { lbm[0][tid] = p.bias1[tid]; lbm[1][tid] = mean[tid]; }
+
+  int py, px;
+  {
+    const int n = tile0 * BP + wave * 32 + (lane & 31);
+    py = n / W; px = n - py * W;
+  }
+  float pre[2][8];
+  auto fetch = [&]() {
+    conv1_patch_load(x, min(py, H - 1), px, H, W, kgrp, pre);
+    px += BP;
+    while (px >= W) { px -= W; ++py; }
+  };
+  fetch();
+  half8 wh[2][2], wl[2][2];
+  conv1_weights(p.wfrag, lane, wh, wl);
+#pragma unroll
+  for (int s = 0; s < 2; ++s) {
+    half8 h, l;
+#pragma unroll
+    for (int j = 0; j < 8; ++j) {
+      const float v = rm[s][j >> 2][j & 3] * sM;
+      h[j] = (half_t)v;
+      l[j] = (half_t)(v - (float)h[j]);
+    }
+    *reinterpret_cast<half8*>(lm[s][0] + moff) = h;
+    *reinterpret_cast<half8*>(lm[s][1] + moff) = l;
+  }
+  __syncthreads();
+
+  const int xrow = wave * 32 + (lane & 31);
+  const float inv = 1.f / (sx * sM);
+  for (int t = 0; t < ntile; ++t) {
+    f32x16 f[2];
+    {
+      float cur[2][8];
+      conv1_patch_values(pre, kgrp, p.img.clamp01, cur);
+      if (t + 1 < ntile) fetch();
+      conv1_tile(wh, wl, [=](int ks, int j) { return cur[ks][j]; }, f);
+    }
+#pragma unroll
+    for (int s = 0; s < 2; ++s)
+#pragma unroll
+      for (int rq = 0; rq < 4; ++rq) {
+        const int ch = s * 32 + 8 * rq + 4 * kgrp;
+        const f32x4 b1 = *reinterpret_cast<const f32x4*>(&lbm[0][ch]), mc = *reinterpret_cast<const f32x4*>(&lbm[1][ch]);
+        half4 h, l;
+#pragma unroll
+        for (int j = 0; j < 4; ++j) {
+          const float v = (conv1_act(f[s][rq * 4 + j], b1[j]) - mc[j]) * sx;
+          h[j] = (half_t)v;
+          l[j] = (half_t)(v - (float)h[j]);
+        }
+        const int off = (xrow * 4 + (rq ^ ((xrow >> 2) & 3))) * 16 + kgrp * 8;
+        *reinterpret_cast<half4*>(lx[s][0] + off) = h;
+        *reinterpret_cast<half4*>(lx[s][1] + off) = l;
+      }
+    __syncthreads();
+
+    f32x16 acc[TN];
+#pragma unroll
+    for (int j = 0; j < TN; ++j)
+#pragma unroll
+      for (int r = 0; r < 16; ++r) acc[j][r] = 0.f;
+#pragma unroll
+    for (int s = 0; s < 2; ++s)
+#pragma unroll
+      for (int ks = 0; ks < 2; ++ks) {
+        const int chunk = ks * 2 + (lane >> 5);
+        half8 bh[TN], bl[TN];
+        const int r = wm * 32 + (lane & 31);
+        const int offa = (r * 4 + (chunk ^ ((r >> 2) & 3))) * 16;
+        const half8 ah = *reinterpret_cast<const half8*>(lm[s][0] + offa), al = *reinterpret_cast<const half8*>(lm[s][1] + offa);
+#pragma unroll
+        for (int j = 0; j < TN; ++j) {
+          const int rb = (wn * TN + j) * 32 + (lane & 31);
+          const int off = (rb * 4 + (chunk ^ ((rb >> 2) & 3))) * 16;
+          bh[j] = *reinterpret_cast<const half8*>(lx[s][0] + off);
+          bl[j] = *reinterpret_cast<const half8*>(lx[s][1] + off);
+        }
+#pragma unroll
+        for (int j = 0; j < TN; ++j) {
+          acc[j] = __builtin_amdgcn_mfma_f32_32x32x16_f16(al, bh[j], acc[j], 0, 0, 0);
+          acc[j] = __builtin_amdgcn_mfma_f32_32x32x16_f16(ah, bl[j], acc[j], 0, 0, 0);
+          acc[j] = __builtin_amdgcn_mfma_f32_32x32x16_f16(ah, bh[j], acc[j], 0, 0, 0);
+        }
+      }
+    __syncthreads();
+
+    const int n0 = (tile0 + t) * BP;
+#pragma unroll
+    for (int j = 0; j < TN; ++j) {
+      const int n = n0 + (wn * TN + j) * 32 + (lane & 31);
+      const bool n_ok = n < N;
+      const size_t row = ((size_t)pair * N + (n_ok ? n : 0)) * C;
+      const int cb = wm * 32;
+      unsigned pk[4][2];
+#pragma unroll
+      for (int rq = 0; rq < 4; ++rq) {
+        const int co = cb + 8 * rq + 4 * kgrp;
+        f32x4 v;
+#pragma unroll
+        for (int q = 0; q < 4; ++q) v[q] = acc[j][rq * 4 + q] * inv + bvs[rq][q];
+        if (p.out32 && n_ok) *reinterpret_cast<f32x4*>(p.out32 + row + co) = v;
+        typedef _Float16 h2 __attribute__((ext_vector_type(2)));
+        h2 lo = {(half_t)v[0], (half_t)v[1]}, hi = {(half_t)v[2], (half_t)v[3]};
+        pk[rq][0] = __builtin_bit_cast(unsigned, lo);
+        pk[rq][1] = __builtin_bit_cast(unsigned, hi);
+      }
+      if (p.out16) {
+#pragma unroll
+        for (int m = 0; m < 2; ++m) {
+          auto sxw = __builtin_amdgcn_permlane32_swap(pk[2 * m][0], pk[2 * m + 1][0], false, false);
+          auto syw = __builtin_amdgcn_permlane32_swap(pk[2 * m][1], pk[2 * m + 1][1], false, false);
+          u32x4 o = {sxw[0], syw[0], sxw[1], syw[1]};
+          const int co = cb + 16 * m + 8 * kgrp;
+          if (n_ok) *reinterpret_cast<u32x4*>(p.out16 + row + co) = o;
+        }
+      }
+    }
+  }
+}
+
+static int launch_apply_image(const WctCarve& w, const WctImageSrc& src, int P, half_t* out16, float* out32, hipStream_t s) {
+  const WctImageSide& im = src.side[0];
+  ARG_CHECK(im.img && im.H >= 2 && im.W >= 2 && src.wfrag && src.bias);
+  ApplyImageArgs a;
+  static_cast<ApplyArgs&>(a) = apply_args<ApplyArgs>(w, nullptr, im.H * im.W, 64, out16, out32);
+  a.img = im; a.wfrag = src.wfrag; a.bias1 = src.bias;
+  hipLaunchKernelGGL(apply_image_kernel, dim3(cdiv(cdiv(a.N, 128), APPLY_IMAGE_TILES), 1, P), dim3(256), 0, s, a);
+  HIP_TRY(hipGetLastError());
+  return WCT_OK;
+}
 
 static int wct_nslab(int N) { int s = cdiv(N, 64); return s < 1 ? 1 : (s > 256 ? 256 : s); }
 
@@ -383,9 +557,11 @@
 }
 
 int launch_wct(const float* content, int Nc, const float* style, int Ns, int C, int P, WctSkip skip, const WctCall& r,
-               const WctFeatStats* stats, const WctStyleRef* prep, const WctWarmRef* warm, const WctStrength* sm) {
+               const WctFeatStats* stats, const WctStyleRef* prep, const WctWarmRef* warm, const WctStrength* sm, const WctImageSrc* src) {
   const int mode = r.mode, stages = r.stages; hipStream_t s = r.stream;
   ARG_CHECK(C % 32 == 0 && C >= 32 && C <= 1024 && Nc >= 2 && Ns >= 2 && P >= 1 && P <= 32);
+  ARG_CHECK(!src || (C == 64 && !prep && !warm && !sm && stats && stats->u[0] && stats->umax[0] && stats->u[1] && stats->umax[1] &&
+                     src->side[0].H * src->side[0].W == Nc && src->side[1].H * src->side[1].W == Ns));
   ARG_CHECK(!sm || strength_ok(*sm, Nc));
   ARG_CHECK(skip == WCT_SKIP_NONE || skip == WCT_SKIP_SHARED_STYLE);
   ARG_CHECK(!warm || (warm->basis && (skip == WCT_SKIP_NONE || prep)));
@@ -397,7 +573,9 @@
   int rc;
   if (stages & WCT_STAGE_COV) {
     if ((rc = launch_means(content, Nc, style, Ns, C, P, w, false, skip, s, stats))) return rc;
-    if ((rc = launch_cov(content, Nc, style, Ns, C, P, w, cov_eps(mode, r.eps), skip, s))) return rc;
+    if (src) rc = launch_cov_image(*src, P, w, cov_eps(mode, r.eps), skip, s);
+    else rc = launch_cov(content, Nc, style, Ns, C, P, w, cov_eps(mode, r.eps), skip, s);
+    if (rc) return rc;
   }
   if (stages & WCT_STAGE_EIG) {
     const bool rotate = warm && warm->valid;
@@ -412,6 +590,10 @@
   if (prep && (rc = launch_style_load(*prep, 1, w, C, true, s))) return rc;
   if ((rc = launch_spectral_tail(w, C, P, sm ? 1.f : r.alpha, mode, r.eps, skip, P, s))) return rc;
   if (sm) return launch_blend_apply_map(w, content, Nc, C, P, skip, r, *sm);
+  if (src) {
+    if ((rc = launch_blend(w, C, P, r.alpha, skip, s))) return rc;
+    return launch_apply_image(w, *src, P, r.out16, r.out32, s);
+  }
   return launch_blend_apply(w, content, Nc, C, P, skip, r);
 }
 
diff --git a/wct_tf_amd/csrc/wct_stages.h b/wct_tf_amd/csrc/wct_stages.h
--- a/wct_tf_amd/csrc/wct_stages.h
+++ b/wct_tf_amd/csrc/wct_stages.h
@@ -67,6 +67,7 @@
 int launch_cov(const float* content, int Nc, const float* style, int Ns, int C, int P, const WctCarve& w, float eps, WctSkip skip,
                hipStream_t s);
 int launch_plan_stats(const SlotPlan& sp, int C, bool with_var, bool with_cov, float eps, hipStream_t s);
+int launch_cov_image(const WctImageSrc& src, int P, const WctCarve& w, float eps, WctSkip skip, hipStream_t s);
 int launch_eig_stage(const WctCarve& w, int C, int P, WctSkip skip, int u_f16, int* sweeps_dev, int* eig_fail, hipStream_t s,
                      int check_from = 2);
 int launch_spectral_tail(const WctCarve& w, int C, int P, float alpha, int mode, float eps_in, WctSkip skip, int nwhite, hipStream_t s);
```
